# AlexGidiotis/Multimodal-Gesture-Recognition-with-LSTMs-and-CTC

Hardware: AMD Instinct MI355X
Metric: train frames/sec, fusion BiLSTM+CTC (higher is better)
Workload: dtype f32

## Files before the change

### include/mgr.h

```cpp
#ifndef MGR_H_
#define MGR_H_

#include <stddef.h>
#include <stdint.h>

#ifdef __cplusplus
extern "C" {
#endif

typedef struct mgr_ctx mgr_ctx;
typedef struct mgr_comm mgr_comm;

#define MGR_NUM_STREAMS 8
#define MGR_NUM_EVENTS 64
#define MGR_UNIQUE_ID_BYTES 128

int mgr_version(void);
const char* mgr_last_error(void);
int mgr_device_count(int* n);
int mgr_ctx_create(int device, mgr_ctx** out);
int mgr_ctx_destroy(mgr_ctx* ctx);
int mgr_device_info(mgr_ctx* ctx, int* cu_count, size_t* hbm_bytes, char* name, int name_len);

int mgr_alloc(mgr_ctx* ctx, size_t bytes, void** dptr);
int mgr_free(mgr_ctx* ctx, void* dptr);
int mgr_memset(mgr_ctx* ctx, void* d, int byte, size_t n);
int mgr_h2d(mgr_ctx* ctx, void* d, const void* h, size_t n);
int mgr_host_alloc(mgr_ctx* ctx, size_t bytes, void** out);
int mgr_host_free(mgr_ctx* ctx, void* p);
int mgr_h2d_async(mgr_ctx* ctx, void* d, const void* h_pinned, size_t n);
int mgr_d2h(mgr_ctx* ctx, void* h, const void* d, size_t n);
int mgr_d2h_async(mgr_ctx* ctx, void* h_pinned, const void* d, size_t n);
int mgr_event_sync(mgr_ctx* ctx, int ev);
int mgr_d2d(mgr_ctx* ctx, void* dst, const void* src, size_t n);
int mgr_sync(mgr_ctx* ctx);
int mgr_stream_set(mgr_ctx* ctx, int idx);
int mgr_stream_wait(mgr_ctx* ctx, int waiter, int waited);
int mgr_stream_set_priority(mgr_ctx* ctx, int idx, int level);
int mgr_event_record(mgr_ctx* ctx, int ev);
int mgr_stream_wait_event(mgr_ctx* ctx, int waiter, int ev);
int mgr_event_elapsed_ms(mgr_ctx* ctx, int ev0, int ev1, float* ms);
enum {
  MGR_K_GEMM_NN = 0, MGR_K_GEMM_TN = 1, MGR_K_GEMM_NT = 2, MGR_K_SCAN_FWD = 3, MGR_K_SCAN_BWD = 4,
  MGR_K_DENSE_FWD = 5, MGR_K_DENSE_BWD = 6, MGR_K_CTC = 7, MGR_K_ADAM = 8, MGR_K_MISC = 9, MGR_K_ALLREDUCE = 10,
  MGR_K_SCAN_FWD_NARROW = 11, MGR_K_COUNT = 12
};
int mgr_prof_enable(mgr_ctx* ctx, int family_mask);
int mgr_prof_get(mgr_ctx* ctx, int family, int* launches, float* ms);
int mgr_prof_reset(mgr_ctx* ctx);

int mgr_add_gaussian_noise(mgr_ctx* ctx, const float* X, float* Y, size_t n, float stddev, uint64_t seed);
int mgr_dropout_mask(mgr_ctx* ctx, float* mask, size_t n, float p, uint64_t seed);

int mgr_lstm_pack(mgr_ctx* ctx, const float* src, float* dst, int rows, int H, int to_keras);
int mgr_transpose(mgr_ctx* ctx, const float* src, float* dst, int rows, int cols);
int mgr_lstm_input_proj(mgr_ctx* ctx, const float* X, int ldx, const float* mask4, const float* Wp,
                        const float* bp, float* Z, int B, int T, int F, int H);
int mgr_lstm_input_proj_pair(mgr_ctx* ctx, const float* X, int ldx, const float* mask4_fwd, const float* Wp_fwd,
                             const float* bp_fwd, float* Z_fwd, const float* mask4_rev, const float* Wp_rev,
                             const float* bp_rev, float* Z_rev, int B, int T, int F, int H);
size_t mgr_lstm_input_proj_dropout_ws_bytes(int B, int F, int H);
int mgr_lstm_input_proj_dropout(mgr_ctx* ctx, const float* X, int ldx, const float* mask4, float drop_rate,
                                const float* Wp, const float* bp, float* Z, int B, int T, int F, int H, void* ws,
                                size_t ws_bytes);
int mgr_lstm_input_proj_dropout_wants_transposed(mgr_ctx* ctx, float drop_rate, int F);
int mgr_lstm_input_proj_dropout_t(mgr_ctx* ctx, const float* XT, int ldt, const float* mask4, float drop_rate,
                                  const float* Wp, const float* bp, float* Z, int B, int T, int F, int H, void* ws,
                                  size_t ws_bytes, float x_absmax);
int mgr_transpose_bt(mgr_ctx* ctx, const float* X, int ldx, float* XT, int ldt, int B, int T, int F);
size_t mgr_lstm_input_proj_dropout_ts_ws_bytes(int B, int F, int H);
int mgr_lstm_input_proj_dropout_ts(mgr_ctx* ctx, const float* XS, int ldt, const float* mask4, float drop_rate,
                                   const float* Wp, const float* bp, float* Z, int B, int T, int F, int H, void* ws,
                                   size_t ws_bytes);
int mgr_transpose_bt_split(mgr_ctx* ctx, const float* X, int ldx, float* XS, int ldt, int B, int T, int F);
int mgr_transpose_bt_split_shift(mgr_ctx* ctx, const float* X, int ldx, float* XS, int ldt, int B, int T, int F, int tshift);
int mgr_weight_planes_cache(mgr_ctx* ctx, const float* Wp, int frozen);
size_t mgr_lstm_scan_ws_bytes(int B, int T, int H);
int mgr_lstm_scan_fwd(mgr_ctx* ctx, const float* Z, const float* Up, float* Y, int ldy, const float* R,
                      int ldr, float* gates, float* cs, int B, int T, int H, int reverse, void* ws,
                      size_t ws_bytes);
typedef struct mgr_scan_job {
  const float* Z;
  const float* Up;
  float* Y;
  const float* R;
  float* gates;
  float* cs;
  int ldy, ldr, B, T, H, reverse;
  float* YT;
  long long ytb;
  int ldt;
  int yt_split;
} mgr_scan_job;
size_t mgr_lstm_scan_multi_ws_bytes(int njobs, const mgr_scan_job* jobs);
int mgr_lstm_scan_fwd_multi(mgr_ctx* ctx, int njobs, const mgr_scan_job* jobs, void* ws, size_t ws_bytes);
enum { MGR_SCAN_FORM_AUTO = 0, MGR_SCAN_FORM_PLAIN = 1, MGR_SCAN_FORM_FUSED = 3,
       MGR_SCAN_FORM_FUSED_ANY = 4 };
enum { MGR_BPTT_FORM_AUTO = 0, MGR_BPTT_FORM_TRIMMED = 1, MGR_BPTT_FORM_YIELDING = 2, MGR_BPTT_FORM_DIRECT = 3,
       MGR_BPTT_FORM_FUSED = 4, MGR_BPTT_FORM_FUSED_DIRECT = 5,
       MGR_BPTT_FORM_SINGLE_CU = 6 };
#define MGR_SEQ_NONE 0xFFFFFFFFu
typedef struct mgr_scan_launch_opts {
  unsigned struct_size;
  int form;
  unsigned* seq_out;
} mgr_scan_launch_opts;
int mgr_lstm_scan_fwd_multi_ex(mgr_ctx* ctx, int njobs, const mgr_scan_job* jobs, void* ws, size_t ws_bytes,
                               const mgr_scan_launch_opts* opts);
#define MGR_ABI_REVISION 7
int mgr_abi_struct_sizes(unsigned out[4]);
enum {
  MGR_TUNE_SCAN_PATH = 0,
  MGR_TUNE_SCAN_SYNC_CHECK = 1,
  MGR_TUNE_SCAN_PRINT_PLAN = 2,
  MGR_TUNE_SCAN_NO_XCD_LOCAL = 3,
  MGR_TUNE_SCAN_FORM = 4,
  MGR_TUNE_SCAN_LDS_IMAGE = 7,
  MGR_TUNE_BPTT_SPLIT_ROLE = 8,
  MGR_TUNE_PROJ_DENSE = 9,
  MGR_TUNE_PROJ_DENSE16_MASKED = 10,
  MGR_TUNE_PROJ_WIDE_TILES = 11,
  MGR_TUNE_PROJ_TS_TILE = 12,
  MGR_TUNE_DENSE_VALU = 13,
  MGR_TUNE_SCAN_F32_MFMA = 14,
  MGR_TUNE_GEMM_F32 = 15,
  MGR_TUNE_BPTT_FORM = 16,
  MGR_TUNE_CTC_ONE_SAMPLE = 18,
  MGR_TUNE_BPTT_SINGLE_CU = 19,
  MGR_TUNE_CTC_CHAIN_LDS_KIB = 20,
  MGR_TUNE_CTC_FRAME_LDS_KIB = 21,
  MGR_TUNE_COUNT = 24
};
int mgr_tune(mgr_ctx* ctx, int key, int value);
int mgr_tune_get(mgr_ctx* ctx, int key, int* value);
enum { MGR_SCAN_GAVE_UP = 1, MGR_SCAN_NONFINITE = 8 };
int mgr_scan_status(mgr_ctx* ctx, unsigned* out);
int mgr_scan_status_ex(mgr_ctx* ctx, unsigned out[4]);
int mgr_scan_status_clear(mgr_ctx* ctx);
int mgr_scan_status_bind(mgr_ctx* ctx, void* block);
int mgr_scan_status_inject(mgr_ctx* ctx, unsigned bits);
int mgr_update_gate_eval(mgr_ctx* ctx, unsigned mask, float* flag);
int mgr_update_gate_set(mgr_ctx* ctx, const float* flag);
int mgr_stream_wait_next_resident(mgr_ctx* ctx, int timeout_us);
int mgr_stream_wait_resident(mgr_ctx* ctx, unsigned seq, int timeout_us);
int mgr_stream_wait_resident_word(mgr_ctx* ctx, const unsigned* seq_word, int timeout_us);
int mgr_resident_wait_stats(mgr_ctx* ctx, unsigned out[4]);
int mgr_persist_stats(mgr_ctx* ctx, int* launches, int* serialised);
int mgr_probe_xcc(mgr_ctx* ctx, int nblocks, int threads, int lds_bytes, int32_t* out);
int mgr_probe_guest(mgr_ctx* ctx, int nblocks, int threads, int lds_bytes, int us, int64_t* out);
int mgr_stream_delay(mgr_ctx* ctx, int us);
int mgr_lstm_scan_bwd(mgr_ctx* ctx, const float* dY, int lddy, const float* gates, const float* cs,
                      const float* Up, float* dZ, int B, int T, int H, int reverse, void* ws, size_t ws_bytes);
typedef struct mgr_scan_bwd_job {
  const float* dY;
  const float* gates;
  const float* cs;
  const float* Up;
  float* dZ;
  int lddy, B, T, H, reverse;
  unsigned* dzmax;
  float* dbsum;
} mgr_scan_bwd_job;
size_t mgr_lstm_scan_bwd_multi_ws_bytes(int njobs, const mgr_scan_bwd_job* jobs);
int mgr_lstm_scan_bwd_multi(mgr_ctx* ctx, int njobs, const mgr_scan_bwd_job* jobs, void* ws, size_t ws_bytes);
int mgr_lstm_scan_bwd_multi_ex(mgr_ctx* ctx, int njobs, const mgr_scan_bwd_job* jobs, void* ws, size_t ws_bytes,
                               const mgr_scan_launch_opts* opts);
size_t mgr_lstm_param_grads_ws_bytes(int B, int T, int F, int H);
int mgr_lstm_param_grads(mgr_ctx* ctx, const float* X, int ldx, const float* mask4, const float* Hs, int ldh,
                         const float* dZ, float* dWp, float* dUp, float* dbp, int B, int T, int F, int H,
                         int reverse, void* ws, size_t ws_bytes);
size_t mgr_lstm_param_grads_dropout_ws_bytes(int B, int T, int F, int H);
int mgr_lstm_param_grads_dropout(mgr_ctx* ctx, const float* X, int ldx, const float* mask4, float drop_rate,
                                 const float* Hs, int ldh, const float* dZ, float* dWp, float* dUp, float* dbp, int B,
                                 int T, int F, int H, int reverse, void* ws, size_t ws_bytes);
int mgr_lstm_param_grads_dropout_wants_transposed(mgr_ctx* ctx, float drop_rate, int F);
size_t mgr_lstm_param_grads_dropout_t_ws_bytes(int B, int T, int F, int H, int ldt);
int mgr_lstm_param_grads_dropout_t(mgr_ctx* ctx, const float* XT, int ldt, const float* mask4, float drop_rate,
                                   const float* Hs, int ldh, const float* dZ, float* dWp, float* dUp, float* dbp, int B,
                                   int T, int F, int H, int reverse, void* ws, size_t ws_bytes, float x_absmax);
size_t mgr_lstm_param_grads_dropout_ts_ws_bytes(int B, int T, int F, int H, int ldt);
int mgr_lstm_param_grads_dropout_ts(mgr_ctx* ctx, const float* XS, int ldt, const float* mask4, float drop_rate,
                                    const float* Hs, int ldh, const float* dZ, float* dWp, float* dUp, float* dbp, int B,
                                    int T, int F, int H, int reverse, void* ws, size_t ws_bytes, const unsigned* dzmax,
                                    const float* dbsum, const void* proj_ws, const float* HsT);
int mgr_lstm_input_grad(mgr_ctx* ctx, const float* dZ, const float* Wp, const float* mask4, float* dX,
                        int lddx, int accumulate, int B, int T, int F, int H);

int mgr_dense_softmax_fwd(mgr_ctx* ctx, const float* A, int lda, const float* dmask, float p, uint64_t seed,
                          const float* Wd, const float* bd, float* P, int B, int T, int D, int C);
size_t mgr_dense_bwd_ws_bytes(int B, int T, int D, int C);
int mgr_dense_bwd(mgr_ctx* ctx, const float* A, int lda, const float* dmask, float p, uint64_t seed,
                  const float* dLogits, const float* Wd, float* dWd, float* dbd, float* dA, int ldda, int B,
                  int T, int D, int C, void* ws, size_t ws_bytes);
size_t mgr_head_ws_bytes(int B, int T, int D, int C, int Lmax);
int mgr_head_fwd_bwd(mgr_ctx* ctx, const float* A, int lda, const float* dmask, float p, uint64_t seed, const float* Wd, const float* bd,
                     const int32_t* labels, const int32_t* input_len, const int32_t* label_len, int B, int T, int D, int C, int Lmax,
                     int skip, int blank, float eps, float gscale, float* P, float* loss, float* loss_mean, float* dLogits, float* dWd,
                     float* dbd, float* dA, int ldda, void* ws, size_t ws_bytes);

size_t mgr_ctc_ws_bytes(int B, int T, int C, int Lmax);
int mgr_ctc_loss_grad(mgr_ctx* ctx, const float* P, const int32_t* labels, const int32_t* input_len,
                      const int32_t* label_len, int B, int T, int C, int Lmax, int skip, int blank, float eps,
                      float gscale, float* loss, float* dLogits, void* ws, size_t ws_bytes);

int mgr_adam_step(mgr_ctx* ctx, float* p, const float* g, float* m, float* v, size_t n, float lr_t, float b1,
                  float b2, float eps, float clipvalue, float gscale);
int mgr_maxnorm_cols(mgr_ctx* ctx, float* W, int rows, int cols, float maxv, float eps);
int mgr_add2d(mgr_ctx* ctx, const float* A, int lda, const float* Bm, int ldb, float* Out, int ldo, size_t rows,
              int cols);
int mgr_mean(mgr_ctx* ctx, const float* x, int n, float* out);

int mgr_comm_unique_id(uint8_t id[MGR_UNIQUE_ID_BYTES]);
int mgr_comm_init_rank(mgr_ctx* ctx, int nranks, int rank, const uint8_t id[MGR_UNIQUE_ID_BYTES], mgr_comm** out);
int mgr_allreduce_sum(mgr_comm* comm, float* dbuf, size_t n);
int mgr_allreduce_max(mgr_comm* comm, float* dbuf, size_t n);
int mgr_comm_destroy(mgr_comm* comm);
int mgr_comm_count(mgr_comm* comm, int* nranks_seen, int* rank_seen);

int mgr_frame_argmax(mgr_ctx* ctx, const float* P, int B, int T, int C, int skip, int32_t* best, float* prob);
size_t mgr_ctc_beam_ws_bytes(int B, int T, int C, int beam);
int mgr_ctc_beam_search(mgr_ctx* ctx, const float* P, const int32_t* input_len, int B, int T, int C, int skip,
                        int blank, int beam, float eps, int merge_repeated, int32_t* out, int32_t* out_len,
                        double* logp, void* ws, size_t ws_bytes);
size_t mgr_ctc_beam_lm_ws_bytes(int B, int T, int C, int beam, int top_paths);
int mgr_ctc_beam_search_lm(mgr_ctx* ctx, const float* P, const int32_t* input_len, int B, int T, int C, int skip, int blank, int beam,
                           float eps, const double* ext, const double* fin, int top_paths, int32_t* out, int32_t* out_len,
                           double* score, double* logp_ctc, void* ws, size_t ws_bytes);

size_t mgr_ctc_align_ws_bytes(int B, int T, int C, int Lmax);
int mgr_ctc_align(mgr_ctx* ctx, const float* P, const int32_t* labels, const int32_t* input_len, const int32_t* label_len, int B, int T,
                  int C, int Lmax, int skip, int blank, float eps, int32_t* path, int32_t* seg, float* conf, double* logp, void* ws,
                  size_t ws_bytes);
#define MGR_SEGMENTS_MAX_FRAMES 8192
int mgr_greedy_segments(mgr_ctx* ctx, const float* P, int B, int T, int C, int skip, float thr, int cap, int32_t* n_runs, int32_t* lab,
                        int32_t* seg, float* conf);

#define MGR_LEXICON_MAX_PHRASES 64
#define MGR_LEXICON_MAX_WORDS   255
size_t mgr_ctc_lexicon_ws_bytes(int B, int T, int C, int G, const int32_t* phrase_off);
int mgr_ctc_lexicon_decode(mgr_ctx* ctx, const float* P, const int32_t* input_len, int B, int T, int C, int skip, int blank, float eps,
                           const int32_t* phrase_off, const int32_t* phrase_words, int G, const double* ext, const double* fin, int cap,
                           int32_t* n_phr, int32_t* phr, int32_t* seg, float* conf, int32_t* path, double* score, double* logp, void* ws,
                           size_t ws_bytes);

#define MGR_RESCORE_MAX_LABELS 255
#define MGR_RESCORE_MAX_WIDTH  65536
size_t mgr_ctc_rescore_ws_bytes(int B, int T, int C, int G, const int32_t* phrase_off);
int mgr_ctc_rescore(mgr_ctx* ctx, const float* P, const int32_t* input_len, int B, int T, int C, int skip, int blank, float eps,
                    const int32_t* phrase_off, const int32_t* phrase_words, int G, const int32_t* hyp, const int32_t* hyp_len, int K,
                    int Lh, double* logp, int32_t* n_lab, void* ws, size_t ws_bytes);

#define MGR_RISK_MAX_SLOTS 32
size_t mgr_ctc_risk_ws_bytes(int B, int T, int C, int K, int Lcap, int G, const int32_t* phrase_off);
int mgr_ctc_risk_grad(mgr_ctx* ctx, const float* P, const int32_t* input_len, int B, int T, int C, int skip, int blank, float eps,
                      const int32_t* phrase_off, const int32_t* phrase_words, int G, const int32_t* hyp, const int32_t* hyp_len, int K,
                      int Lh, int Lcap, const int32_t* risk, float risk_scale, float post_scale, float gscale, int accumulate,
                      double* logp, float* weight, float* exp_risk, float* dLogits, void* ws, size_t ws_bytes);

#define MGR_SAMPLE_MAX_DRAWS 32
int mgr_ctc_sample_paths(mgr_ctx* ctx, const float* P, const int32_t* input_len, int B, int T, int C, int skip, int blank, float eps,
                         uint64_t seed, int K, int32_t* out, int32_t* out_len, int32_t* count, int32_t* n_unique, int32_t* path);

#define MGR_EDIT_MAX_LEN  4095
#define MGR_EDIT_MAX_COST 16384
size_t mgr_edit_distance_ws_bytes(int n_pairs, int Lh, int Lr, int want_ops);
int mgr_edit_distance(mgr_ctx* ctx, const int32_t* hyp, const int32_t* hyp_len, int n_hyp, int Lh, const int32_t* ref,
                      const int32_t* ref_len, int n_ref, int Lr, const int32_t* pair_h, const int32_t* pair_r, int n_pairs, int cost_sub,
                      int cost_del, int cost_ins, uint64_t ignore_mask, int32_t* dist, int32_t* counts, int32_t* lens, int8_t* ops,
                      int32_t* n_ops, void* ws, size_t ws_bytes);

#define MGR_CONV_NO_GRAD 0xFF
int mgr_conv_pool_fwd(mgr_ctx* ctx, const float* X, int N, int Hin, int Win, int Cin, const float* W, const float* b, int ks, int Cout,
                      float* Y, uint8_t* code);
int mgr_conv_pool_bwd_data(mgr_ctx* ctx, const float* dY, const uint8_t* code, const float* W, int N, int Hin, int Win, int Cin, int ks,
                           int Cout, float* dX);
size_t mgr_conv_pool_bwd_weights_ws_bytes(int N, int Hin, int Win, int Cin, int ks, int Cout);
int mgr_conv_pool_bwd_weights(mgr_ctx* ctx, const float* X, const float* dY, const uint8_t* code, int N, int Hin, int Win, int Cin, int ks,
                              int Cout, float* dW, float* db, void* ws, size_t ws_bytes);

#define MGR_SKELETAL_JOINT_COLS 12
#define MGR_SKELETAL_FEATURE_COLS 23
int mgr_skeletal_features(mgr_ctx* ctx, const double* joints, size_t n_frames, double* out);

#define MGR_ACTIVITY_JOINT_COLS 20
#define MGR_ACTIVITY_REST_COLS 16
#define MGR_ACTIVITY_OUT_COLS 5
#define MGR_ACTIVITY_MAX_FILES 65536
#define MGR_ACTIVITY_MAX_FRAMES (1LL << 26)
int mgr_skeletal_activity(mgr_ctx* ctx, const int32_t* joints, const int64_t* offsets, int n_files, long long n_frames, int rest_given,
                          int32_t* rest, int32_t* out, int32_t* status);

size_t mgr_mfcc_ws_bytes(int n_utts, long long n_frames, int frameSize, int fftN, int numChans, int numCeps);
int mgr_mfcc(mgr_ctx* ctx, const int16_t* samples, const int64_t* sample_offsets, int n_utts, long long n_frames, int frameSize,
             int frameRate, int fftN, int numChans, int numCeps, int cepLifter, double preemph, int deltas, int accs, int out_stride,
             const int32_t* loChan, const double* loWt, float* out, const int64_t* out_offsets, void* ws, size_t ws_bytes);

int mgr_roi_crop(mgr_ctx* ctx, const uint8_t* frames, int n, int H, int W, const int32_t* boxes, int img_dim, uint8_t* out);

#ifdef __cplusplus
}
#endif
#endif
```

### multimodal-gesture-recognition-with-lstms-and-ctc_amd/_capi.py

```python
import ctypes as C
import os

import numpy as np

HERE = os.path.dirname(os.path.abspath(__file__))
LIB_PATH = os.path.join(HERE, "libmgr.so")

c_float_p = C.POINTER(C.c_float)
c_int32_p = C.POINTER(C.c_int32)
vp = C.c_void_p
sz = C.c_size_t
u64 = C.c_uint64
i32 = C.c_int

SIGNATURES = {
    "mgr_version": (i32, []),
    "mgr_last_error": (C.c_char_p, []),
    "mgr_device_count": (i32, [C.POINTER(i32)]),
    "mgr_ctx_create": (i32, [i32, C.POINTER(vp)]),
    "mgr_ctx_destroy": (i32, [vp]),
    "mgr_device_info": (i32, [vp, C.POINTER(i32), C.POINTER(sz), C.c_char_p, i32]),
    "mgr_alloc": (i32, [vp, sz, C.POINTER(vp)]),
    "mgr_free": (i32, [vp, vp]),
    "mgr_memset": (i32, [vp, vp, i32, sz]),
    "mgr_h2d": (i32, [vp, vp, vp, sz]),
    "mgr_d2h": (i32, [vp, vp, vp, sz]),
    "mgr_d2d": (i32, [vp, vp, vp, sz]),
    "mgr_d2h_async": (i32, [vp, vp, vp, sz]),
    "mgr_event_sync": (i32, [vp, i32]),
    "mgr_sync": (i32, [vp]),
    "mgr_stream_set": (i32, [vp, i32]),
    "mgr_stream_wait": (i32, [vp, i32, i32]),
    "mgr_stream_set_priority": (i32, [vp, i32, i32]),
    "mgr_event_record": (i32, [vp, i32]),
    "mgr_stream_wait_event": (i32, [vp, i32, i32]),
    "mgr_event_elapsed_ms": (i32, [vp, i32, i32, C.POINTER(C.c_float)]),
    "mgr_prof_enable": (i32, [vp, i32]),
    "mgr_prof_get": (i32, [vp, i32, C.POINTER(i32), C.POINTER(C.c_float)]),
    "mgr_prof_reset": (i32, [vp]),
    "mgr_add_gaussian_noise": (i32, [vp, vp, vp, sz, C.c_float, u64]),
    "mgr_dropout_mask": (i32, [vp, vp, sz, C.c_float, u64]),
    "mgr_lstm_pack": (i32, [vp, vp, vp, i32, i32, i32]),
    "mgr_transpose": (i32, [vp, vp, vp, i32, i32]),
    "mgr_lstm_input_proj": (i32, [vp, vp, i32, vp, vp, vp, vp, i32, i32, i32, i32]),
    "mgr_lstm_input_proj_dropout_ws_bytes": (sz, [i32, i32, i32]),
    "mgr_lstm_input_proj_dropout": (i32, [vp, vp, i32, vp, C.c_float, vp, vp, vp, i32, i32, i32, i32, vp, sz]),
    "mgr_lstm_input_proj_dropout_wants_transposed": (i32, [vp, C.c_float, i32]),
    "mgr_lstm_input_proj_dropout_t": (i32, [vp, vp, i32, vp, C.c_float, vp, vp, vp, i32, i32, i32, i32, vp, sz, C.c_float]),
    "mgr_transpose_bt": (i32, [vp, vp, i32, vp, i32, i32, i32, i32]),
    "mgr_lstm_input_proj_dropout_ts_ws_bytes": (sz, [i32, i32, i32]),
    "mgr_lstm_input_proj_dropout_ts": (i32, [vp, vp, i32, vp, C.c_float, vp, vp, vp, i32, i32, i32, i32, vp, sz]),
    "mgr_transpose_bt_split": (i32, [vp, vp, i32, vp, i32, i32, i32, i32]),
    "mgr_transpose_bt_split_shift": (i32, [vp, vp, i32, vp, i32, i32, i32, i32, i32]),
    "mgr_weight_planes_cache": (i32, [vp, vp, i32]),
    "mgr_lstm_input_proj_pair": (i32, [vp, vp, i32, vp, vp, vp, vp, vp, vp, vp, vp, i32, i32, i32, i32]),
    "mgr_lstm_scan_ws_bytes": (sz, [i32, i32, i32]),
    "mgr_lstm_scan_fwd": (i32, [vp, vp, vp, vp, i32, vp, i32, vp, vp, i32, i32, i32, i32, vp, sz]),
    "mgr_lstm_scan_multi_ws_bytes": (sz, [i32, vp]),
    "mgr_lstm_scan_fwd_multi": (i32, [vp, i32, vp, vp, sz]),
    "mgr_lstm_scan_fwd_multi_ex": (i32, [vp, i32, vp, vp, sz, vp]),
    "mgr_abi_struct_sizes": (i32, [vp]),
    "mgr_tune": (i32, [vp, i32, i32]),
    "mgr_tune_get": (i32, [vp, i32, C.POINTER(i32)]),
    "mgr_probe_xcc": (i32, [vp, i32, i32, i32, vp]),
    "mgr_stream_delay": (i32, [vp, i32]),
    "mgr_probe_guest": (i32, [vp, i32, i32, i32, i32, vp]),
    "mgr_host_alloc": (i32, [vp, sz, C.POINTER(vp)]),
    "mgr_host_free": (i32, [vp, vp]),
    "mgr_h2d_async": (i32, [vp, vp, vp, sz]),
    "mgr_scan_status": (i32, [vp, vp]),
    "mgr_scan_status_clear": (i32, [vp]),
    "mgr_scan_status_ex": (i32, [vp, vp]),
    "mgr_scan_status_bind": (i32, [vp, vp]),
    "mgr_scan_status_inject": (i32, [vp, C.c_uint]),
    "mgr_update_gate_eval": (i32, [vp, C.c_uint, vp]),
    "mgr_update_gate_set": (i32, [vp, vp]),
    "mgr_stream_wait_next_resident": (i32, [vp, i32]),
    "mgr_stream_wait_resident": (i32, [vp, C.c_uint, i32]),
    "mgr_stream_wait_resident_word": (i32, [vp, vp, i32]),
    "mgr_resident_wait_stats": (i32, [vp, vp]),
    "mgr_persist_stats": (i32, [vp, C.POINTER(i32), C.POINTER(i32)]),
    "mgr_skeletal_features": (i32, [vp, vp, sz, vp]),
    "mgr_skeletal_activity": (i32, [vp, vp, vp, i32, C.c_longlong, i32, vp, vp, vp]),
    "mgr_mfcc_ws_bytes": (sz, [i32, C.c_longlong, i32, i32, i32, i32]),
    "mgr_mfcc": (i32, [vp, vp, vp, i32, C.c_longlong, i32, i32, i32, i32, i32, i32, C.c_double, i32, i32, i32, vp, vp, vp, vp, vp,
                       sz]),
    "mgr_lstm_scan_bwd_multi_ws_bytes": (sz, [i32, vp]),
    "mgr_lstm_scan_bwd_multi": (i32, [vp, i32, vp, vp, sz]),
    "mgr_lstm_scan_bwd_multi_ex": (i32, [vp, i32, vp, vp, sz, vp]),
    "mgr_lstm_scan_bwd": (i32, [vp, vp, i32, vp, vp, vp, vp, i32, i32, i32, i32, vp, sz]),
    "mgr_lstm_param_grads_ws_bytes": (sz, [i32, i32, i32, i32]),
    "mgr_lstm_param_grads": (i32, [vp, vp, i32, vp, vp, i32, vp, vp, vp, vp, i32, i32, i32, i32, i32, vp, sz]),
    "mgr_lstm_param_grads_dropout_ws_bytes": (sz, [i32, i32, i32, i32]),
    "mgr_lstm_param_grads_dropout": (i32, [vp, vp, i32, vp, C.c_float, vp, i32, vp, vp, vp, vp, i32, i32, i32, i32, i32, vp, sz]),
    "mgr_lstm_param_grads_dropout_wants_transposed": (i32, [vp, C.c_float, i32]),
    "mgr_lstm_param_grads_dropout_t_ws_bytes": (sz, [i32, i32, i32, i32, i32]),
    "mgr_lstm_param_grads_dropout_t": (i32, [vp, vp, i32, vp, C.c_float, vp, i32, vp, vp, vp, vp, i32, i32, i32, i32, i32, vp, sz, C.c_float]),
    "mgr_lstm_param_grads_dropout_ts_ws_bytes": (sz, [i32, i32, i32, i32, i32]),
    "mgr_lstm_param_grads_dropout_ts": (i32, [vp, vp, i32, vp, C.c_float, vp, i32, vp, vp, vp, vp, i32, i32, i32, i32, i32, vp, sz, vp, vp, vp, vp]),
    "mgr_lstm_input_grad": (i32, [vp, vp, vp, vp, vp, i32, i32, i32, i32, i32, i32]),
    "mgr_dense_softmax_fwd": (i32, [vp, vp, i32, vp, C.c_float, u64, vp, vp, vp, i32, i32, i32, i32]),
    "mgr_dense_bwd_ws_bytes": (sz, [i32, i32, i32, i32]),
    "mgr_dense_bwd": (i32, [vp, vp, i32, vp, C.c_float, u64, vp, vp, vp, vp, vp, i32, i32, i32, i32, i32, vp, sz]),
    "mgr_head_ws_bytes": (sz, [i32, i32, i32, i32, i32]),
    "mgr_head_fwd_bwd": (i32, [vp, vp, i32, vp, C.c_float, u64, vp, vp, vp, vp, vp, i32, i32, i32, i32, i32, i32, i32, C.c_float, C.c_float,
                               vp, vp, vp, vp, vp, vp, vp, i32, vp, sz]),
    "mgr_ctc_ws_bytes": (sz, [i32, i32, i32, i32]),
    "mgr_ctc_loss_grad": (i32, [vp, vp, vp, vp, vp, i32, i32, i32, i32, i32, i32, C.c_float, C.c_float, vp, vp, vp, sz]),
    "mgr_adam_step": (i32, [vp, vp, vp, vp, vp, sz, C.c_float, C.c_float, C.c_float, C.c_float, C.c_float, C.c_float]),
    "mgr_maxnorm_cols": (i32, [vp, vp, i32, i32, C.c_float, C.c_float]),
    "mgr_add2d": (i32, [vp, vp, i32, vp, i32, vp, i32, sz, i32]),
    "mgr_mean": (i32, [vp, vp, i32, vp]),
    "mgr_comm_unique_id": (i32, [C.c_char_p]),
    "mgr_comm_init_rank": (i32, [vp, i32, i32, C.c_char_p, C.POINTER(vp)]),
    "mgr_allreduce_sum": (i32, [vp, vp, sz]),
    "mgr_allreduce_max": (i32, [vp, vp, sz]),
    "mgr_comm_destroy": (i32, [vp]),
    "mgr_comm_count": (i32, [vp, C.POINTER(i32), C.POINTER(i32)]),
    "mgr_frame_argmax": (i32, [vp, vp, i32, i32, i32, i32, vp, vp]),
    "mgr_ctc_beam_ws_bytes": (sz, [i32, i32, i32, i32]),
    "mgr_ctc_beam_search": (i32, [vp, vp, vp, i32, i32, i32, i32, i32, i32, C.c_float, i32, vp, vp, vp, vp, sz]),
    "mgr_ctc_beam_lm_ws_bytes": (sz, [i32, i32, i32, i32, i32]),
    "mgr_ctc_beam_search_lm": (i32, [vp, vp, vp, i32, i32, i32, i32, i32, i32, C.c_float, vp, vp, i32, vp, vp, vp, vp, vp, sz]),
    "mgr_ctc_align_ws_bytes": (sz, [i32, i32, i32, i32]),
    "mgr_ctc_align": (i32, [vp, vp, vp, vp, vp, i32, i32, i32, i32, i32, i32, C.c_float, vp, vp, vp, vp, vp, sz]),
    "mgr_greedy_segments": (i32, [vp, vp, i32, i32, i32, i32, C.c_float, i32, vp, vp, vp, vp]),
    "mgr_ctc_lexicon_ws_bytes": (sz, [i32, i32, i32, i32, vp]),
    "mgr_ctc_lexicon_decode": (i32, [vp, vp, vp, i32, i32, i32, i32, i32, C.c_float, vp, vp, i32, vp, vp, i32, vp, vp, vp, vp, vp, vp, vp, vp,
                                     sz]),
    "mgr_ctc_rescore_ws_bytes": (sz, [i32, i32, i32, i32, vp]),
    "mgr_ctc_rescore": (i32, [vp, vp, vp, i32, i32, i32, i32, i32, C.c_float, vp, vp, i32, vp, vp, i32, i32, vp, vp, vp, sz]),
    "mgr_ctc_risk_ws_bytes": (sz, [i32, i32, i32, i32, i32, i32, vp]),
    "mgr_ctc_risk_grad": (i32, [vp, vp, vp, i32, i32, i32, i32, i32, C.c_float, vp, vp, i32, vp, vp, i32, i32, i32, vp, C.c_float, C.c_float,
                                C.c_float, i32, vp, vp, vp, vp, vp, sz]),
    "mgr_ctc_sample_paths": (i32, [vp, vp, vp, i32, i32, i32, i32, i32, C.c_float, u64, i32, vp, vp, vp, vp, vp]),
    "mgr_edit_distance_ws_bytes": (sz, [i32, i32, i32, i32]),
    "mgr_edit_distance": (i32, [vp, vp, vp, i32, i32, vp, vp, i32, i32, vp, vp, i32, i32, i32, i32, u64, vp, vp, vp, vp, vp, vp, sz]),
    "mgr_conv_pool_fwd": (i32, [vp, vp, i32, i32, i32, i32, vp, vp, i32, i32, vp, vp]),
    "mgr_conv_pool_bwd_data": (i32, [vp, vp, vp, vp, i32, i32, i32, i32, i32, i32, vp]),
    "mgr_conv_pool_bwd_weights_ws_bytes": (sz, [i32, i32, i32, i32, i32, i32]),
    "mgr_conv_pool_bwd_weights": (i32, [vp, vp, vp, vp, i32, i32, i32, i32, i32, i32, vp, vp, vp, sz]),
    "mgr_roi_crop": (i32, [vp, vp, i32, i32, i32, vp, i32, vp]),
}

SCAN_GAVE_UP, SCAN_NONFINITE = 1, 8

(K_GEMM_NN, K_GEMM_TN, K_GEMM_NT, K_SCAN_FWD, K_SCAN_BWD, K_DENSE_FWD, K_DENSE_BWD, K_CTC, K_ADAM, K_MISC, K_ALLREDUCE, K_SCAN_FWD_NARROW) = range(12)
KERNEL_FAMILIES = ["gemm_nn", "gemm_tn", "gemm_nt", "scan_fwd", "scan_bwd", "dense_fwd", "dense_bwd", "ctc", "adam", "misc", "allreduce",
                   "scan_fwd_narrow"]



class ScanJob(C.Structure):
    _fields_ = [("Z", vp), ("Up", vp), ("Y", vp), ("R", vp), ("gates", vp), ("cs", vp),
                ("ldy", i32), ("ldr", i32), ("B", i32), ("T", i32), ("H", i32), ("reverse", i32),
                ("YT", vp), ("ytb", C.c_longlong), ("ldt", i32), ("yt_split", i32)]


class ScanBwdJob(C.Structure):
    _fields_ = [("dY", vp), ("gates", vp), ("cs", vp), ("Up", vp), ("dZ", vp),
                ("lddy", i32), ("B", i32), ("T", i32), ("H", i32), ("reverse", i32), ("dzmax", vp), ("dbsum", vp)]


class ScanLaunchOpts(C.Structure):
    _fields_ = [("struct_size", C.c_uint), ("form", i32), ("seq_out", vp)]


SCAN_FORM_AUTO, SCAN_FORM_PLAIN, SCAN_FORM_FUSED, SCAN_FORM_FUSED_ANY = 0, 1, 3, 4
BPTT_FORM_AUTO, BPTT_FORM_TRIMMED, BPTT_FORM_YIELDING, BPTT_FORM_DIRECT, BPTT_FORM_FUSED, BPTT_FORM_FUSED_DIRECT, BPTT_FORM_SINGLE_CU = range(7)
SEQ_NONE = 0xFFFFFFFF
ABI_REVISION = 7
TUNE_SCAN_PATH = 0
TUNE_SCAN_SYNC_CHECK = 1
TUNE_SCAN_PRINT_PLAN = 2
TUNE_SCAN_NO_XCD_LOCAL = 3
TUNE_SCAN_FORM = 4
TUNE_SCAN_LDS_IMAGE = 7
TUNE_BPTT_SPLIT_ROLE = 8
TUNE_PROJ_DENSE = 9
TUNE_PROJ_DENSE16_MASKED = 10
TUNE_PROJ_WIDE_TILES = 11
TUNE_PROJ_TS_TILE = 12
TUNE_DENSE_VALU = 13
TUNE_SCAN_F32_MFMA = 14
TUNE_GEMM_F32 = 15
TUNE_BPTT_FORM = 16
TUNE_CTC_ONE_SAMPLE = 18
TUNE_BPTT_SINGLE_CU = 19
TUNE_CTC_CHAIN_LDS_KIB = 20
TUNE_CTC_FRAME_LDS_KIB = 21
TUNE_COUNT = 24


def make_launch_opts(form=0, seq_out=0):
    o = ScanLaunchOpts()
    o.struct_size = C.sizeof(ScanLaunchOpts)
    o.form = int(form)
    o.seq_out = int(seq_out) or None
    return o


def make_scan_bwd_jobs(jobs):
    arr = (ScanBwdJob * len(jobs))()
    for a, j in zip(arr, jobs):
        for k in ("dY", "gates", "cs", "Up", "dZ", "dzmax", "dbsum"):
            v = j.get(k, 0)
            setattr(a, k, v.ptr if isinstance(v, DeviceArray) else (v or 0))
        for k in ("lddy", "B", "T", "H", "reverse"):
            setattr(a, k, int(j[k]))
    return arr


def make_scan_jobs(jobs):
    arr = (ScanJob * len(jobs))()
    for a, j in zip(arr, jobs):
        for k in ("Z", "Up", "Y", "R", "gates", "cs", "YT"):
            v = j.get(k, 0)
            setattr(a, k, v.ptr if isinstance(v, DeviceArray) else (v or 0))
        for k in ("ldy", "ldr", "B", "T", "H", "reverse", "ytb", "ldt", "yt_split"):
            setattr(a, k, int(j.get(k, 0)))
    return arr


_lib = None


class MgrError(RuntimeError):
    pass


def load_library(build_if_missing=True):
    global _lib
    if _lib is not None:
        return _lib
    if not os.path.exists(LIB_PATH) and build_if_missing:
        from . import _build
        _build.build(verbose=False)
    if not os.path.exists(LIB_PATH):
        raise MgrError("libmgr.so is missing (%s) and could not be built; there is no CPU fallback" % LIB_PATH)
    lib = C.CDLL(LIB_PATH)
    for name, (res, args) in SIGNATURES.items():
        fn = getattr(lib, name)
        fn.restype = res
        fn.argtypes = args
    sizes = (C.c_uint * 4)()
    if lib.mgr_abi_struct_sizes(sizes) != 0 or tuple(sizes) != (C.sizeof(ScanJob), C.sizeof(ScanBwdJob), C.sizeof(ScanLaunchOpts), ABI_REVISION):
        raise MgrError("libmgr.so was built from another include/mgr.h than this binding (struct sizes / revision %s, expected %s): rebuild it"
                       % (tuple(sizes), (C.sizeof(ScanJob), C.sizeof(ScanBwdJob), C.sizeof(ScanLaunchOpts), ABI_REVISION)))
    _lib = lib
    return lib


def check(rc, lib=None):
    if rc != 0:
        lib = lib or load_library()
        raise MgrError("libmgr error %d: %s" % (rc, lib.mgr_last_error().decode(errors="replace")))


class DeviceArray:

    __slots__ = ("dev", "ptr", "shape", "dtype", "nbytes", "_own")

    def __init__(self, dev, ptr, shape, dtype, own=True):
# ... 146 lines not shown
```

### multimodal-gesture-recognition-with-lstms-and-ctc_amd/csrc/common.h

```cpp
#pragma once
#include <hip/hip_runtime.h>
#include <stdarg.h>
#include <stdint.h>
#include <stdio.h>
#include <string.h>

#include "../../include/mgr.h"
#include "ws_layout.h"

constexpr int MGR_MAX_PERSIST = 8;
constexpr int MGR_MAX_FROZEN = 32;

constexpr size_t MGR_SMALL_D2H = 4096;

enum : unsigned {
  MGR_ATTR_SCAN_CLUSTER = 1u, MGR_ATTR_SCAN_CLUSTER_BWD = 2u, MGR_ATTR_SCAN_CLUSTER_FUSED = 64u,
  MGR_ATTR_PROJ_SPLIT = 16u, MGR_ATTR_DW_SPLIT = 32u, MGR_ATTR_PROJ_NARROW = 2048u,
  MGR_ATTR_CTC = 128u, MGR_ATTR_ALIGN = 512u, MGR_ATTR_SEGMENTS = 1024u, MGR_ATTR_ROI = 256u,
  MGR_ATTR_LEXICON = 4096u, MGR_ATTR_RISK = 8192u,
};

struct mgr_ctx {
  int device;
  int cu_count;
  size_t hbm_bytes;
  char name[64];
  hipStream_t streams[MGR_NUM_STREAMS];
  int cur;
  hipEvent_t events[MGR_NUM_EVENTS];
  hipEvent_t xev[64];
  int xev_next;
  int prof_mask;
  struct ProfPair {
    hipEvent_t a, b;
  };
  ProfPair* prof_pairs[MGR_K_COUNT];
  int prof_n[MGR_K_COUNT];
  int prof_cap[MGR_K_COUNT];
  float prof_ms[MGR_K_COUNT];
  int prof_launches[MGR_K_COUNT];
  int tune[MGR_TUNE_COUNT];
  void* h_small_pinned;
  unsigned* sticky_status;
  unsigned* status_bound;
  const float* gate_flag;
  struct Persist {
    hipEvent_t done;
    int active, stream, wgs, waves, per_cu, fused;
    unsigned seq;
  };
  Persist persist[MGR_MAX_PERSIST];
  unsigned persist_seq;
  int persist_serialised;
  unsigned attr_done;
  struct PlaneEntry {
    const void* Wp;
    const void* ws;
    int B, F, H;
    const char* region;
    size_t region_bytes;
  };
  const void* frozen_w[MGR_MAX_FROZEN];
  PlaneEntry planes[MGR_MAX_FROZEN];
  unsigned planes_evict, frozen_evict;
};

int mgr_fail(int code, const char* fmt, ...);

static inline bool mgr_planes_overlap(const mgr_ctx::PlaneEntry& e, const void* p, size_t n) {
  const char* a = static_cast<const char*>(p);
  return e.Wp && a < e.region + e.region_bytes && e.region < a + n;
}
static inline void mgr_planes_forget_range(mgr_ctx* c, const void* p, size_t n) {
  if (!p || !n) return;
  for (int i = 0; i < MGR_MAX_FROZEN; ++i)
    if (mgr_planes_overlap(c->planes[i], p, n)) c->planes[i] = mgr_ctx::PlaneEntry{};
}

#define MGR_HIP(expr)                                                                      \
  do {                                                                                     \
    hipError_t _e = (expr);                                                                \
    if (_e != hipSuccess) return mgr_fail(-2, "%s failed: %s", #expr, hipGetErrorString(_e)); \
  } while (0)

#define MGR_REQUIRE(cond, ...)                  \
  do {                                          \
    if (!(cond)) return mgr_fail(-1, __VA_ARGS__); \
  } while (0)

#define MGR_LAUNCH_CHECK() MGR_HIP(hipGetLastError())

static inline hipStream_t mgr_stream(mgr_ctx* c) { return c->streams[c->cur]; }
static inline unsigned* mgr_status_block(mgr_ctx* c) { return c->status_bound ? c->status_bound : c->sticky_status; }

int mgr_prof_begin(mgr_ctx* c, int family);
int mgr_prof_end(mgr_ctx* c, int family);

static inline size_t mgr_align_up(size_t x, size_t a) { return (x + a - 1) / a * a; }
static inline int mgr_grid256(size_t n, size_t cap) { return (int)((n + 255) / 256 < cap ? (n + 255) / 256 : cap); }

__host__ __device__ static inline uint64_t mgr_mix64(uint64_t z) {
  z += 0x9E3779B97F4A7C15ull;
  z = (z ^ (z >> 30)) * 0xBF58476D1CE4E5B9ull;
  z = (z ^ (z >> 27)) * 0x94D049BB133111EBull;
  return z ^ (z >> 31);
}
__host__ __device__ static inline uint32_t mgr_rand_u32(uint64_t seed, uint64_t idx) {
  return (uint32_t)(mgr_mix64(seed * 0xD1342543DE82EF95ull + idx) >> 32);
}
__host__ __device__ static inline float mgr_drop_scale(uint64_t seed, uint64_t idx, float p, float inv_keep) {
  float u = (float)(mgr_rand_u32(seed, idx) >> 8) * (1.0f / 16777216.0f);
  return (u >= p) ? inv_keep : 0.0f;
}
int mgr_transpose_bt_strided(mgr_ctx* c, const float* X, int ldx, float* XT, int ldt, long long xtb, int ldt_fill, int B, int T, int F);
int mgr_transpose_bt_split_strided(mgr_ctx* c, const float* X, int ldx, float* XS, int ldt, long long xsb, int ldt_fill, int B, int T, int F);
int mgr_param_grads_du_db(mgr_ctx* c, const float* Hs, int ldh, const float* dZ, float* dUp, float* dbp, int B, int T, int F, int H, int reverse,
                          void* ws, const float* dbsum);

int mgr_rowmax_bt(mgr_ctx* c, const float* dZ, int N, int T, int B, unsigned* zmax, float* zsum);
```

### multimodal-gesture-recognition-with-lstms-and-ctc_amd/csrc/elementwise.hip

```cpp
#include "common.h"

namespace {

constexpr int kBlock = 256;
static inline int grid_for(size_t n, int per_block = kBlock) {
  size_t g = (n + per_block - 1) / per_block;
  if (g > 2048) g = 2048;
  if (g < 1) g = 1;
  return (int)g;
}

__global__ void k_add_noise(const float* __restrict__ X, float* __restrict__ Y, size_t n, float stddev, uint64_t seed) {
  size_t npair = (n + 1) / 2;
  for (size_t i = blockIdx.x * (size_t)blockDim.x + threadIdx.x; i < npair; i += (size_t)gridDim.x * blockDim.x) {
    uint64_t r = mgr_mix64(seed * 0xD1342543DE82EF95ull + i);
    float u1 = ((float)((uint32_t)(r >> 40)) + 1.0f) * (1.0f / 16777216.0f);
    float u2 = (float)((uint32_t)(r >> 8) & 0xFFFFFF) * (1.0f / 16777216.0f);
    float rad = sqrtf(-2.0f * logf(u1)) * stddev;
    float s, c;
    sincosf(6.283185307179586f * u2, &s, &c);
    size_t e = 2 * i;
    Y[e] = X[e] + rad * c;
    if (e + 1 < n) Y[e + 1] = X[e + 1] + rad * s;
  }
}

__global__ void k_dropout_mask(float* __restrict__ m, size_t n, float p, float inv_keep, uint64_t seed) {
  for (size_t i = blockIdx.x * (size_t)blockDim.x + threadIdx.x; i < n; i += (size_t)gridDim.x * blockDim.x)
    m[i] = mgr_drop_scale(seed, i, p, inv_keep);
}

__global__ void k_pack(const float* __restrict__ src, float* __restrict__ dst, int rows, int H, int to_keras) {
  size_t n = (size_t)rows * 4 * H;
  for (size_t i = blockIdx.x * (size_t)blockDim.x + threadIdx.x; i < n; i += (size_t)gridDim.x * blockDim.x) {
    size_t r = i / (4 * H);
    int c = (int)(i % (4 * H));
    int sc;
    if (to_keras) {
      int g = c / H, u = c % H;
      sc = u * 4 + g;
    } else {
      int u = c / 4, g = c % 4;
      sc = g * H + u;
    }
    dst[i] = src[r * 4 * H + sc];
  }
}

__global__ void k_transpose(const float* __restrict__ src, float* __restrict__ dst, int rows, int cols) {
  __shared__ float tile[32][33];
  int bx = blockIdx.x * 32, by = blockIdx.y * 32;
  int tx = threadIdx.x & 31, ty = threadIdx.x >> 5;
  for (int j = ty; j < 32; j += 8) {
    int r = by + j, c = bx + tx;
    tile[j][tx] = (r < rows && c < cols) ? src[(size_t)r * cols + c] : 0.f;
  }
  __syncthreads();
  for (int j = ty; j < 32; j += 8) {
    int c = bx + j, r = by + tx;
    if (c < cols && r < rows) dst[(size_t)c * rows + r] = tile[tx][j];
  }
}

__global__ void k_adam(float* __restrict__ p, const float* __restrict__ g, float* __restrict__ m, float* __restrict__ v,
                       size_t n, float lr_t, float b1, float b2, float eps, float clipvalue, float gscale,
                       const float* __restrict__ gate, unsigned* __restrict__ skipped) {
  if (gate && gate[0] != 0.f) {
    if (blockIdx.x == 0 && threadIdx.x == 0) atomicAdd(skipped, 1u);
    return;
  }
  for (size_t i = blockIdx.x * (size_t)blockDim.x + threadIdx.x; i < n; i += (size_t)gridDim.x * blockDim.x) {
    float gi = g[i] * gscale;
    if (clipvalue > 0.f) gi = fminf(fmaxf(gi, -clipvalue), clipvalue);
    float mi = b1 * m[i] + (1.f - b1) * gi;
    float vi = b2 * v[i] + (1.f - b2) * gi * gi;
    m[i] = mi;
    v[i] = vi;
    p[i] = p[i] - lr_t * mi / (sqrtf(vi) + eps);
  }
}

constexpr int MN_RG = 32;
__global__ __launch_bounds__(32 * MN_RG) void k_maxnorm(float* __restrict__ W, int rows, int cols, float maxv, float eps,
                                                         const float* __restrict__ gate) {
  __shared__ float part[MN_RG][32];
  if (gate && gate[0] != 0.f) return;
  int tx = threadIdx.x & 31, ty = threadIdx.x >> 5;
  int c = blockIdx.x * 32 + tx;
  float s = 0.f;
  if (c < cols)
    for (int r = ty; r < rows; r += MN_RG) {
      float w = W[(size_t)r * cols + c];
      s += w * w;
    }
  part[ty][tx] = s;
  __syncthreads();
  if (ty == 0) {
    float t = 0.f;
    for (int k = 0; k < MN_RG; ++k) t += part[k][tx];
    float nrm = sqrtf(t);
    part[0][tx] = fminf(fmaxf(nrm, 0.f), maxv) / (eps + nrm);
  }
  __syncthreads();
  float sc = part[0][tx];
  if (c < cols)
    for (int r = ty; r < rows; r += MN_RG) W[(size_t)r * cols + c] *= sc;
}

__global__ void k_add2d(const float* __restrict__ A, int lda, const float* __restrict__ Bm, int ldb, float* __restrict__ O,
                        int ldo, size_t rows, int cols) {
  size_t n = rows * (size_t)cols;
  for (size_t i = blockIdx.x * (size_t)blockDim.x + threadIdx.x; i < n; i += (size_t)gridDim.x * blockDim.x) {
    size_t r = i / cols;
    int c = (int)(i % cols);
    O[r * ldo + c] = A[r * lda + c] + Bm[r * ldb + c];
  }
}

__global__ void k_mean(const float* __restrict__ x, int n, float* __restrict__ out) {
  __shared__ double sh[kBlock];
  double s = 0;
  for (int i = threadIdx.x; i < n; i += blockDim.x) s += (double)x[i];
  sh[threadIdx.x] = s;
  __syncthreads();
  for (int o = kBlock / 2; o > 0; o >>= 1) {
    if ((int)threadIdx.x < o) sh[threadIdx.x] += sh[threadIdx.x + o];
    __syncthreads();
  }
  if (threadIdx.x == 0) out[0] = (float)(sh[0] / (double)n);
}

__global__ void k_frame_argmax(const float* __restrict__ P, int B, int T, int C, int skip, int32_t* __restrict__ best,
                               float* __restrict__ prob) {
  int To = T - skip;
  size_t n = (size_t)B * To;
  for (size_t i = blockIdx.x * (size_t)blockDim.x + threadIdx.x; i < n; i += (size_t)gridDim.x * blockDim.x) {
    int b = (int)(i / To), t = (int)(i % To);
    const float* row = P + ((size_t)b * T + skip + t) * C;
    float mx = row[0];
    int am = 0;
    for (int c = 1; c < C; ++c) {
      float v = row[c];
      if (v > mx) {
        mx = v;
        am = c;
      }
    }
    best[i] = am;
    prob[i] = mx;
  }
}

__global__ void k_probe_xcc(int32_t* out) {
  extern __shared__ float dummy[];
  unsigned x;
  asm volatile("s_getreg_b32 %0, hwreg(HW_REG_XCC_ID)" : "=s"(x));
  if (threadIdx.x == 0) out[blockIdx.x] = (int32_t)(x & 0xF);
}

__global__ void k_guest(long long* __restrict__ out, int us) {
  extern __shared__ float dummy[];
  const unsigned long long t0 = wall_clock64();
  if (us > 0) {
    const unsigned long long ticks = (unsigned long long)us * 100ull;
    for (int i = 0; i < (1 << 22); ++i) {
      if (wall_clock64() - t0 >= ticks) break;
      __builtin_amdgcn_s_sleep(16);
    }
  }
  if (threadIdx.x == 0) {
    out[2 * blockIdx.x] = (long long)t0;
    out[2 * blockIdx.x + 1] = (long long)wall_clock64();
  }
}

}

__global__ void k_delay(int us) {
  const unsigned long long t0 = wall_clock64();
  const unsigned long long ticks = (unsigned long long)us * 100ull;
  for (int i = 0; i < (1 << 22); ++i) {
    if (wall_clock64() - t0 >= ticks) break;
    __builtin_amdgcn_s_sleep(16);
  }
}

extern "C" {

int mgr_stream_delay(mgr_ctx* c, int us) {
  MGR_REQUIRE(c && us >= 0 && us <= 100000, "bad argument");
  if (us == 0) return 0;
  hipLaunchKernelGGL(k_delay, dim3(1), dim3(64), 0, mgr_stream(c), us);
  MGR_LAUNCH_CHECK();
  return 0;
}

int mgr_probe_guest(mgr_ctx* c, int nblocks, int threads, int lds_bytes, int us, int64_t* out) {
  MGR_REQUIRE(c && out && nblocks > 0 && threads > 0 && threads <= 1024 && lds_bytes >= 0 && lds_bytes <= 160 * 1024 && us >= 0 && us <= 100000,
              "bad argument");
  MGR_HIP(hipFuncSetAttribute(reinterpret_cast<const void*>(k_guest), hipFuncAttributeMaxDynamicSharedMemorySize, 160 * 1024));
  hipLaunchKernelGGL(k_guest, dim3(1), dim3(64), 0, mgr_stream(c), reinterpret_cast<long long*>(out), 0);
  hipLaunchKernelGGL(k_guest, dim3(nblocks), dim3(threads), lds_bytes, mgr_stream(c), reinterpret_cast<long long*>(out) + 2, us);
  MGR_LAUNCH_CHECK();
  return 0;
}

int mgr_probe_xcc(mgr_ctx* c, int nblocks, int threads, int lds_bytes, int32_t* out) {
  MGR_REQUIRE(c && out && nblocks > 0 && threads > 0, "bad argument");
  MGR_HIP(hipFuncSetAttribute(reinterpret_cast<const void*>(k_probe_xcc), hipFuncAttributeMaxDynamicSharedMemorySize, 160 * 1024));
  hipLaunchKernelGGL(k_probe_xcc, dim3(nblocks), dim3(threads), lds_bytes, mgr_stream(c), out);
  MGR_LAUNCH_CHECK();
  return 0;
}

int mgr_add_gaussian_noise(mgr_ctx* c, const float* X, float* Y, size_t n, float stddev, uint64_t seed) {
  MGR_REQUIRE(c && X && Y, "null argument");
  if (n == 0) return 0;
  mgr_prof_begin(c, MGR_K_MISC);
  hipLaunchKernelGGL(k_add_noise, dim3(grid_for((n + 1) / 2)), dim3(kBlock), 0, mgr_stream(c), X, Y, n, stddev, seed);
  MGR_LAUNCH_CHECK();
  mgr_prof_end(c, MGR_K_MISC);
  return 0;
}

int mgr_dropout_mask(mgr_ctx* c, float* mask, size_t n, float p, uint64_t seed) {
  MGR_REQUIRE(c && mask, "null argument");
  MGR_REQUIRE(p >= 0.f && p < 1.f, "dropout rate %f out of [0,1)", p);
  if (n == 0) return 0;
  hipLaunchKernelGGL(k_dropout_mask, dim3(grid_for(n)), dim3(kBlock), 0, mgr_stream(c), mask, n, p, 1.0f / (1.0f - p), seed);
  MGR_LAUNCH_CHECK();
  return 0;
}

int mgr_lstm_pack(mgr_ctx* c, const float* src, float* dst, int rows, int H, int to_keras) {
  MGR_REQUIRE(c && src && dst && src != dst, "null or aliased argument");
  MGR_REQUIRE(rows > 0 && H > 0, "bad shape");
  hipLaunchKernelGGL(k_pack, dim3(grid_for((size_t)rows * 4 * H)), dim3(kBlock), 0, mgr_stream(c), src, dst, rows, H, to_keras);
  MGR_LAUNCH_CHECK();
  return 0;
}

int mgr_transpose(mgr_ctx* c, const float* src, float* dst, int rows, int cols) {
  MGR_REQUIRE(c && src && dst && src != dst, "null or aliased argument");
  MGR_REQUIRE(rows > 0 && cols > 0, "bad shape");
  dim3 grid((cols + 31) / 32, (rows + 31) / 32);
  hipLaunchKernelGGL(k_transpose, grid, dim3(kBlock), 0, mgr_stream(c), src, dst, rows, cols);
  MGR_LAUNCH_CHECK();
  return 0;
}

int mgr_adam_step(mgr_ctx* c, float* p, const float* g, float* m, float* v, size_t n, float lr_t, float b1, float b2,
                  float eps, float clipvalue, float gscale) {
  MGR_REQUIRE(c && p && g && m && v, "null argument");
  if (n == 0) return 0;
  mgr_prof_begin(c, MGR_K_ADAM);
  hipLaunchKernelGGL(k_adam, dim3(grid_for(n)), dim3(kBlock), 0, mgr_stream(c), p, g, m, v, n, lr_t, b1, b2, eps, clipvalue, gscale,
                     c->gate_flag, mgr_status_block(c) + 2);
  MGR_LAUNCH_CHECK();
  mgr_prof_end(c, MGR_K_ADAM);
  return 0;
}

int mgr_maxnorm_cols(mgr_ctx* c, float* W, int rows, int cols, float maxv, float eps) {
  MGR_REQUIRE(c && W, "null argument");
  MGR_REQUIRE(rows > 0 && cols > 0, "bad shape");
  hipLaunchKernelGGL(k_maxnorm, dim3((cols + 31) / 32), dim3(32 * MN_RG), 0, mgr_stream(c), W, rows, cols, maxv, eps, c->gate_flag);
  MGR_LAUNCH_CHECK();
  return 0;
}

int mgr_add2d(mgr_ctx* c, const float* A, int lda, const float* Bm, int ldb, float* Out, int ldo, size_t rows, int cols) {
  MGR_REQUIRE(c && A && Bm && Out, "null argument");
  MGR_REQUIRE(cols > 0 && lda >= cols && ldb >= cols && ldo >= cols, "bad shape");
  if (rows == 0) return 0;
  hipLaunchKernelGGL(k_add2d, dim3(grid_for(rows * (size_t)cols)), dim3(kBlock), 0, mgr_stream(c), A, lda, Bm, ldb, Out, ldo, rows, cols);
  MGR_LAUNCH_CHECK();
  return 0;
}

int mgr_mean(mgr_ctx* c, const float* x, int n, float* out) {
  MGR_REQUIRE(c && x && out && n > 0, "bad argument");
  hipLaunchKernelGGL(k_mean, dim3(1), dim3(kBlock), 0, mgr_stream(c), x, n, out);
  MGR_LAUNCH_CHECK();
  return 0;
}

int mgr_frame_argmax(mgr_ctx* c, const float* P, int B, int T, int C, int skip, int32_t* best, float* prob) {
  MGR_REQUIRE(c && P && best && prob, "null argument");
  MGR_REQUIRE(B > 0 && T > skip && C > 0 && skip >= 0, "bad shape");
  hipLaunchKernelGGL(k_frame_argmax, dim3(grid_for((size_t)B * (T - skip))), dim3(kBlock), 0, mgr_stream(c), P, B, T, C, skip, best, prob);
  MGR_LAUNCH_CHECK();
  return 0;
}

}
```

### multimodal-gesture-recognition-with-lstms-and-ctc_amd/csrc/gemm.hip

```cpp
#include "common.h"
#include "split_f16.h"

namespace {

#ifndef MGR_GEMM_BK
#define MGR_GEMM_BK 16
#endif
#ifndef MGR_GEMM_NBUF
#define MGR_GEMM_NBUF 2
#endif
constexpr int BM = 128, BN = 128, BK = MGR_GEMM_BK, NBUF = MGR_GEMM_NBUF, LDS_LD = BM + 4;
constexpr int LPT = BK / 8;

struct RegTile {
  float v[4 * LPT];
};

__device__ __forceinline__ void load_kc(RegTile& r, const float* __restrict__ base, size_t ld, int m0, int k0, int Mlim,
                                        int Klim, bool vec, int tid) {
#pragma unroll
  for (int i = 0; i < LPT; ++i) {
    int idx4 = tid + i * 256;
    int m = idx4 / (BK / 4), k4 = (idx4 % (BK / 4)) * 4;
    int gm = m0 + m, gk = k0 + k4;
// ... 1059 lines not shown
  fetch(R1, (nst > 1 ? 1 : 0) * TK);
  stash(R0, 0);
  __syncthreads();
  for (int st = 0; st < nst; st += 2) {
    fetch(R0, (st + 2 < nst ? st + 2 : nst - 1) * TK);
    mma(0);
    stash(R1, 1);
    __syncthreads();
    fetch(R1, (st + 3 < nst ? st + 3 : nst - 1) * TK);
    if (st + 1 < nst) mma(1);
    stash(R0, 0);
    __syncthreads();
  }
  float* out = P + (size_t)gb * Fp * H;
#pragma unroll
  for (int mt = 0; mt < 2; ++mt)
#pragma unroll
    for (int nt = 0; nt < 2; ++nt) {
      const int u = u0 + acc_col(wc * 64 + nt * 32, lane & 31);
      const float cz = 1.f / zscale(u < H ? u : H - 1), cx = 1.f / sx;
#pragma unroll
      for (int reg = 0; reg < 16; ++reg) {
        const int r = acc_row(wr * 64 + mt * 32, reg, lane >> 5);
        if (q0 + r < cnt && u < H) out[(size_t)(q0 + r) * H + u] = acc[mt][nt][reg] * cx * cz * kval[(size_t)gb * Fp + q0 + r];
      }
    }
}

__global__ __launch_bounds__(256) void k_dw_gather(const float* __restrict__ P, const int* __restrict__ kpos, float* __restrict__ dWp,
                                                   int B, int F, int Fp, int H) {
  const size_t n = (size_t)4 * F * H;
  for (size_t i = blockIdx.x * (size_t)256 + threadIdx.x; i < n; i += (size_t)gridDim.x * 256) {
    const int u = (int)(i % H);
    const int f = (int)((i / H) % F);
    const int g = (int)(i / ((size_t)H * F));
    float s = 0.f;
    for (int b = 0; b < B; ++b) {
      const int pos = kpos[((size_t)g * B + b) * F + f];
      if (pos >= 0) s += P[(((size_t)g * B + b) * Fp + pos) * H + u];
    }
    dWp[(size_t)f * 4 * H + 4 * u + g] = s;
  }
}

__global__ __launch_bounds__(256, 2) void k_gemm_nt(const float* __restrict__ dZ, const float* __restrict__ Wp,
                                                 const float* __restrict__ mask4, float* __restrict__ dX, int lddx,
                                                 int accumulate, int B, int T, int F, int N) {
  __shared__ __attribute__((aligned(16))) float As2[NBUF][BK][LDS_LD];
  __shared__ __attribute__((aligned(16))) float Bs2[NBUF][BK][LDS_LD];
  const int tid = threadIdx.x, lane = tid & 63, wave = tid >> 6, wr = wave >> 1, wc = wave & 1;
  const int f0 = blockIdx.x * BN, r0 = blockIdx.y * BM, b = blockIdx.z;
  const float* Zb = dZ + (size_t)b * T * N;
  f32x16 acc[2][2];
  zero_acc(acc);
  RegTile ra, rb, rm;
  if (mask4) {
#pragma unroll
    for (int i = 0; i < LPT; ++i) {
      int idx4 = tid + i * 256;
      int f = f0 + idx4 / (BK / 4);
      f = f < F ? f : F - 1;
#pragma unroll
      for (int g = 0; g < 4; ++g) rm.v[i * 4 + g] = mask4[((size_t)g * B + b) * F + f];
    }
  }
  auto stash = [&](int buf) {
    if (mask4) {
#pragma unroll
      for (int e = 0; e < 4 * LPT; ++e) rb.v[e] *= rm.v[e];
    }
    store_kc(As2[buf], ra, tid);
    store_kc(Bs2[buf], rb, tid);
  };
  const int nfast = N / BK;
  if (nfast > 0) {
    load_kc_fast(ra, Zb, (size_t)N, r0, 0, T, tid);
    load_kc_fast(rb, Wp, (size_t)N, f0, 0, F, tid);
    stash(0);
    __syncthreads();
    int buf = 0;
    for (int kt = 0; kt < nfast; ++kt) {
      const bool more = kt + 1 < nfast;
      if (more) {
        load_kc_fast(ra, Zb, (size_t)N, r0, (kt + 1) * BK, T, tid);
        load_kc_fast(rb, Wp, (size_t)N, f0, (kt + 1) * BK, F, tid);
      }
      mma_stage(As2[buf], Bs2[buf], acc, wr, wc, lane);
      if (NBUF == 1) __syncthreads();
      if (more) stash(buf ^ (NBUF - 1));
      __syncthreads();
      buf ^= (NBUF - 1);
    }
  }
  for (int k0 = nfast * BK; k0 < N; k0 += BK) {
    load_kc(ra, Zb, (size_t)N, r0, k0, T, N, true, tid);
    load_kc(rb, Wp, (size_t)N, f0, k0, F, N, true, tid);
    stash(0);
    __syncthreads();
    mma_stage(As2[0], Bs2[0], acc, wr, wc, lane);
    __syncthreads();
  }
#pragma unroll
  for (int mt = 0; mt < 2; ++mt)
#pragma unroll
    for (int nt = 0; nt < 2; ++nt) {
      int f = f0 + acc_col(wc * 64 + nt * 32, lane & 31);
#pragma unroll
      for (int reg = 0; reg < 16; ++reg) {
        int r = r0 + acc_row(wr * 64 + mt * 32, reg, lane >> 5);
        if (r < T && f < F) {
          float* o = dX + ((size_t)b * T + r) * lddx + f;
          *o = accumulate ? (*o + acc[mt][nt][reg]) : acc[mt][nt][reg];
        }
      }
    }
}

__global__ void k_reduce(const float* __restrict__ slab, float* __restrict__ out, size_t n, int nslab) {
  for (size_t i = blockIdx.x * (size_t)blockDim.x + threadIdx.x; i < n; i += (size_t)gridDim.x * blockDim.x) {
    float s = 0.f;
    for (int k = 0; k < nslab; ++k) s += slab[(size_t)k * n + i];
    out[i] = s;
  }
}

__global__ __launch_bounds__(256) void k_colsum(const float* __restrict__ dZ, float* __restrict__ slab, size_t rows, int N,
                                                int rows_per_wg) {
  __shared__ float4 part[128];
  const size_t rbeg = (size_t)blockIdx.x * rows_per_wg;
  const size_t rend = rbeg + rows_per_wg < rows ? rbeg + rows_per_wg : rows;
  const int cl = threadIdx.x & 127, ry = threadIdx.x >> 7, N4 = N / 4;
  for (int c0 = 0; c0 < N4; c0 += 128) {
    const int c4 = c0 + cl;
    float4 s = make_float4(0.f, 0.f, 0.f, 0.f);
    if (c4 < N4)
      for (size_t r = rbeg + ry; r < rend; r += 2) {
        const float4 v = *reinterpret_cast<const float4*>(dZ + r * N + 4 * c4);
        s.x += v.x;
        s.y += v.y;
        s.z += v.z;
        s.w += v.w;
      }
    if (ry == 1) part[cl] = s;
    __syncthreads();
    if (ry == 0 && c4 < N4) {
      const float4 o = part[cl];
      *reinterpret_cast<float4*>(slab + (size_t)blockIdx.x * N + 4 * c4) = make_float4(s.x + o.x, s.y + o.y, s.z + o.z, s.w + o.w);
    }
    __syncthreads();
  }
}

__global__ __launch_bounds__(256) void k_reduce_tall(const float* __restrict__ slab, float* __restrict__ out, int n, int nslab) {
  __shared__ float part[8][32];
  const int e = blockIdx.x * 32 + (threadIdx.x & 31), kl = threadIdx.x >> 5;
  float s = 0.f;
  if (e < n)
    for (int k = kl; k < nslab; k += 8) s += slab[(size_t)k * n + e];
  part[kl][threadIdx.x & 31] = s;
  __syncthreads();
  if (kl == 0 && e < n) {
    float t = 0.f;
    for (int k = 0; k < 8; ++k) t += part[k][threadIdx.x & 31];
    out[e] = t;
  }
}

static int tn_groups(int B, int F, int N) {
  int tiles = ((F + BM - 1) / BM) * ((N + BN - 1) / BN);
  int sg = (1024 + tiles - 1) / tiles;
  if (sg > B) sg = B;
  if (sg < 1) sg = 1;
  return sg;
}
static int colsum_wgs(size_t rows) {
  size_t w = (rows + 31) / 32;
  if (w > 512) w = 512;
  if (w < 1) w = 1;
  return (int)w;
}

static bool aligned16(const void* p) { return (reinterpret_cast<uintptr_t>(p) & 15) == 0; }

struct SplitCall {
  bool f16, trusted;
  float sx;
  unsigned* gate;
};
static SplitCall split_call(const mgr_ctx* c, float x_absmax, bool shape_ok , unsigned* gate_word) {
  const float xb = fabsf(x_absmax);
  SplitCall k;
  k.trusted = x_absmax < 0.f;
  k.f16 = shape_ok && xb > 0.f && xb < 1.0e30f && c->tune[MGR_TUNE_GEMM_F32] == 0;
  k.sx = k.f16 ? split_scale<SPLIT_NONFINITE_NONE>(xb, SPLIT_NO_FLOOR) : 0.f;
  k.gate = (k.f16 && !k.trusted) ? gate_word : nullptr;
  return k;
}
static void launch_absmax_gate(hipStream_t s, const float* X, size_t n4, const SplitCall& k) {
  hipLaunchKernelGGL(k_absmax_gate, dim3(mgr_grid256(n4, 4096)), dim3(256), 0, s, X, n4, 65000.f / k.sx, k.gate);
}

}

extern "C" {

int mgr_lstm_input_proj(mgr_ctx* c, const float* X, int ldx, const float* mask4, const float* Wp, const float* bp,
                        float* Z, int B, int T, int F, int H) {
  MGR_REQUIRE(c && X && Wp && bp && Z, "null argument");
  MGR_REQUIRE(B > 0 && T > 0 && F > 0 && H > 0 && ldx >= F, "bad shape");
  MGR_REQUIRE(aligned16(Wp) && aligned16(Z), "Wp/Z must be 16-byte aligned");
  int N = 4 * H;
  int vecA = (ldx % 4 == 0) && (F % 4 == 0) && aligned16(X);
  dim3 grid((N + BN - 1) / BN, (T + BM - 1) / BM, B);
  mgr_prof_begin(c, MGR_K_GEMM_NN);
  hipLaunchKernelGGL(k_gemm_nn, grid, dim3(256), 0, mgr_stream(c), X, ldx, mask4, Wp, bp, Z, B, T, F, N, vecA);
  MGR_LAUNCH_CHECK();
  mgr_prof_end(c, MGR_K_GEMM_NN);
  return 0;
}

int mgr_lstm_input_proj_pair(mgr_ctx* c, const float* X, int ldx, const float* mask4_fwd, const float* Wp_fwd,
                             const float* bp_fwd, float* Z_fwd, const float* mask4_rev, const float* Wp_rev,
                             const float* bp_rev, float* Z_rev, int B, int T, int F, int H) {
  MGR_REQUIRE(c && X && Wp_fwd && bp_fwd && Z_fwd && Wp_rev && bp_rev && Z_rev, "null argument");
  MGR_REQUIRE((mask4_fwd == nullptr) == (mask4_rev == nullptr), "both directions masked or neither");
  MGR_REQUIRE(B > 0 && T > 0 && F > 0 && H > 0 && ldx >= F, "bad shape");
  const int Nd = 4 * H;
  const bool fast = (ldx % 4 == 0) && (F % BK == 0) && aligned16(X) && aligned16(Wp_fwd) && aligned16(Wp_rev);
  if (!fast || (2 * Nd + BN - 1) / BN >= 2 * ((Nd + BN - 1) / BN)) {
    int r = mgr_lstm_input_proj(c, X, ldx, mask4_fwd, Wp_fwd, bp_fwd, Z_fwd, B, T, F, H);
    if (r) return r;
    return mgr_lstm_input_proj(c, X, ldx, mask4_rev, Wp_rev, bp_rev, Z_rev, B, T, F, H);
  }
  dim3 grid((2 * Nd + BN - 1) / BN, (T + BM - 1) / BM, B);
  mgr_prof_begin(c, MGR_K_GEMM_NN);
  hipLaunchKernelGGL(k_gemm_nn2, grid, dim3(256), 0, mgr_stream(c), X, ldx, mask4_fwd, mask4_rev, Wp_fwd, Wp_rev, bp_fwd, bp_rev,
                     Z_fwd, Z_rev, B, T, F, Nd);
  MGR_LAUNCH_CHECK();
  mgr_prof_end(c, MGR_K_GEMM_NN);
  return 0;
}

static size_t sp_fp(int F) { return (size_t)(F + SP_SK - 1) / SP_SK * SP_SK; }

struct ProjDropWs { int* kidx; float* kval; int* kcnt; unsigned* wmax; float* Wg; size_t bytes; };
static ProjDropWs proj_dropout_ws_layout(void* ws, int B, int F, int H) {
  mgr_ws_carver w(ws);
  const size_t nl = (size_t)4 * B * sp_fp(F);
  return {w.take<int>(nl), w.take<float>(nl), w.take<int>((size_t)4 * B), w.take<unsigned>(64), w.take<float>((size_t)F * 4 * H), w.off};
}
size_t mgr_lstm_input_proj_dropout_ws_bytes(int B, int F, int H) { return proj_dropout_ws_layout(nullptr, B, F, H).bytes; }

static bool sparse_proj_shape(const mgr_ctx* c, float drop_rate, int F) {
  return drop_rate >= 0.3f && F >= 16 && F <= SP_MAXF && c->tune[MGR_TUNE_PROJ_DENSE] == 0;
}

int mgr_lstm_input_proj_dropout_wants_transposed(mgr_ctx* c, float drop_rate, int F) {
  return (c && sparse_proj_shape(c, drop_rate, F) && F >= 128) ? 1 : 0;
}

static int input_proj_dropout_impl(mgr_ctx* c, const float* X, int ldx, bool transposed, const float* mask4, float drop_rate,
                                   const float* Wp, const float* bp, float* Z, int B, int T, int F, int H, void* ws, size_t ws_bytes,
                                   float x_absmax = 0.f) {
  const int Fp = (int)sp_fp(F);
  const ProjDropWs L = proj_dropout_ws_layout(ws, B, F, H);
  int *kidx = L.kidx, *kcnt = L.kcnt;
  float *kval = L.kval, *Wg = L.Wg;
  unsigned* wmax = L.wmax;
  hipStream_t s = mgr_stream(c);
  const SplitCall sc = split_call(c, x_absmax, transposed && drop_rate < 0.99f, wmax + 1);
  const bool f16 = sc.f16;
  unsigned* const gate = sc.gate;
  const bool dense = f16 && (!mask4 || c->tune[MGR_TUNE_PROJ_DENSE16_MASKED] == 2);
  MGR_REQUIRE(mask4 || transposed, "a projection without a dropout mask is only handled from the transposed copy");
  const bool lists = !dense || gate;
  mgr_prof_begin(c, MGR_K_GEMM_NN);
  if (!transposed && mask4 && F >= 16 && F <= NP_MAXF && c->tune[MGR_TUNE_PROJ_WIDE_TILES] != 2) {
    if (!(c->attr_done & MGR_ATTR_PROJ_NARROW)) {
      MGR_HIP(hipFuncSetAttribute(reinterpret_cast<const void*>(k_proj_narrow<32>), hipFuncAttributeMaxDynamicSharedMemorySize, (int)np_lds_bytes(NP_MAXF)));
      c->attr_done |= MGR_ATTR_PROJ_NARROW;
    }
    const int nchunk = ((T + SP_TM - 1) / SP_TM + NP_RPW - 1) / NP_RPW;
    const int nwg = ((H + NP_TU - 1) / NP_TU) * ((nchunk * B + 7) / 8) * 8;
    if (F <= 20)
      hipLaunchKernelGGL(k_proj_narrow<10>, dim3(nwg), dim3(256), np_lds_bytes(F), s, X, ldx, mask4, Wp, bp, Z, B, T, F, H);
    else if (F <= 40)
      hipLaunchKernelGGL(k_proj_narrow<20>, dim3(nwg), dim3(256), np_lds_bytes(F), s, X, ldx, mask4, Wp, bp, Z, B, T, F, H);
    else
      hipLaunchKernelGGL(k_proj_narrow<32>, dim3(nwg), dim3(256), np_lds_bytes(F), s, X, ldx, mask4, Wp, bp, Z, B, T, F, H);
    MGR_LAUNCH_CHECK();
    mgr_prof_end(c, MGR_K_GEMM_NN);
    return 0;
  }
  if (lists && mask4)
    hipLaunchKernelGGL(k_mask_compact, dim3(4 * B), dim3(64), 0, s, mask4, F, Fp, kidx, kval, kcnt, (int*)nullptr, wmax);
  else if (lists)
    hipLaunchKernelGGL(k_mask_all, dim3(4 * B), dim3(64), 0, s, F, Fp, kidx, kval, kcnt, wmax);
  else
    MGR_HIP(hipMemsetAsync(wmax, 0, sizeof(unsigned), s));
  {
    const size_t n = (size_t)F * H;
    const int wgs = mgr_grid256(n, 2048);
    hipLaunchKernelGGL(k_gate_major, dim3(wgs), dim3(256), 0, s, Wp, Wg, F, H, wmax);
  }
  const bool wide = c->tune[MGR_TUNE_PROJ_WIDE_TILES] == 2 && !transposed;
  const int tu = wide ? 128 : 64;
  const int ntiles = ((H + tu - 1) / tu) * ((((T + SP_TM - 1) / SP_TM) * B + 7) / 8) * 8;
  if (f16) {
    const float sx = sc.sx;
    if (gate) {
      MGR_HIP(hipMemsetAsync(gate, 0, sizeof(unsigned), s));
      launch_absmax_gate(s, X, (size_t)B * F * ldx / 4, sc);
    }
    if (dense)
      hipLaunchKernelGGL(k_gemm_nn_dense16, dim3(ntiles), dim3(256), 0, s, X, ldx, mask4, Wg, bp, Z, B, T, F, H, wmax,
                         mask4 ? 1.f / (1.f - drop_rate) : 1.f, sx, gate);
    else
      hipLaunchKernelGGL(k_gemm_nn_sparse16, dim3(ntiles), dim3(256), 0, s, X, ldx, kidx, kval, kcnt, Wg, bp, Z, B, T, Fp, F, H, wmax,
// ... 255 lines not shown
```

### multimodal-gesture-recognition-with-lstms-and-ctc_amd/csrc/gemm_split.hip

```cpp
#include "common.h"
#include "split_f16.h"

namespace {

typedef short tr4 __attribute__((__vector_size__(4 * sizeof(short))));
typedef short tr8 __attribute__((__vector_size__(8 * sizeof(short))));
typedef __attribute__((address_space(3))) char lds_char;
typedef __attribute__((address_space(3))) tr4 lds_tr4;

constexpr float XS_SCALE = 8192.f;
constexpr int PS_TM = 128, PS_SK = 32;
constexpr int PS_HP = 128;

__device__ __forceinline__ void ps_dma_b128(const void* gbase, unsigned voff, unsigned lds_addr) {
  unsigned keep;
  asm volatile("s_mov_b32 %0, m0\n\ts_mov_b32 m0, %3\n\ts_nop 0\n\tglobal_load_lds_dwordx4 %1, %2\n\ts_mov_b32 m0, %0"
               : "=&s"(keep)
               : "v"(voff), "s"(gbase), "s"(lds_addr)
               : "memory");
}
__device__ __forceinline__ int ps_swz(int row) { return ((row & 3) << 2) | ((row >> 2) & 3); }

__global__ __launch_bounds__(64) void k_lists32(const float* __restrict__ mask4, int F, int Fp32, int* __restrict__ lists, int* __restrict__ kcnt,
                                                int* __restrict__ kpos ,
                                                unsigned* __restrict__ cword) {
  const int gb = blockIdx.x, lane = threadIdx.x;
  int* out = lists + (size_t)gb * Fp32;
  int n = 0;
  unsigned seen = 0u;
  bool mixed = false;
  if (mask4) {
    const float* m = mask4 + (size_t)gb * F;
    for (int f0 = 0; f0 < F; f0 += 64) {
      const int f = f0 + lane;
      const float v = f < F ? m[f] : 0.f;
      const bool take = f < F && v != 0.f;
      const unsigned long long bal = __ballot(take);
      if (take) {
        out[n + __popcll(bal & ((1ull << lane) - 1ull))] = f | (f << 16);
        const unsigned vb = __float_as_uint(v);
        mixed = mixed || (seen != 0u && seen != vb);
        seen = vb;
      }
      if (kpos && f < F) kpos[(size_t)gb * F + f] = take ? n + __popcll(bal & ((1ull << lane) - 1ull)) : -1;
      n += __popcll(bal);
    }
  } else {
    for (int f = lane; f < F; f += 64) {
      out[f] = f | (f << 16);
      if (kpos) kpos[(size_t)gb * F + f] = f;
    }
    n = F;
    seen = __float_as_uint(1.f);
  }
  const unsigned long long have = __ballot(seen != 0u);
  if (have) {
    const unsigned first = __shfl(seen, __ffsll((long long)have) - 1);
    mixed = __any(mixed || (seen != 0u && seen != first));
    if (lane == 0) {
      const unsigned old = atomicCAS(cword, 0u, first);
      if (mixed || (old != 0u && old != first)) atomicExch(cword, 0x7FC00000u);
    }
  }
  if (lane == 0) kcnt[gb] = n;
  __syncthreads();
  const int first_kept = n > 0 ? (out[0] & 0xFFFF) : 0;
  for (int i = n + lane; i < (n + 31) / 32 * 32; i += 64) out[i] = first_kept | (F << 16);
}

__global__ __launch_bounds__(256) void k_wmax(const float* __restrict__ Wp, size_t n4, unsigned* __restrict__ wmax) {
  __shared__ float part[4];
  float m = 0.f;
  for (size_t i = blockIdx.x * (size_t)256 + threadIdx.x; i < n4; i += (size_t)gridDim.x * 256) {
    const float4 w = reinterpret_cast<const float4*>(Wp)[i];
    m = fmaxf(fmaxf(m, fmaxf(fabsf(w.x), fabsf(w.y))), fmaxf(fabsf(w.z), fabsf(w.w)));
  }
#pragma unroll
  for (int o = 32; o > 0; o >>= 1) m = fmaxf(m, __shfl_xor(m, o));
  if ((threadIdx.x & 63) == 0) part[threadIdx.x >> 6] = m;
  __syncthreads();
  if (threadIdx.x == 0) atomicMax(wmax, __float_as_uint(fmaxf(fmaxf(part[0], part[1]), fmaxf(part[2], part[3]))));
}
__device__ __forceinline__ float ps_wscale(const unsigned* wmax) {
  return split_scale<SPLIT_NONFINITE_ZERO>(__uint_as_float(*wmax), -60);
}
__global__ __launch_bounds__(256) void k_wplanes(const float* __restrict__ Wp, _Float16* __restrict__ WS, int F, int H, int Hp,
                                                 const unsigned* __restrict__ wmax) {
  const float sw = ps_wscale(wmax);
  const size_t n = (size_t)(F + 1) * Hp;
  for (size_t i = blockIdx.x * (size_t)256 + threadIdx.x; i < n; i += (size_t)gridDim.x * 256) {
    const int u = (int)(i % Hp), f = (int)(i / Hp);
    float4 w = make_float4(0.f, 0.f, 0.f, 0.f);
    if (f < F && u < H) w = *reinterpret_cast<const float4*>(Wp + ((size_t)f * H + u) * 4);
    const float g4[4] = {w.x, w.y, w.z, w.w};
#pragma unroll
    for (int g = 0; g < 4; ++g) {
      _Float16 hi, lo;
      split_f16(g4[g] * sw, hi, lo);
      _Float16* row = WS + ((size_t)g * (F + 1) + f) * 2 * Hp;
      row[u] = hi;
      row[Hp + u] = lo;
    }
  }
}

constexpr int TS_TT = 128, TS_LP = 66;
__device__ __forceinline__ float dw_zscale(unsigned zm_bits);

template <bool SCALED>
__device__ __forceinline__ void ts_tile(const float* __restrict__ Xb, int ldx, float* __restrict__ XSb, int ldt, int T, int F, int fill, int tshift,
                                        const unsigned* __restrict__ zmax_b, bool vec) {
  __shared__ __attribute__((aligned(16))) unsigned img[2][64][TS_LP];
  const int t0 = blockIdx.x * TS_TT, f0 = blockIdx.y * 64;
  const int lane = threadIdx.x & 63, w = threadIdx.x >> 6;
  {
    const int f = f0 + lane, fc = f < F ? f : F - 1;
    float v[16][2];
#pragma unroll
    for (int i = 0; i < 16; ++i)
#pragma unroll
      for (int h = 0; h < 2; ++h) {
        const int ts = t0 + 2 * (w + 4 * i) + h + tshift;
        v[i][h] = Xb[(size_t)(ts < 0 ? 0 : ts < T ? ts : T - 1) * ldx + fc];
      }
#pragma unroll
    for (int i = 0; i < 16; ++i)
#pragma unroll
      for (int h = 0; h < 2; ++h) {
        const int t = t0 + 2 * (w + 4 * i) + h, ts = t + tshift;
        v[i][h] = (t < T && ts >= 0 && ts < T && f < F) ? v[i][h] : 0.f;
      }
    float sc = XS_SCALE;
    if constexpr (SCALED) sc = dw_zscale(zmax_b[fc]);
#pragma unroll
    for (int i = 0; i < 16; ++i) {
      _Float16 hi0, lo0, hi1, lo1;
      split_f16(v[i][0] * sc, hi0, lo0);
      split_f16(v[i][1] * sc, hi1, lo1);
      const int p = w + 4 * i;
      img[0][lane][p] = (unsigned)__builtin_bit_cast(unsigned short, hi0) | ((unsigned)__builtin_bit_cast(unsigned short, hi1) << 16);
      img[1][lane][p] = (unsigned)__builtin_bit_cast(unsigned short, lo0) | ((unsigned)__builtin_bit_cast(unsigned short, lo1) << 16);
    }
  }
  __syncthreads();
  const int j = lane & 15;
  const int t = t0 + 8 * j;
#pragma unroll
  for (int i = 0; i < 4; ++i) {
    const int r = (lane >> 4) + 4 * w + 16 * i, f = f0 + r;
    if (f >= F || t >= fill) continue;
    _Float16* row = reinterpret_cast<_Float16*>(XSb + (size_t)f * ldt);
    const uint2 h0 = *reinterpret_cast<const uint2*>(&img[0][r][4 * j]), h1 = *reinterpret_cast<const uint2*>(&img[0][r][4 * j + 2]);
    const uint2 l0 = *reinterpret_cast<const uint2*>(&img[1][r][4 * j]), l1 = *reinterpret_cast<const uint2*>(&img[1][r][4 * j + 2]);
    if (vec && t + 8 <= fill) {
      *reinterpret_cast<uint4*>(row + t) = make_uint4(h0.x, h0.y, h1.x, h1.y);
      *reinterpret_cast<uint4*>(row + ldt + t) = make_uint4(l0.x, l0.y, l1.x, l1.y);
    } else {
      const unsigned hw[4] = {h0.x, h0.y, h1.x, h1.y}, lw[4] = {l0.x, l0.y, l1.x, l1.y};
#pragma unroll
      for (int k = 0; k < 8; ++k)
        if (t + k < fill) {
          row[t + k] = __builtin_bit_cast(_Float16, (unsigned short)(hw[k >> 1] >> (16 * (k & 1))));
          row[ldt + t + k] = __builtin_bit_cast(_Float16, (unsigned short)(lw[k >> 1] >> (16 * (k & 1))));
        }
    }
  }
}

__global__ __launch_bounds__(256) void k_transpose_split(const float* __restrict__ X, int ldx, float* __restrict__ XS, int ldt, int T, int F,
                                                         long long xsb , int fill, int tshift,
                                                         int vec ) {
  const int b = blockIdx.z;
  ts_tile<false>(X + (size_t)b * T * ldx, ldx, XS + (size_t)b * (xsb ? (size_t)xsb : (size_t)F * ldt), ldt, T, F, fill, tshift, nullptr, vec != 0);
}

template <int WC>
struct PsCfg {
  static constexpr int NW = 2 * WC, TU = 32 * WC, NBUF = WC == 2 ? 3 : 4;
  static constexpr int B_ROW = 4 * TU;
  static constexpr int A_BYTES = 2 * PS_SK * 256, B_BYTES = PS_SK * B_ROW, STAGE = A_BYTES + B_BYTES, LDS = NBUF * STAGE;
  static constexpr int NI = PS_SK / NW;
  static constexpr int AI = 16 / NW;
  static constexpr int BI = B_BYTES / 1024 / NW;
  static constexpr int RB = 1024 / B_ROW;
};

template <int WC>
__global__ __launch_bounds__(128 * WC, WC == 2 ? 2 : 1) void k_proj_split(const char* __restrict__ XS, int ldt, const int* __restrict__ lists,
                                                                          const int* __restrict__ kcnt, const unsigned* __restrict__ cword,
                                                                          const char* __restrict__ WS, int Hp, const unsigned* __restrict__ wmax,
                                                                          const float* __restrict__ bp, float* __restrict__ Z, int B, int T,
                                                                          int Fp32, int F, int H) {
  typedef PsCfg<WC> C;
  extern __shared__ __attribute__((aligned(16))) char ps_smem[];
  const int tid = threadIdx.x, lane = tid & 63;
  const int wave = __builtin_amdgcn_readfirstlane(tid >> 6), wr = wave / WC, wc = wave % WC;
  const int N = 4 * H;
  const int ncol = (H + C::TU - 1) / C::TU, nrow = (T + PS_TM - 1) / PS_TM;
  const XcdTile wt = xcd_tile(blockIdx.x, ncol);
  const int rt = wt.group;
  if (rt >= nrow * B) return;
  const int u0 = wt.item * C::TU, r0 = (rt % nrow) * PS_TM, b = rt / nrow;
  const char* XSb = XS + (size_t)b * F * ldt * 4;
  const unsigned lds0 = (unsigned)(uintptr_t)(lds_char*)ps_smem;

  const int c1 = (__builtin_amdgcn_readfirstlane(kcnt[0 * B + b]) + PS_SK - 1) / PS_SK;
  const int c2 = c1 + (__builtin_amdgcn_readfirstlane(kcnt[1 * B + b]) + PS_SK - 1) / PS_SK;
  const int c3 = c2 + (__builtin_amdgcn_readfirstlane(kcnt[2 * B + b]) + PS_SK - 1) / PS_SK;
  const int NT = c3 + (__builtin_amdgcn_readfirstlane(kcnt[3 * B + b]) + PS_SK - 1) / PS_SK;

  const int dch = lane & 15;
  const int hsel = -(lane >> 5);
  const int drow = lane >> 4;
  const int m1 = -(int)(drow == 1), m2 = -(int)(drow == 2), m3 = -(int)(drow == 3);
  unsigned a_src[C::AI], b_src[C::BI];
#pragma unroll
  for (int i = 0; i < C::AI; ++i) {
    const int k = 2 * (C::AI * wave + i) + (lane >> 5);
    const int ch = dch ^ ps_swz(k);
    a_src[i] = (unsigned)((drow & 1) * 2 * ldt + (r0 + 8 * ch) * 2);
  }
#pragma unroll
  for (int j = 0; j < C::BI; ++j) {
    if constexpr (WC == 2) {
      const int k = 4 * (C::BI * wave + j) + drow;
      const int ch = dch ^ ps_swz(k);
      b_src[j] = (unsigned)((ch >> 3) * 2 * Hp + (u0 + 8 * (ch & 7)) * 2);
    } else {
      const int k = 2 * (C::BI * wave + j) + (lane >> 5);
      const int ch = dch ^ ps_swz(k);
      b_src[j] = (unsigned)((drow & 1) * 2 * Hp + (u0 + 8 * ch) * 2);
    }
  }
  struct Idx {
    int e[C::NI];
  };
  auto stage_gate = [&](int n) { return (n >= c1) + (n >= c2) + (n >= c3); };
  auto load_idx = [&](Idx& I, int n) {
    n = n < NT ? n : NT - 1;
    const int g = stage_gate(n);
    const int first = n >= c3 ? c3 : n >= c2 ? c2 : n >= c1 ? c1 : 0;
    const int* lp = lists + ((size_t)g * B + b) * Fp32 + (n - first) * PS_SK + C::NI * wave;
#pragma unroll
    for (int r = 0; r < C::NI; ++r) I.e[r] = lp[r];
  };
  auto issue = [&](const Idx& I, int n) {
    const unsigned buf = lds0 + (unsigned)(n % C::NBUF) * C::STAGE;
    const int wbase = stage_gate(n < NT ? n : NT - 1) * (F + 1);
#pragma unroll
    for (int i = 0; i < C::AI; ++i) {
      const int f0 = I.e[2 * i] & 0xFFFF, f1 = I.e[2 * i + 1] & 0xFFFF;
      const int f = f0 + ((f1 - f0) & hsel);
      ps_dma_b128(XSb, (unsigned)f * (unsigned)(4 * ldt) + a_src[i], buf + (unsigned)((C::AI * wave + i) * 1024));
    }
#pragma unroll
    for (int j = 0; j < C::BI; ++j) {
// ... 109 lines not shown

__global__ __launch_bounds__(256) void k_rowmax_bt(const float* __restrict__ dZ, int N, int T, unsigned* __restrict__ zmax, float* __restrict__ zsum) {
  __shared__ float part[2][4][64];
  const int b = blockIdx.y, col = blockIdx.x * 64 + (threadIdx.x & 63), w = threadIdx.x >> 6;
  float m = 0.f, sm = 0.f;
  if (col < N) {
    const float* p = dZ + (size_t)b * T * N + col;
    for (int t = w; t < T; t += 4) {
      const float v = p[(size_t)t * N];
      m = fmaxf(m, fabsf(v));
      sm += v;
    }
  }
  part[0][w][threadIdx.x & 63] = m;
  part[1][w][threadIdx.x & 63] = sm;
  __syncthreads();
  if (w == 0 && col < N) {
    if (zmax) zmax[(size_t)b * N + col] = __float_as_uint(fmaxf(fmaxf(part[0][0][threadIdx.x], part[0][1][threadIdx.x]), fmaxf(part[0][2][threadIdx.x], part[0][3][threadIdx.x])));
    if (zsum) zsum[(size_t)b * N + col] = (part[1][0][threadIdx.x] + part[1][1][threadIdx.x]) + (part[1][2][threadIdx.x] + part[1][3][threadIdx.x]);
  }
}
__device__ __forceinline__ float dw_zscale(unsigned zm_bits) {
  return split_scale<SPLIT_NONFINITE_NAN>(__uint_as_float(zm_bits), -100);
}
__global__ __launch_bounds__(256) void k_transpose_split_scaled(const float* __restrict__ dZ, int N, float* __restrict__ dZS, int ldt, int T,
                                                                const unsigned* __restrict__ zmax, int vec) {
  const int b = blockIdx.z;
  ts_tile<true>(dZ + (size_t)b * T * N, N, dZS + (size_t)b * N * ldt, ldt, T, N, ldt, 0, zmax + (size_t)b * N, vec != 0);
}

typedef float dw_f4 __attribute__((ext_vector_type(4)));

template <int NW>
__global__ __launch_bounds__(64 * NW, 1) void k_dw_split(const char* __restrict__ XS, int ldt, const int* __restrict__ lists,
                                                         const int* __restrict__ kcnt, const unsigned* __restrict__ cword,
                                                         const char* __restrict__ dZS, const unsigned* __restrict__ zmax, float* __restrict__ P,
                                                         int B, int T, int Fp32, int F, int H) {
  constexpr int MB = 8 / NW;
  constexpr int NBUF = NW == 8 ? 4 : 3;
  constexpr int DPW = 16 / NW;
  extern __shared__ __attribute__((aligned(16))) char dw_smem[];
  const int tid = threadIdx.x, lane = tid & 63;
  const int wave = __builtin_amdgcn_readfirstlane(tid >> 6), wr = wave >> 1, wc = wave & 1;
  const int N = 4 * H;
  const int nft = (Fp32 + DW_BM - 1) / DW_BM, nut = (H + DW_BN - 1) / DW_BN, wps = 4 * nft * nut;
  const XcdTile wt = xcd_tile(blockIdx.x, wps);
  const int b = wt.group;
  if (b >= B) return;
  const int w_ = wt.item, g = w_ / (nft * nut), gb = g * B + b;
  const int q0 = ((w_ / nut) % nft) * DW_BM, u0 = (w_ % nut) * DW_BN;
  const int cnt = kcnt[gb];
  if (q0 >= cnt) return;
  const unsigned lds0 = (unsigned)(uintptr_t)(lds_char*)dw_smem;
  const char* XSb = XS + (size_t)b * F * ldt * 4;
  const char* ZSb = dZS + (size_t)b * N * ldt * 4;

  unsigned a_off[DPW], b_off[DPW];
#pragma unroll
  for (int i = 0; i < DPW; ++i) {
    const int id = DPW * wave + i, part = id >> 3, r = 16 * (id & 7) + (lane >> 2);
    const int ch = (lane & 3) ^ ((r >> 2) & 3);
    int q = q0 + r;
    q = q < cnt ? q : cnt - 1;
    const int f = lists[(size_t)gb * Fp32 + q] & 0xFFFF;
    a_off[i] = (unsigned)f * (unsigned)(4 * ldt) + (unsigned)(part * 2 * ldt + ch * 16);
    int u = u0 + r;
    u = u < H ? u : H - 1;
    b_off[i] = (unsigned)(4 * u + g) * (unsigned)(4 * ldt) + (unsigned)(part * 2 * ldt + ch * 16);
  }
  const int nst = (T + DW_TK - 1) / DW_TK;
  auto issue = [&](int n) {
    const unsigned buf = lds0 + (unsigned)(n % NBUF) * DW_STAGE;
    const int nn = (n < nst ? n : nst - 1) * DW_TK * 2;
#pragma unroll
    for (int i = 0; i < DPW; ++i) {
      ps_dma_b128(XSb + nn, a_off[i], buf + (unsigned)((DPW * wave + i) * 1024));
      ps_dma_b128(ZSb + nn, b_off[i], buf + (unsigned)(16384 + (DPW * wave + i) * 1024));
    }
  };
  const int l31 = lane & 31, kh = lane >> 5;
  unsigned oA[MB][2], oB[2][2];
#pragma unroll
  for (int mb = 0; mb < MB; ++mb) {
    const int m = 32 * MB * wr + 32 * mb + l31;
#pragma unroll
    for (int ks = 0; ks < 2; ++ks) oA[mb][ks] = (unsigned)(m * 64 + 16 * ((2 * ks + kh) ^ ((m >> 2) & 3)));
  }
#pragma unroll
  for (int nb = 0; nb < 2; ++nb) {
    const int nn = 64 * wc + 32 * nb + l31;
#pragma unroll
    for (int ks = 0; ks < 2; ++ks) oB[nb][ks] = (unsigned)(16384 + nn * 64 + 16 * ((2 * ks + kh) ^ ((nn >> 2) & 3)));
  }
  f32x16 acc[MB][2];
  zero_acc(acc);
  constexpr int PD = NBUF - 1;
#pragma unroll
  for (int s0 = 0; s0 < PD; ++s0) issue(s0);
  for (int n = 0; n < nst; ++n) {
    if constexpr (NW == 8)
      asm volatile("s_waitcnt vmcnt(8)" ::: "memory");
    else
      asm volatile("s_waitcnt vmcnt(8)" ::: "memory");
    __syncthreads();
    issue(n + PD);
    const unsigned sb = lds0 + (unsigned)(n % NBUF) * DW_STAGE;
#pragma unroll
    for (int ks = 0; ks < 2; ++ks) {
      dw_f4 fa[MB][2], fb[2][2];
      const unsigned ca0 = sb + oA[0][ks], ca1 = sb + oA[MB - 1][ks], cb0 = sb + oB[0][ks], cb1 = sb + oB[1][ks];
      if constexpr (MB == 1)
        asm volatile("ds_read_b128 %0, %6\n\tds_read_b128 %2, %7\n\tds_read_b128 %4, %8\n\tds_read_b128 %1, %6 offset:8192"
                     "\n\tds_read_b128 %3, %7 offset:8192\n\tds_read_b128 %5, %8 offset:8192\n\ts_waitcnt lgkmcnt(0)"
                     : "=&v"(fa[0][0]), "=&v"(fa[0][1]), "=&v"(fb[0][0]), "=&v"(fb[0][1]), "=&v"(fb[1][0]), "=&v"(fb[1][1])
                     : "v"(ca0), "v"(cb0), "v"(cb1)
                     : "memory");
      else
        asm volatile("ds_read_b128 %0, %8\n\tds_read_b128 %4, %10\n\tds_read_b128 %6, %11\n\tds_read_b128 %2, %9"
                     "\n\tds_read_b128 %1, %8 offset:8192\n\tds_read_b128 %5, %10 offset:8192\n\tds_read_b128 %7, %11 offset:8192"
                     "\n\tds_read_b128 %3, %9 offset:8192\n\ts_waitcnt lgkmcnt(0)"
                     : "=&v"(fa[0][0]), "=&v"(fa[0][1]), "=&v"(fa[MB - 1][0]), "=&v"(fa[MB - 1][1]), "=&v"(fb[0][0]), "=&v"(fb[0][1]),
                       "=&v"(fb[1][0]), "=&v"(fb[1][1])
                     : "v"(ca0), "v"(ca1), "v"(cb0), "v"(cb1)
                     : "memory");
#pragma unroll
      for (int mb = 0; mb < MB; ++mb) {
        const f16x8 ah = __builtin_bit_cast(f16x8, fa[mb][0]), al = __builtin_bit_cast(f16x8, fa[mb][1]);
#pragma unroll
        for (int nb = 0; nb < 2; ++nb) {
          const f16x8 bh = __builtin_bit_cast(f16x8, fb[nb][0]), bl = __builtin_bit_cast(f16x8, fb[nb][1]);
          mfma3_split(ah, al, bh, bl, acc[mb][nb]);
        }
      }
    }
  }
  asm volatile("s_waitcnt vmcnt(0)" ::: "memory");
  const float cf = __uint_as_float(*cword) * (1.f / XS_SCALE);
  float* out = P + (size_t)gb * Fp32 * H;
#pragma unroll
  for (int nb = 0; nb < 2; ++nb) {
    const int u = acc_col(u0 + 64 * wc + 32 * nb, l31);
    const float cz = u < H ? 1.f / dw_zscale(zmax[(size_t)b * N + 4 * u + g]) : 0.f;
#pragma unroll
    for (int mb = 0; mb < MB; ++mb)
#pragma unroll
      for (int reg = 0; reg < 16; ++reg) {
        const int r = acc_row(32 * MB * wr + 32 * mb, reg, kh);
        if (q0 + r < cnt && u < H) out[(size_t)(q0 + r) * H + u] = acc[mb][nb][reg] * cf * cz;
      }
  }
}

constexpr int DG_SB = 8;
__global__ __launch_bounds__(256) void k_dw_gather32(const float* __restrict__ P, const int* __restrict__ kpos, float* __restrict__ dWp, int B, int F,
                                                     int Fp32, int H, int vec ) {
  const size_t n = (size_t)F * H;
  for (size_t i = blockIdx.x * (size_t)256 + threadIdx.x; i < n; i += (size_t)gridDim.x * 256) {
    const int u = (int)(i % H);
    const int f = (int)(i / H);
    float sacc[4] = {0.f, 0.f, 0.f, 0.f};
    for (int b0 = 0; b0 < B; b0 += DG_SB) {
      int pos[DG_SB][4];
      float v[DG_SB][4];
#pragma unroll
      for (int k = 0; k < DG_SB; ++k)
#pragma unroll
        for (int g = 0; g < 4; ++g) pos[k][g] = b0 + k < B ? (kpos ? kpos[((size_t)g * B + b0 + k) * F + f] : f) : -1;
#pragma unroll
      for (int k = 0; k < DG_SB; ++k)
#pragma unroll
        for (int g = 0; g < 4; ++g) {
          v[k][g] = 0.f;
          if (pos[k][g] >= 0) v[k][g] = P[(((size_t)g * B + b0 + k) * Fp32 + pos[k][g]) * H + u];
        }
#pragma unroll
      for (int k = 0; k < DG_SB; ++k)
#pragma unroll
        for (int g = 0; g < 4; ++g)
          if (pos[k][g] >= 0) sacc[g] += v[k][g];
    }
    float* out = dWp + ((size_t)f * H + u) * 4;
    if (vec) {
      *reinterpret_cast<float4*>(out) = make_float4(sacc[0], sacc[1], sacc[2], sacc[3]);
    } else {
#pragma unroll
      for (int g = 0; g < 4; ++g) out[g] = sacc[g];
    }
  }
}

static bool aligned16(const void* p) { return (reinterpret_cast<uintptr_t>(p) & 15) == 0; }
static int hp_of(int H) { return (H + PS_HP - 1) / PS_HP * PS_HP; }
static int fp32_of(int F) { return (F + PS_SK - 1) / PS_SK * PS_SK; }

}

extern "C" {

struct ProjTsWs { int *lists, *kcnt; unsigned* words ; _Float16* WSp; int* kpos; size_t bytes; };
static ProjTsWs proj_ts_ws_layout(const void* ws, int B, int F, int H) {
  mgr_ws_carver w(ws);
  return {w.take<int>((size_t)4 * B * fp32_of(F)), w.take<int>((size_t)4 * B), w.take<unsigned>(64),
          w.take<_Float16>((size_t)4 * (F + 1) * 2 * hp_of(H)), w.take<int>((size_t)4 * B * F), w.off};
}
size_t mgr_lstm_input_proj_dropout_ts_ws_bytes(int B, int F, int H) { return proj_ts_ws_layout(nullptr, B, F, H).bytes; }

int mgr_lstm_input_proj_dropout_ts(mgr_ctx* c, const float* XS, int ldt, const float* mask4, float drop_rate, const float* Wp,
                                   const float* bp, float* Z, int B, int T, int F, int H, void* ws, size_t ws_bytes) {
  MGR_REQUIRE(c && XS && Wp && bp && Z, "null argument");
  MGR_REQUIRE(B > 0 && T > 0 && H > 0 && F >= 16 && F <= 2048, "bad shape (16 <= F <= 2048)");
  MGR_REQUIRE(ldt % PS_TM == 0 && ldt >= T, "the split copy must be padded to whole row tiles of %d (ldt %d, T %d)", PS_TM, ldt, T);
  MGR_REQUIRE(aligned16(XS) && aligned16(bp) && aligned16(Z) && aligned16(Wp), "XS / bp / Z / Wp must be 16-byte aligned");
  MGR_REQUIRE((size_t)F * ldt * 4 < (1ull << 32), "sample block too large");
  const ProjTsWs L = proj_ts_ws_layout(ws, B, F, H);
  const size_t need = L.bytes;
  MGR_REQUIRE(ws && ws_bytes >= need, "workspace too small");
  (void)drop_rate;
  const int Fp32 = fp32_of(F), Hp = hp_of(H);
  int *lists = L.lists, *kcnt = L.kcnt, *kpos = L.kpos;
  unsigned* words = L.words;
  _Float16* WSp = L.WSp;
  hipStream_t s = mgr_stream(c);
  if (!(c->attr_done & MGR_ATTR_PROJ_SPLIT)) {
    MGR_HIP(hipFuncSetAttribute(reinterpret_cast<const void*>(k_proj_split<2>), hipFuncAttributeMaxDynamicSharedMemorySize, PsCfg<2>::LDS));
    MGR_HIP(hipFuncSetAttribute(reinterpret_cast<const void*>(k_proj_split<4>), hipFuncAttributeMaxDynamicSharedMemorySize, PsCfg<4>::LDS));
    c->attr_done |= MGR_ATTR_PROJ_SPLIT;
  }
  mgr_prof_begin(c, MGR_K_GEMM_NN);
  const char* region = reinterpret_cast<const char*>(words);
  const size_t region_bytes = (size_t)(reinterpret_cast<const char*>(kpos) - region);
  bool frozen = false;
  int hit = -1;
  for (int i = 0; i < MGR_MAX_FROZEN; ++i) frozen = frozen || (c->frozen_w[i] == Wp);
  if (frozen) {
    for (int i = 0; i < MGR_MAX_FROZEN; ++i) {
      const mgr_ctx::PlaneEntry& e = c->planes[i];
      if (e.Wp == Wp && e.ws == ws && e.B == B && e.F == F && e.H == H) hit = i;
    }
  }
  for (int i = 0; i < MGR_MAX_FROZEN; ++i)
    if (i != hit && mgr_planes_overlap(c->planes[i], ws, need)) c->planes[i] = mgr_ctx::PlaneEntry{};
  const bool cached = hit >= 0;
  MGR_HIP(hipMemsetAsync(words + (cached ? 1 : 0), 0, (cached ? 1 : 2) * sizeof(unsigned), s));
  hipLaunchKernelGGL(k_lists32, dim3(4 * B), dim3(64), 0, s, mask4, F, Fp32, lists, kcnt, kpos, words + 1);
  if (!cached) {
    const size_t n4 = (size_t)F * H;
    hipLaunchKernelGGL(k_wmax, dim3(mgr_grid256(n4, 256)), dim3(256), 0, s, Wp, n4, words);
    const size_t n = (size_t)(F + 1) * Hp;
    hipLaunchKernelGGL(k_wplanes, dim3(mgr_grid256(n, 2048)), dim3(256), 0, s, Wp, WSp, F, H, Hp, words);
    if (frozen) {
      int slot = -1;
      for (int i = 0; i < MGR_MAX_FROZEN && slot < 0; ++i)
        if (!c->planes[i].Wp) slot = i;
      if (slot < 0) slot = (int)(c->planes_evict++ % MGR_MAX_FROZEN);
      c->planes[slot] = mgr_ctx::PlaneEntry{Wp, ws, B, F, H, region, region_bytes};
    }
  }
  const int waste128 = (H + 127) / 128 * 128 - H, waste64 = (H + 63) / 64 * 64 - H;
  const bool wide = c->tune[MGR_TUNE_PROJ_TS_TILE] == 2 || (c->tune[MGR_TUNE_PROJ_TS_TILE] == 0 && waste128 - waste64 <= H / 8);
  const int tu = wide ? 128 : 64;
  const int ntiles = ((H + tu - 1) / tu) * ((((T + PS_TM - 1) / PS_TM) * B + 7) / 8) * 8;
  if (wide)
    hipLaunchKernelGGL(k_proj_split<4>, dim3(ntiles), dim3(512), PsCfg<4>::LDS, s, reinterpret_cast<const char*>(XS), ldt, lists, kcnt, words + 1,
                       reinterpret_cast<const char*>(WSp), Hp, words, bp, Z, B, T, Fp32, F, H);
  else
    hipLaunchKernelGGL(k_proj_split<2>, dim3(ntiles), dim3(256), PsCfg<2>::LDS, s, reinterpret_cast<const char*>(XS), ldt, lists, kcnt, words + 1,
                       reinterpret_cast<const char*>(WSp), Hp, words, bp, Z, B, T, Fp32, F, H);
  MGR_LAUNCH_CHECK();
  mgr_prof_end(c, MGR_K_GEMM_NN);
  return 0;
}

struct DwTsGroup { int *lists, *kcnt; unsigned* words ; int* kpos; float* P; };
static DwTsGroup dw_ts_group(mgr_ws_carver& w, int B, int F, int H) {
  const size_t nl = (size_t)4 * B * fp32_of(F);
  return {w.take<int>(nl), w.take<int>((size_t)4 * B), w.take<unsigned>(64), w.take<int>((size_t)4 * B * F), w.take<float>(nl * H)};
}
struct DwTsWs { DwTsGroup dW; float* dZS; unsigned* zmax; DwTsGroup dU; size_t bytes; };
static DwTsWs dw_ts_ws_layout(void* ws, int B, int T, int F, int H, int ldt) {
  mgr_ws_carver w(ws, mgr_lstm_param_grads_ws_bytes(B, T, F, H));
  return {dw_ts_group(w, B, F, H), w.take<float>((size_t)B * 4 * H * ldt), w.take<unsigned>((size_t)B * 4 * H), dw_ts_group(w, B, H, H), w.off};
}
size_t mgr_lstm_param_grads_dropout_ts_ws_bytes(int B, int T, int F, int H, int ldt) { return dw_ts_ws_layout(nullptr, B, T, F, H, ldt).bytes; }

int mgr_lstm_param_grads_dropout_ts(mgr_ctx* c, const float* XS, int ldt, const float* mask4, float drop_rate, const float* Hs, int ldh,
                                    const float* dZ, float* dWp, float* dUp, float* dbp, int B, int T, int F, int H, int reverse,
                                    void* ws, size_t ws_bytes, const unsigned* dzmax, const float* dbsum, const void* proj_ws,
                                    const float* HsT) {
  MGR_REQUIRE(c && XS && mask4 && Hs && dZ && dWp && dUp && dbp, "null argument");
  mgr_planes_forget_range(c, ws, ws_bytes);
  MGR_REQUIRE(B > 0 && T > 0 && H > 0 && F >= 16 && F <= 2048 && ldh >= H, "bad shape (16 <= F <= 2048)");
  MGR_REQUIRE(ldt % 32 == 0 && ldt >= (T + DW_TK - 1) / DW_TK * DW_TK, "the split copy must be padded to whole stages of %d time steps (ldt %d, T %d)", DW_TK, ldt, T);
  MGR_REQUIRE(aligned16(dZ) && aligned16(XS), "dZ / XS must be 16-byte aligned");
  MGR_REQUIRE((size_t)F * ldt * 4 < (1ull << 32) && (size_t)4 * H * ldt * 4 < (1ull << 32), "sample block too large");
  const DwTsWs L = dw_ts_ws_layout(ws, B, T, F, H, ldt);
  MGR_REQUIRE(ws && ws_bytes >= L.bytes, "workspace too small");
  (void)drop_rate;
  mgr_prof_begin(c, MGR_K_GEMM_TN);
  MGR_REQUIRE(!HsT || (H >= 16 && aligned16(HsT) && (size_t)H * ldt * 4 < (1ull << 32)), "HsT: 16 <= H, 16-byte aligned");
  int r = mgr_param_grads_du_db(c, Hs, ldh, dZ, HsT ? nullptr : dUp, dbp, B, T, F, H, reverse, ws, dbsum);
  if (r) return r;
  const int Fp32 = fp32_of(F), N = 4 * H;
  int *lists = L.dW.lists, *kcnt = L.dW.kcnt, *kpos = L.dW.kpos;
  unsigned* words = L.dW.words;
  float *P = L.dW.P, *dZS = L.dZS;
  const unsigned* zmax = dzmax ? dzmax : L.zmax;
  const int Hp32 = fp32_of(H);
  int *lists2 = L.dU.lists, *kcnt2 = L.dU.kcnt;
  unsigned* words2 = L.dU.words;
  float* P2 = L.dU.P;
  hipStream_t s = mgr_stream(c);
  if (!(c->attr_done & MGR_ATTR_DW_SPLIT)) {
    MGR_HIP(hipFuncSetAttribute(reinterpret_cast<const void*>(k_dw_split<8>), hipFuncAttributeMaxDynamicSharedMemorySize, 4 * DW_STAGE));
    MGR_HIP(hipFuncSetAttribute(reinterpret_cast<const void*>(k_dw_split<4>), hipFuncAttributeMaxDynamicSharedMemorySize, 3 * DW_STAGE));
    c->attr_done |= MGR_ATTR_DW_SPLIT;
  }
  if (proj_ws) {
    const ProjTsWs Lp = proj_ts_ws_layout(proj_ws, B, F, H);
    lists = Lp.lists, kcnt = Lp.kcnt, words = Lp.words, kpos = Lp.kpos;
  } else {
    MGR_HIP(hipMemsetAsync(words, 0, 2 * sizeof(unsigned), s));
    hipLaunchKernelGGL(k_lists32, dim3(4 * B), dim3(64), 0, s, mask4, F, Fp32, lists, kcnt, kpos, words + 1);
  }
  if (!dzmax) hipLaunchKernelGGL(k_rowmax_bt, dim3((N + 63) / 64, B), dim3(256), 0, s, dZ, N, T, const_cast<unsigned*>(zmax), (float*)nullptr);
  hipLaunchKernelGGL(k_transpose_split_scaled, dim3((ldt + TS_TT - 1) / TS_TT, (N + 63) / 64, B), dim3(256), 0, s, dZ, N, dZS, ldt, T, zmax,
                     (int)(ldt % 8 == 0));
  if (HsT) {
    const int grid2 = 8 * ((B + 7) / 8) * 4 * ((Hp32 + DW_BM - 1) / DW_BM) * ((H + DW_BN - 1) / DW_BN);
    MGR_HIP(hipMemsetAsync(words2, 0, 2 * sizeof(unsigned), s));
    hipLaunchKernelGGL(k_lists32, dim3(4 * B), dim3(64), 0, s, (const float*)nullptr, H, Hp32, lists2, kcnt2, (int*)nullptr, words2 + 1);
    if (c->tune[MGR_TUNE_PROJ_TS_TILE] == 1)
      hipLaunchKernelGGL(k_dw_split<4>, dim3(grid2), dim3(256), 3 * DW_STAGE, s, reinterpret_cast<const char*>(HsT), ldt, lists2, kcnt2, words2 + 1,
                         reinterpret_cast<const char*>(dZS), zmax, P2, B, T, Hp32, H, H);
    else
      hipLaunchKernelGGL(k_dw_split<8>, dim3(grid2), dim3(512), 4 * DW_STAGE, s, reinterpret_cast<const char*>(HsT), ldt, lists2, kcnt2, words2 + 1,
                         reinterpret_cast<const char*>(dZS), zmax, P2, B, T, Hp32, H, H);
    const size_t n2 = (size_t)H * H;
    hipLaunchKernelGGL(k_dw_gather32, dim3(mgr_grid256(n2, 4096)), dim3(256), 0, s, P2, (const int*)nullptr, dUp, B, H,
                       Hp32, H, (int)aligned16(dUp));
  }
  const int grid = 8 * ((B + 7) / 8) * 4 * ((Fp32 + DW_BM - 1) / DW_BM) * ((H + DW_BN - 1) / DW_BN);
  if (c->tune[MGR_TUNE_PROJ_TS_TILE] == 1)
    hipLaunchKernelGGL(k_dw_split<4>, dim3(grid), dim3(256), 3 * DW_STAGE, s, reinterpret_cast<const char*>(XS), ldt, lists, kcnt, words + 1,
                       reinterpret_cast<const char*>(dZS), zmax, P, B, T, Fp32, F, H);
  else
    hipLaunchKernelGGL(k_dw_split<8>, dim3(grid), dim3(512), 4 * DW_STAGE, s, reinterpret_cast<const char*>(XS), ldt, lists, kcnt, words + 1,
                       reinterpret_cast<const char*>(dZS), zmax, P, B, T, Fp32, F, H);
  const size_t n = (size_t)F * H;
  hipLaunchKernelGGL(k_dw_gather32, dim3(mgr_grid256(n, 4096)), dim3(256), 0, s, P, kpos, dWp, B, F, Fp32, H,
                     (int)aligned16(dWp));
  MGR_LAUNCH_CHECK();
  mgr_prof_end(c, MGR_K_GEMM_TN);
  return 0;
}

int mgr_weight_planes_cache(mgr_ctx* c, const float* Wp, int frozen) {
  MGR_REQUIRE(c && Wp, "null argument");
  for (int i = 0; i < MGR_MAX_FROZEN; ++i) {
    if (c->planes[i].Wp == Wp) c->planes[i] = mgr_ctx::PlaneEntry{};
    if (c->frozen_w[i] == Wp) c->frozen_w[i] = nullptr;
  }
  if (!frozen) return 0;
  for (int i = 0; i < MGR_MAX_FROZEN; ++i)
    if (!c->frozen_w[i]) {
      c->frozen_w[i] = Wp;
      return 0;
    }
  const int victim = (int)(c->frozen_evict++ % MGR_MAX_FROZEN);
  for (int i = 0; i < MGR_MAX_FROZEN; ++i)
    if (c->planes[i].Wp == c->frozen_w[victim]) c->planes[i] = mgr_ctx::PlaneEntry{};
  c->frozen_w[victim] = Wp;
  return 0;
}

int mgr_transpose_bt_split(mgr_ctx* c, const float* X, int ldx, float* XS, int ldt, int B, int T, int F) {
  MGR_REQUIRE(c && X && XS, "null argument");
  MGR_REQUIRE(B > 0 && T > 0 && F > 0 && ldx >= F && ldt >= T && ldt % 8 == 0, "bad shape");
  mgr_prof_begin(c, MGR_K_MISC);
  hipLaunchKernelGGL(k_transpose_split, dim3((ldt + TS_TT - 1) / TS_TT, (F + 63) / 64, B), dim3(256), 0, mgr_stream(c), X, ldx, XS, ldt, T, F, 0LL, ldt, 0,
                     (int)aligned16(XS));
  MGR_LAUNCH_CHECK();
  mgr_prof_end(c, MGR_K_MISC);
  return 0;
}

int mgr_transpose_bt_split_shift(mgr_ctx* c, const float* X, int ldx, float* XS, int ldt, int B, int T, int F, int tshift) {
  MGR_REQUIRE(c && X && XS, "null argument");
  MGR_REQUIRE(B > 0 && T > 0 && F > 0 && ldx >= F && ldt >= T && ldt % 8 == 0 && tshift >= -1 && tshift <= 1, "bad shape");
  mgr_prof_begin(c, MGR_K_MISC);
  hipLaunchKernelGGL(k_transpose_split, dim3((ldt + TS_TT - 1) / TS_TT, (F + 63) / 64, B), dim3(256), 0, mgr_stream(c), X, ldx, XS, ldt, T, F, 0LL, ldt, tshift,
                     (int)aligned16(XS));
  MGR_LAUNCH_CHECK();
  mgr_prof_end(c, MGR_K_MISC);
  return 0;
}

}

int mgr_rowmax_bt(mgr_ctx* c, const float* dZ, int N, int T, int B, unsigned* zmax, float* zsum) {
  hipLaunchKernelGGL(k_rowmax_bt, dim3((N + 63) / 64, B), dim3(256), 0, mgr_stream(c), dZ, N, T, zmax, zsum);
  MGR_LAUNCH_CHECK();
  return 0;
}

int mgr_transpose_bt_split_strided(mgr_ctx* c, const float* X, int ldx, float* XS, int ldt, long long xsb, int ldt_fill, int B, int T, int F) {
  hipLaunchKernelGGL(k_transpose_split, dim3((ldt_fill + TS_TT - 1) / TS_TT, (F + 63) / 64, B), dim3(256), 0, mgr_stream(c), X, ldx, XS, ldt, T, F, xsb, ldt_fill, 0,
                     (int)(aligned16(XS) && ldt % 8 == 0 && xsb % 4 == 0));
  MGR_LAUNCH_CHECK();
  return 0;
}
```

### multimodal-gesture-recognition-with-lstms-and-ctc_amd/engine.py

```python
import collections
import ctypes as C
import itertools
import math

import numpy as np

from . import _capi, decoding
from ._capi import Device, DeviceArray
from .spec import frontend_layers, input_width


def _pad4(n):
    return (n + 3) // 4 * 4


class _Arena:

    def __init__(self, dev):
        self.dev = dev
        self.arrays = []

    def _keep(self, a):
        self.arrays.append(a)
        return a

    def empty(self, shape, dtype=np.float32):
        return self._keep(self.dev.empty(shape, dtype))

    def zeros(self, shape, dtype=np.float32):
        return self._keep(self.dev.zeros(shape, dtype))

    def bytes(self, nbytes):
        return self._keep(self.dev.bytes(nbytes))

    def pinned(self, shape, dtype=np.float32):
        return self.dev.pinned(shape, dtype)

    def release(self, arrays):
        dead = set(id(a) for a in arrays)
        for a in arrays:
            a.free()
        self.arrays = [a for a in self.arrays if id(a) not in dead]
        self.dev._arrays = [a for a in self.dev._arrays if id(a) not in dead]

    def free_all(self):
        dead = set(id(a) for a in self.arrays)
        for a in self.arrays:
            a.free()
        self.dev._arrays = [a for a in self.dev._arrays if id(a) not in dead]
        self.arrays = []


class _LstmDir:

    def __init__(self, prefix, d, fin, H, trainable):
        self.prefix = prefix
        self.d = d
        self.reverse = 1 if d == "bwd" else 0
        self.fin = fin
        self.H = H
        self.trainable = trainable
        self.Wp = self.Up = self.bp = None
        self.gWp = self.gUp = self.gbp = None
        self.mask = None
        self.Z = None
        self.gates = self.cs = self.dZ = self.dzmax = self.dbsum = None
        self.ws_scan = self.ws_pg = self.ws_sp = None
        self.lists_mask = 0
        self.HsT = None
        self.hst_ready = False


class Schedule:

    def __init__(self, pipeline=True, defer_param_grads=True, encoders_run_ahead=True, resident_wait_us=2000,
                 transposed_inputs=True, bptt_beside_deepest_scan=True, split_rows=True, encoders_two_ahead=True,
                 deepest_scan_after_fusion_proj=True, depth1_proj_ahead=True, bptt_yields_beside_scans=True,
                 fused_encoder_scans=True, fused_wide_tiles=True, bptt_direct_when_alone=False, fusion_scan_fused=True,
                 bptt_fused=False, chain_stream_priority=0, param_grads_two_streams=False, first_pass_on_encoder_stream=True,
                 bptt_single_cu=False, du_split=True):
        self.bptt_single_cu = bool(bptt_single_cu)
        self.du_split = bool(du_split)
        self.first_pass_on_encoder_stream = bool(first_pass_on_encoder_stream)
        self.param_grads_two_streams = bool(param_grads_two_streams)
        self.chain_stream_priority = int(chain_stream_priority)
        self.bptt_fused = bool(bptt_fused)
        self.fusion_scan_fused = bool(fusion_scan_fused)
        self.bptt_direct_when_alone = bool(bptt_direct_when_alone)
        self.fused_wide_tiles = bool(fused_wide_tiles)
        self.fused_encoder_scans = bool(fused_encoder_scans)
        self.bptt_yields_beside_scans = bool(bptt_yields_beside_scans)
        self.depth1_proj_ahead = bool(depth1_proj_ahead)
        self.deepest_scan_after_fusion_proj = bool(deepest_scan_after_fusion_proj)
        self.encoders_two_ahead = bool(encoders_two_ahead)
        self.split_rows = bool(split_rows)
        self.bptt_beside_deepest_scan = bool(bptt_beside_deepest_scan)
        self.transposed_inputs = bool(transposed_inputs)
        self.pipeline = bool(pipeline)
        self.defer_param_grads = bool(defer_param_grads)
        self.encoders_run_ahead = bool(encoders_run_ahead)
        self.resident_wait_us = int(resident_wait_us)


class Engine:
    def __init__(self, spec, B, T, Lmax, device=0, seed=1234, comm=None, world=1, inference_only=False, schedule=None):
        self.spec = spec
        self.B, self.T, self.Lmax = int(B), int(T), int(Lmax)
        cdev = getattr(comm, "dev", None)
        if cdev is not None:
            if isinstance(device, Device) and device is not cdev:
                raise ValueError("the communicator was created on another Device than the engine's")
            device = cdev
        self._own_dev = not isinstance(device, Device)
        self.dev = device if isinstance(device, Device) else Device(device)
        self.schedule = schedule or Schedule()
        self.mem = _Arena(self.dev)
        self.lib = self.dev.lib
        self.seed = int(seed)
        self.comm = comm
        self.world = int(world)
        self.inference_only = inference_only
        if self.schedule.chain_stream_priority:
            if self.schedule.chain_stream_priority > 0:
                self.dev.call("mgr_stream_set_priority", 0, 1)
            else:
                self.dev.call("mgr_stream_set_priority", self.ES, -1)
        self._adam_calls = 0
        self.rng_step = 0
        self._risk = None
        self._build()

    def _build(self):
        sp, dev, B, T = self.spec, self.mem, self.B, self.T
        table = sp.weight_table()
        self.seg = {}
        off = 0
        for name, shape, tr, kind in table:
            n = int(np.prod(shape))
            if tr:
                self.seg[name] = (off, n, shape, kind)
                off += _pad4(n)
        self.n_train = off
        self.params = dev.zeros((max(off, 4),))
        self.status = dev.zeros((16,), np.uint32)
        self._pass_status = [dev.zeros((16,), np.uint32) for _ in range(2)]
        self.loss_host = dev.pinned((4,), np.float32)
        self.status_host = dev.pinned((4,), np.uint32)
        self._seq_words = dev.pinned((16,), np.uint32)
        self._seq_words[...] = 0
        self._seq_next = 0
        self._gate_log = collections.deque(maxlen=16)
        self.gloss_host = [dev.pinned((4,), np.float32) for _ in range(2)]
        self._gloss_step = [-1, -1]
        if not self.inference_only:
            self.grads = dev.zeros((max(off, 4) + 4,))
            self.gate_flag = self.grads.view(max(off, 4), (4,))
            self.loss_slot = self.grads.view(max(off, 4) + 1, (1,))
            self.m = dev.zeros((max(off, 4),))
            self.v = dev.zeros((max(off, 4),))
        self.frozen = {}
        for name, shape, tr, kind in table:
            if not tr:
                self.frozen[name] = dev.zeros((_pad4(int(np.prod(shape))),))
        self.kinds = {name: kind for name, _, _, kind in table}
        self.shapes = {name: shape for name, shape, _, _ in table}

        self.dirs = {}
        train = not self.inference_only
        for prefix, fin, H, p, tr in sp.lstm_layers():
            for d in ("fwd", "bwd"):
                L = _LstmDir(prefix, d, fin, H, tr)
                base = "%s/%s" % (prefix, d)
                L.Wp, L.Up, L.bp = (self._wview(base + "/W"), self._wview(base + "/U"), self._wview(base + "/b"))
                if tr and train:
                    L.gWp, L.gUp, L.gbp = (self._gview(base + "/W"), self._gview(base + "/U"), self._gview(base + "/b"))
                    L.gates = dev.empty((B, T, H, 4))
                    L.cs = dev.empty((B, T, H))
                    L.dZ = dev.empty((B, T, 4 * H))
                    L.dzmax = dev.zeros((B, 4 * H), np.uint32)
                    L.dbsum = dev.zeros((B, 4 * H))
                    L.ws_scan = dev.bytes(self.lib.mgr_lstm_scan_ws_bytes(B, T, H))
                    need = (self.lib.mgr_lstm_param_grads_dropout_ws_bytes(B, T, fin, H) if p > 0
                            else self.lib.mgr_lstm_param_grads_ws_bytes(B, T, fin, H))
                    if p > 0 and self.schedule.transposed_inputs:
                        need = max(need, self.lib.mgr_lstm_param_grads_dropout_t_ws_bytes(B, T, fin, H, (T + 127) // 128 * 128))
                        if self._ts_shape(fin):
                            need = max(need, self.lib.mgr_lstm_param_grads_dropout_ts_ws_bytes(B, T, fin, H, (T + 127) // 128 * 128))
                    L.ws_pg = dev.bytes(need)
                if p > 0:
                    L.mask = dev.empty((4, B, fin))
                    need = self.lib.mgr_lstm_input_proj_dropout_ws_bytes(B, fin, H)
                    if self._ts_shape(fin):
                        need = max(need, self.lib.mgr_lstm_input_proj_dropout_ts_ws_bytes(B, fin, H))
                    L.ws_sp = dev.bytes(need)
                L.p = p
                self.dirs[base] = L

        W = sp.concat_width
        self.X = {}
        self.Y1 = {}
        self.Y2 = {}
        self.dY1 = {}
        self.Zbuf = {}
        self.Z1buf = {}
        self._xcur = {}
        self._xin_ring = [{}, {}]
        self._xin_slot = 0
        self._xin_pin = None
        self._xin_user = [-1, -1]
        self._xin_copied = [False, False]
        self._lab_copied = [False, False]
        self._lab_user = [-1, -1]
        self._step_id = 0
        self._synced_step = -1
        self.fe = {}
        for s in sp.streams:
            for ring in self._xin_ring:
                ring[s["name"]] = dev.empty((B, T, input_width(s)))
            if s.get("frontend"):
                self._build_frontend(s, train)
            if s["noise"] > 0:
                self.X[s["name"]] = dev.empty((B, T, s["F"]))
            self.Xin = self._xin_ring[0]
            Hs = [lay["H"] for lay in s["layers"]]
            zf = dev.empty((B, T, 4 * max(Hs)))
            zb = dev.empty((B, T, 4 * max(Hs)))
            self.Zbuf[s["name"]] = (zf, zb)
            if train and self.can_pipeline and self.schedule.depth1_proj_ahead and len(Hs) == 2:
                self.Z1buf[s["name"]] = (dev.empty((B, T, 4 * Hs[0])), dev.empty((B, T, 4 * Hs[0])))
            if len(Hs) == 2:
                self.Y1[s["name"]] = dev.empty((B, T, 2 * Hs[0]))
                if s["trainable"] and train:
                    if s["residual"]:
                        self.Y2[s["name"]] = dev.empty((B, T, 2 * Hs[1]))
                    self.dY1[s["name"]] = dev.empty((B, T, 2 * Hs[0]))
        self.FEAT = dev.empty((B, T, W))
        self._feat_ring = [self.FEAT]
        if (train and self.can_pipeline) or self.inference_only:
            self._feat_ring.append(dev.empty((B, T, W)))
        self.ldt = (T + 127) // 128 * 128
        self.Y1T = {}
        self._featT = {}
        self._featT_ready = {}
        self._xt_split = {}
        if self.schedule.transposed_inputs:
            want = lambda p, F: bool(self.lib.mgr_lstm_input_proj_dropout_wants_transposed(self.dev.ctx, C.c_float(float(p)), int(F)))
            for s in sp.streams:
                if len(s["layers"]) == 2 and want(s["layers"][1]["dropout"], 2 * s["layers"][0]["H"]):
                    self.Y1T[s["name"]] = dev.zeros((B, 2 * s["layers"][0]["H"], self.ldt))
            if sp.fusion and want(sp.fusion["dropout"], W):
                for fb in self._feat_ring:
                    self._featT[fb.ptr] = dev.zeros((B, W, self.ldt))
        self._feat_idx = 0
        self._prefetched = None
        self._prefetched_for = None
        self._masks = {}
        any_tr_stream = any(s["trainable"] for s in sp.streams)
        if sp.fusion:
            Hf = sp.fusion["H"]
            self.ZF = (dev.empty((B, T, 4 * Hf)), dev.empty((B, T, 4 * Hf)))
            self.YF = dev.empty((B, T, 2 * Hf))
            if train:
                self.dYF = dev.empty((B, T, 2 * Hf))
        if train and any_tr_stream:
            self.dFEAT = dev.empty((B, T, W))
        D, Cn = sp.head_width, sp.num_classes
        self.P = dev.empty((B, T, Cn))
        self.head_mask = None
        if train:
            self.dLogits = dev.empty((B, T, Cn))
            self.loss_b = dev.empty((B,))
            self.loss_mean = dev.empty((4,))
            self._lab_ring = [(dev.empty((B, self.Lmax), np.int32), dev.empty((B,), np.int32), dev.empty((B,), np.int32))
                              for _ in range(2)]
            self._lab_slot = 0
            self.labels_d, self.ilen_d, self.llen_d = self._lab_ring[0]
            self._lab_pin = [(dev.pinned((B, self.Lmax), np.int32), dev.pinned((B,), np.int32), dev.pinned((B,), np.int32))
                             for _ in range(2)]
            self.ws_ctc = dev.bytes(self.lib.mgr_ctc_ws_bytes(B, T, Cn, self.Lmax))
            self.ws_dense = dev.bytes(self.lib.mgr_dense_bwd_ws_bytes(B, T, D, Cn))
            self.ws_head = dev.bytes(self.lib.mgr_head_ws_bytes(B, T, D, Cn, self.Lmax))
        self.dev.sync()

    def _build_frontend(self, s, train):
        dev, N = self.mem, self.B * self.T
        layers = []
        for i, c in enumerate(frontend_layers(s["frontend"])):
            lay = dict(c, Y=dev.empty((self.B, self.T, c["F"])), code=dev.empty((N * c["F"],), np.uint8), dX=None)
            if train and s["trainable"] and i > 0:
                lay["dX"] = dev.empty((N * c["Hin"] * c["Win"] * c["Cin"],))
            layers.append(lay)
        ws = None
        if train and s["trainable"]:
            ws = dev.bytes(max(self.lib.mgr_conv_pool_bwd_weights_ws_bytes(N, c["Hin"], c["Win"], c["Cin"], c["ks"], c["Cout"])
                               for c in layers))
        self.fe[s["name"]] = dict(layers=layers, ws=ws, dF=dev.empty((self.B, self.T, s["F"])) if ws is not None else None)

    def _frontend_fwd(self, name, X):
        N = self.B * self.T
        self.fe[name]["X0"] = X
        for c in self.fe[name]["layers"]:
            pre = "%s/%s/" % (name, c["name"])
            self.dev.call("mgr_conv_pool_fwd", X, N, c["Hin"], c["Win"], c["Cin"], self._wview(pre + "W"), self._wview(pre + "b"),
                          c["ks"], c["Cout"], c["Y"], c["code"])
            X = c["Y"]
        return X

    def _frontend_bwd(self, name):
        fe, N = self.fe[name], self.B * self.T
        layers = fe["layers"]
        dY = fe["dF"]
        for i in range(len(layers) - 1, -1, -1):
# ... 41 lines not shown
        if isinstance(out, tuple):
            return tuple(self._nan_rows(o, bad) for o in out)
        if isinstance(out, list) and len(out) == len(bad):
            return [[] if bad[b] else o for b, o in enumerate(out)]
        if isinstance(out, np.ndarray) and out.shape[:1] == bad.shape:
            out = out.copy()
            out[bad] = np.nan if out.dtype.kind == "f" else -1
        return out

    def set_weights(self, weights):
        dev = self.dev
        dev.stream(0)
        self.clear_scan_status()
        for name, shape, tr, kind in self.spec.weight_table():
            if name not in weights:
                continue
            w = np.ascontiguousarray(np.asarray(weights[name], dtype=np.float32))
            if tuple(w.shape) != tuple(shape):
                raise ValueError("weight %s: expected shape %s, got %s" % (name, shape, w.shape))
            dst = self._wview(name)
            if kind in ("kernel", "recurrent", "bias"):
                H = shape[-1] // 4
                rows = 1 if kind == "bias" else shape[0]
                tmp = dev.array(w.reshape(-1))
                dev.call("mgr_lstm_pack", tmp, dst, rows, H, 0)
                dev.sync()
                tmp.free()
            else:
                dst.view(0, (w.size,)).upload(w.reshape(-1))
        dev.sync()
        self._freeze_planes()

    def _freeze_planes(self):
        for L in self.dirs.values():
            if L.ws_sp is not None and (L.prefix + "/" + L.d + "/W") in self.frozen:
                self.dev.call("mgr_weight_planes_cache", L.Wp, 1)

    def get_weights(self):
        dev = self.dev
        dev.stream(0)
        out = {}
        for name, shape, tr, kind in self.spec.weight_table():
            n = int(np.prod(shape))
            src = self._wview(name)
            if kind in ("kernel", "recurrent", "bias"):
                H = shape[-1] // 4
                rows = 1 if kind == "bias" else shape[0]
                tmp = dev.empty((n,))
                dev.call("mgr_lstm_pack", src, tmp, rows, H, 1)
                out[name] = tmp.download().reshape(shape)
                tmp.free()
            else:
                out[name] = src.view(0, (n,)).download().reshape(shape)
        return out

    def get_grads(self):
        dev = self.dev
        dev.stream(0)
        out = {}
        for name, (off, n, shape, kind) in self.seg.items():
            src = self.grads.view(off, (n,))
            if kind in ("kernel", "recurrent", "bias"):
                H = shape[-1] // 4
                rows = 1 if kind == "bias" else shape[0]
                tmp = dev.empty((n,))
                dev.call("mgr_lstm_pack", src, tmp, rows, H, 1)
                out[name] = tmp.download().reshape(shape)
                tmp.free()
            else:
                out[name] = src.download().reshape(shape)
        return out

    def reset_optimizer(self):
        self.m.zero()
        self.v.zero()
        self.clear_scan_status()
        self.iterations = 0

    def _seed(self, slot):
        return (self.seed * 1000003 + self.rng_step * 131 + slot) & 0xFFFFFFFFFFFFFFFF

    SAMPLE_SLOT = 998
    _head_step = 0

    def _sample_seed(self, base):
        return ((self.seed if base is None else int(base)) * 1000003 + self._head_step * 131 + self.SAMPLE_SLOT) & 0xFFFFFFFFFFFFFFFF

    COPY_STREAM = 7
    EV_IN = (41, 42)
    EV_LAB = (43, 44)
    EV_XIN_COPIED = (59, 60)
    EV_LAB_COPIED = (61, 62)

    def _upload_inputs(self, inputs, rand, train, stream=0):
        dev = self.dev
        slot = self._xin_slot ^ 1
        dev.stream(self.COPY_STREAM)
        if self._xin_user[slot] > self._synced_step:
            dev.wait_event(self.COPY_STREAM, self.EV_IN[slot])
        if self._xin_pin is None:
            self._xin_pin = [{s["name"]: dev.pinned((self.B, self.T, input_width(s)), np.float32) for s in self.spec.streams}
                             for _ in range(2)]
        if self._xin_copied[slot]:
            dev.event_sync(self.EV_XIN_COPIED[slot])
        for s in self.spec.streams:
            x = np.asarray(inputs[s["name"]])
            if s.get("frontend"):
                want = (self.B, self.T) + tuple(int(v) for v in s["frontend"]["input_shape"])
                if x.shape != want:
                    raise ValueError("input %s: expected %s got %s" % (s["name"], want, x.shape))
                x = x.reshape(self.B, self.T, -1)
            elif x.shape != (self.B, self.T, s["F"]):
                raise ValueError("input %s: expected %s got %s" % (s["name"], (self.B, self.T, s["F"]), x.shape))
            stage = self._xin_pin[slot][s["name"]]
            np.copyto(stage, x, casting="unsafe")
            nz = rand.get(s["name"] + "/noise") if rand else None
            if train and nz is not None:
                stage += np.asarray(nz, dtype=np.float32)
            dev.h2d_async(self._xin_ring[slot][s["name"]], stage)
        dev.record(self.EV_XIN_COPIED[slot])
        self._xin_copied[slot] = True
        dev.wait(stream, self.COPY_STREAM)
        self._xin_slot = slot
        self._xin_user[slot] = 1 << 60
        self.Xin = self._xin_ring[slot]
        dev.stream(stream)

    XT_BOUND = -2.0
    _fmt_train = True

    @staticmethod
    def _ts_shape(fin):
        return 128 <= fin <= 2048

    def _split_rows_wanted(self):
        if not self.schedule.split_rows or self.inference_only or not self._fmt_train:
            return False
        v = C.c_int()
        self.dev.call("mgr_tune_get", _capi.TUNE_GEMM_F32, C.byref(v))
        return v.value == 0

    def _make_xt(self, X, ldx, XT, B, T, fin):
        split = self._split_rows_wanted() and self._ts_shape(fin)
        self.dev.call("mgr_transpose_bt_split" if split else "mgr_transpose_bt", X, ldx, XT, self.ldt, B, T, fin)
        self._xt_split[XT.ptr] = split

    def _project_pair(self, X, ldx, pair, Ls, B, T, fin, H, XT=None, xt_ready=False):
        masked = bool(pair[0]) and Ls[0].ws_sp is not None
        unmasked_wide = not pair[0] and XT is not None and 128 <= fin <= 2048 and Ls[0].ws_sp is not None
        if XT is not None and (masked or unmasked_wide) and not xt_ready:
            self._make_xt(X, ldx, XT, B, T, fin)
        split = XT is not None and self._xt_split.get(XT.ptr, False)
        if masked or unmasked_wide:
            for d in range(2):
                m, Wp, bp, Z = pair[4 * d:4 * d + 4]
                ws = Ls[d].ws_sp
                p = float(Ls[d].p) if masked else 0.0
                if split:
                    self.dev.call("mgr_lstm_input_proj_dropout_ts", XT, self.ldt, m, p, Wp, bp, Z, B, T, fin, H, ws, ws.nbytes)
                    Ls[d].lists_mask = m if masked else 0
                elif XT is not None:
                    self.dev.call("mgr_lstm_input_proj_dropout_t", XT, self.ldt, m, p, Wp, bp, Z, B, T, fin, H, ws, ws.nbytes, self.XT_BOUND)
                else:
                    self.dev.call("mgr_lstm_input_proj_dropout", X, ldx, m, p, Wp, bp, Z, B, T, fin, H, ws, ws.nbytes)
        else:
            self.dev.call("mgr_lstm_input_proj_pair", X, ldx, *pair, B, T, fin, H)

    def _prep_mask(self, L, train, rand, slot):
        if not train or L.p <= 0:
            return 0
        key = "%s/%s/mask" % (L.prefix, L.d)
        if rand is not None:
            if key in rand and rand[key] is not None:
                L.mask.upload(np.asarray(rand[key], dtype=np.float32))
                return L.mask.ptr
            return 0
        self.dev.call("mgr_dropout_mask", L.mask, L.mask.size, float(L.p), C.c_uint64(self._seed(slot)))
        return L.mask.ptr

    def _forward(self, train, rand):
        if self._prefetched is not None:
            self.dev.wait(0, self.ES)
            self._prefetched = None
        self._enqueue_encoders(train, rand, self.FEAT, 0, self.rng_step)
        self._enqueue_fusion_head(train, rand, self.FEAT, self.rng_step)
        if train:
            self.rng_step += 1

    def _enqueue_encoders(self, train, rand, feat_buf, es, rng_step, hold_scans_for=None):
        for tag, k in self._encoder_phases(train, rand, feat_buf, es, rng_step):
            if tag != "projected":
                continue
            if hold_scans_for is not None and k >= 1:
                self.dev.stream(es)
                self.dev.wait(es, hold_scans_for)

    def _encoder_phases(self, train, rand, feat_buf, es, rng_step, first_stream=None, z_first=None, seq_words=None):
        sp, dev, B, T = self.spec, self.dev, self.B, self.T
        W = sp.concat_width
        save = train and not self.inference_only
        self._fmt_train = bool(train)
        saved_step, self.rng_step = self.rng_step, rng_step
        slot = 0
        cols = {}
        col = 0
        for s in sp.streams:
            cols[s["name"]] = col
            col += sp.stream_width(s)
        dev.stream(es if first_stream is None else first_stream)
        for si, s in enumerate(sp.streams):
            name = s["name"]
            X = self.Xin[name]
            if train and rand is None and s["noise"] > 0:
                dev.call("mgr_add_gaussian_noise", X, self.X[name], X.size, float(s["noise"]),
                         C.c_uint64(self._seed(900 + si)))
                X = self.X[name]
            if name in self.fe:
                X = self._frontend_fwd(name, X)
            self._xcur[name] = X
        depth = max(len(s["layers"]) for s in sp.streams)
        feat_by_scans = True
        split_now = self._split_rows_wanted()
        for k in range(depth):
            jobs = []
            for si, s in enumerate(sp.streams):
                nl = len(s["layers"])
                if k >= nl:
                    continue
                name = s["name"]
                H = s["layers"][k]["H"]
                last = k == nl - 1
                col = cols[name]
                if k == 0:
                    cur, ldcur, fin = self._xcur[name], s["F"], s["F"]
                else:
                    Hp = s["layers"][k - 1]["H"]
                    cur, ldcur, fin = self.Y1[name], 2 * Hp, 2 * Hp
                pair, Ls_pair = [], []
                for di, dname in enumerate(("fwd", "bwd")):
                    L = self.dirs["%s/l%d/%s" % (name, k, dname)]
                    Ls_pair.append(L)
                    slot += 1
                    mptr = self._prep_mask(L, train, rand, slot)
                    self._masks[(L.prefix, L.d)] = mptr
                    zb = z_first[name] if (k == 0 and z_first is not None) else self.Zbuf[name]
                    pair += [mptr, L.Wp, L.bp, zb[di]]
                self._project_pair(cur, ldcur, pair, Ls_pair, B, T, fin, H, XT=self.Y1T.get(name) if k == 1 else None,
                                   xt_ready=True)
                for di, dname in enumerate(("fwd", "bwd")):
                    L = self.dirs["%s/l%d/%s" % (name, k, dname)]
                    Z = (z_first[name] if (k == 0 and z_first is not None) else self.Zbuf[name])[di]
                    R, ldr = 0, 0
                    YT, ytb = 0, 0
                    yt_fmt = 0
                    if not last:
                        Y, ldy = self.Y1[name].view(di * H, (1,)), 2 * H
                        if name in self.Y1T:
                            YT, ytb = self.Y1T[name].ptr + di * H * self.ldt * 4, 2 * H * self.ldt
                            yt_fmt = int(split_now and self._ts_shape(2 * H))
                            self._xt_split[self.Y1T[name].ptr] = bool(yt_fmt)
                    elif nl == 2 and s["residual"] and name in self.Y2 and save:
                        Y, ldy = self.Y2[name].view(di * H, (1,)), 2 * H
                        feat_by_scans = False
                    else:
                        Y, ldy = feat_buf.view(col + di * H, (1,)), W
                        if nl == 2 and s["residual"]:
                            R, ldr = self.Y1[name].view(di * H, (1,)), 2 * H
                        if feat_buf.ptr in self._featT:
                            YT, ytb = self._featT[feat_buf.ptr].ptr + (col + di * H) * self.ldt * 4, W * self.ldt
                            yt_fmt = int(split_now and self._ts_shape(W))
                            self._xt_split[self._featT[feat_buf.ptr].ptr] = bool(yt_fmt)
                    keep = save and L.trainable
                    jobs.append(dict(Z=Z, Up=L.Up, Y=Y, ldy=ldy, R=R, ldr=ldr, gates=L.gates if keep else 0,
                                     cs=L.cs if keep else 0, B=B, T=T, H=H, reverse=L.reverse, YT=YT, ytb=ytb,
                                     ldt=self.ldt if YT else 0, yt_split=yt_fmt))
            if k == 0:
                dev.record(self.EV_IN[self._xin_slot])
            self.rng_step = saved_step
            yield ("projected", k)
            saved_step, self.rng_step = self.rng_step, rng_step
            self._fmt_train = bool(train)
            dev.stream(es)
            self._scan_multi(jobs, "_ws_multi", form=self._enc_scan_form, seq_word=(seq_words or {}).get(k, 0))
            self.rng_step = saved_step
            yield ("scanned", k)
            saved_step, self.rng_step = self.rng_step, rng_step
            self._fmt_train = bool(train)
            dev.stream(es)
        self._featT_ready[feat_buf.ptr] = feat_by_scans
        for si, s in enumerate(sp.streams):
            name = s["name"]
            if len(s["layers"]) == 2 and s["residual"] and name in self.Y2 and save:
                H = s["layers"][-1]["H"]
                dev.call("mgr_add2d", self.Y1[name], 2 * H, self.Y2[name], 2 * H, feat_buf.view(cols[name], (1,)), W,
                         B * T, 2 * H)
        self.rng_step = saved_step

    def _enqueue_fusion_head(self, train, rand, feat_buf, rng_step, dense=True):
        sp, dev, B, T = self.spec, self.dev, self.B, self.T
        W = sp.concat_width
        save = train and not self.inference_only
        self._fmt_train = bool(train)
        saved_step, self.rng_step = self.rng_step, rng_step
        dev.stream(0)
        feat, ldf = feat_buf, W
        self._featin = feat_buf
# ... 815 lines not shown
            dev.wait_event(ES, self.EV_FPROJ)
        for _ in phases:
            pass
        dev.stream(ES)
        dev.record(self.EV_ENC[self._feat_ring.index(nxt)])
        self._prefetched = nxt
        self._prefetched_for = next_inputs
        dev.stream(0)
        yield

    def _resident_gate(self):
        if self.schedule.resident_wait_us <= 0 or getattr(self.comm, "host_blocking", False):
            return None
        return lambda: self.dev.call("mgr_stream_wait_next_resident", self.schedule.resident_wait_us)

    def _enqueue_next_encoders(self, next_inputs, finish, defer, ahead, depth, free_running=False):
        dev, ES = self.dev, self.ES
        self._feat_idx ^= 1
        nxt = self._feat_ring[self._feat_idx]
        self._prefetched_for = next_inputs
        if next_inputs is not None:
            dev.stream(ES)
            self._upload_inputs(next_inputs, None, True, stream=ES)
            self._xin_user[self._xin_slot] = self._step_id
        if not defer:
            finish()
            self._enqueue_encoders(True, None, nxt, ES, self.rng_step, hold_scans_for=0)
        else:
            for tag, k in self._encoder_phases(True, None, nxt, ES, self.rng_step):
                if tag != "projected":
                    continue
                if ahead and k == 0 and not free_running:
                    dev.stream(ES)
                    dev.wait_event(ES, self.EV_FPROJ)
                if k == depth - 1:
                    dev.wait(0, ES)
                    dev.stream(0)
                    finish(self._resident_gate())
                    if ahead:
                        dev.wait_event(ES, self.EV_PREV)
        dev.stream(ES)
        dev.record(self.EV_ENC[self._feat_ring.index(nxt)])
        self._prefetched = nxt

    def _bilstm_backward(self, prefix, dY, lddy, Xin, ldx, fin, Hbuf, ldh, dX, lddx, defer_param_grads=False, XinT=None):
        dev, B, T = self.dev, self.B, self.T
        jobs = []
        for di, dname in enumerate(("fwd", "bwd")):
            L = self.dirs["%s/%s" % (prefix, dname)]
            H = L.H
            dYv = dY.view(di * H, (1,)) if isinstance(dY, DeviceArray) else dY
            jobs.append(dict(dY=dYv, gates=L.gates, cs=L.cs, Up=L.Up, dZ=L.dZ, lddy=lddy, B=B, T=T, H=H,
                             reverse=L.reverse, dzmax=L.dzmax, dbsum=L.dbsum))
        dev.stream(0)
        arr = _capi.make_scan_bwd_jobs(jobs)
        need = self.lib.mgr_lstm_scan_bwd_multi_ws_bytes(len(jobs), arr)
        if getattr(self, "_ws_bwd_multi", None) is None or self._ws_bwd_multi.nbytes < need:
            self._ws_bwd_multi = self.mem.bytes(need)
        beside_scans = self._beside_scans
        wide_ok = self._wide_ok
        form = _capi.BPTT_FORM_AUTO
        if beside_scans and self.schedule.bptt_yields_beside_scans:
            direct = (self._wide_ok or self._gate_words[1] is not None) and self.schedule.bptt_direct_when_alone
            form = _capi.BPTT_FORM_DIRECT if direct else _capi.BPTT_FORM_YIELDING
            if self._gate_words[0] is not None and self.schedule.bptt_fused:
                form = _capi.BPTT_FORM_FUSED_DIRECT if direct else _capi.BPTT_FORM_FUSED
        if self.schedule.bptt_single_cu and jobs[0]["H"] in (32, 64, 100):
            form = _capi.BPTT_FORM_SINGLE_CU
        opts = _capi.make_launch_opts(form, 0)
        _capi.check(self.lib.mgr_lstm_scan_bwd_multi_ex(dev.ctx, len(jobs), arr, self._ws_bwd_multi.ptr, self._ws_bwd_multi.nbytes,
                                                        C.byref(opts)))

        two = self.schedule.param_grads_two_streams

        def param_grads():
            if two:
                dev.stream(0)
                dev.wait(self.PG_STREAM, 0)
            for di, dname in enumerate(("fwd", "bwd")):
                L = self.dirs["%s/%s" % (prefix, dname)]
                H = L.H
                mptr = self._masks.get((L.prefix, L.d), 0)
                if two:
                    dev.stream(self.PG_STREAM if di == 1 else 0)
                if mptr and XinT is not None and self._xt_split.get(XinT.ptr, False):
                    pws = L.ws_sp if (L.ws_sp is not None and L.lists_mask == mptr) else 0
                    L.lists_mask = 0
                    hst = 0
                    if self.schedule.du_split and H >= 16:
                        self._prep_hst(L, Hbuf.view(di * H, (1,)), ldh)
                        hst, L.hst_ready = L.HsT, False
                    with self._narrow_tiles(beside_scans and not wide_ok):
                        dev.call("mgr_lstm_param_grads_dropout_ts", XinT, self.ldt, mptr, float(L.p), Hbuf.view(di * H, (1,)), ldh, L.dZ,
                                 L.gWp, L.gUp, L.gbp, B, T, fin, H, L.reverse, L.ws_pg, L.ws_pg.nbytes, L.dzmax, L.dbsum, pws, hst)
                elif mptr and XinT is not None and self.lib.mgr_lstm_param_grads_dropout_wants_transposed(
                        dev.ctx, C.c_float(float(L.p)), int(fin)):
                    need = self.lib.mgr_lstm_param_grads_dropout_t_ws_bytes(B, T, fin, H, self.ldt)
                    if L.ws_pg.nbytes < need:
                        L.ws_pg = self.mem.bytes(need)
                    dev.call("mgr_lstm_param_grads_dropout_t", XinT, self.ldt, mptr, float(L.p), Hbuf.view(di * H, (1,)), ldh, L.dZ,
                             L.gWp, L.gUp, L.gbp, B, T, fin, H, L.reverse, L.ws_pg, L.ws_pg.nbytes, self.XT_BOUND)
                elif mptr:
                    dev.call("mgr_lstm_param_grads_dropout", Xin, ldx, mptr, float(L.p), Hbuf.view(di * H, (1,)), ldh, L.dZ,
                             L.gWp, L.gUp, L.gbp, B, T, fin, H, L.reverse, L.ws_pg, L.ws_pg.nbytes)
                else:
                    dev.call("mgr_lstm_param_grads", Xin, ldx, mptr, Hbuf.view(di * H, (1,)), ldh, L.dZ, L.gWp, L.gUp,
                             L.gbp, B, T, fin, H, L.reverse, L.ws_pg, L.ws_pg.nbytes)
            if two:
                dev.stream(0)
                dev.wait(0, self.PG_STREAM)
        if not defer_param_grads:
            param_grads()
        if dX is not None:
            for di, dname in enumerate(("fwd", "bwd")):
                L = self.dirs["%s/%s" % (prefix, dname)]
                mptr = self._masks.get((L.prefix, L.d), 0)
                dev.call("mgr_lstm_input_grad", L.dZ, L.Wp, mptr, dX, lddx, 1 if di == 1 else 0, B, T, fin, L.H)
        return param_grads if defer_param_grads else None

    def _prep_hst(self, L, Hdir, ldh):
        if L.hst_ready:
            return
        if L.HsT is None:
            L.HsT = self.dev.zeros((self.B, L.H, self.ldt))
        self.dev.call("mgr_transpose_bt_split_shift", Hdir, ldh, L.HsT, self.ldt, self.B, self.T, L.H, 1 if L.reverse else -1)
        L.hst_ready = True

    def _stream_backward(self, s, col):
        sp, dev, B, T = self.spec, self.dev, self.B, self.T
        W = sp.concat_width
        name = s["name"]
        nl = len(s["layers"])
        dout = self.dFEAT.view(col, (1,))
        dF = self.fe[name]["dF"] if name in self.fe else None
        if nl == 2:
            H1, H2 = s["layers"][0]["H"], s["layers"][1]["H"]
            if s["residual"]:
                Hbuf, ldh = self.Y2[name], 2 * H2
            else:
                Hbuf, ldh = self.FEAT.view(col, (1,)), W
            self._bilstm_backward("%s/l1" % name, dout, W, self.Y1[name], 2 * H1, 2 * H1, Hbuf, ldh,
                                  self.dY1[name], 2 * H1, XinT=self.Y1T.get(name))
            if s["residual"]:
                dev.call("mgr_add2d", self.dY1[name], 2 * H1, dout, W, self.dY1[name], 2 * H1, B * T, 2 * H1)
            self._bilstm_backward("%s/l0" % name, self.dY1[name], 2 * H1, self._xcur[name], s["F"], s["F"],
                                  self.Y1[name], 2 * H1, dF, s["F"] if dF is not None else 0)
        else:
            H1 = s["layers"][0]["H"]
            self._bilstm_backward("%s/l0" % name, dout, W, self._xcur[name], s["F"], s["F"],
                                  self.FEAT.view(col, (1,)), W, dF, s["F"] if dF is not None else 0)
        if dF is not None:
            self._frontend_bwd(name)

    def apply_gradients(self):
        dev, o = self.dev, self.spec.optimizer
        dev.stream(0)
        self._bind()
        dev.call("mgr_update_gate_eval", _capi.SCAN_GAVE_UP | _capi.SCAN_NONFINITE, self.gate_flag)
        gscale = 1.0
        if self.comm is not None:
            self.comm.allreduce_sum(self.grads, max(self.n_train, 4) + 4)
            gscale = 1.0 / self.world
            step = self._step_id - 1
            dev.d2h_async(self.gloss_host[step & 1], self.gate_flag)
            dev.record(self.EV_GLOSS[step & 1])
            self._gloss_step[step & 1] = step
        k = self.iterations
        lr_k = o["lr"] * (1.0 / (1.0 + o["decay"] * k))
        t = k + 1
        b1, b2 = float(np.float32(o["beta_1"])), float(np.float32(o["beta_2"]))
        lr_t = lr_k * math.sqrt(1.0 - b2 ** t) / (1.0 - b1 ** t)
        dev.call("mgr_update_gate_set", self.gate_flag)
        try:
            dev.call("mgr_adam_step", self.params, self.grads, self.m, self.v, self.n_train, lr_t, b1, b2, o["epsilon"],
                     o["clipvalue"] or 0.0, gscale)
            for name, (off, n, shape, kind) in self.seg.items():
                if kind == "kernel":
                    mv = self.spec.kernel_maxnorm(name.rsplit("/", 2)[0])
                    if mv > 0:
                        dev.call("mgr_maxnorm_cols", self.params.view(off, (n,)), shape[0], shape[1], mv, 1e-7)
        finally:
            dev.call("mgr_update_gate_set", 0)
        self._adam_calls += 1

    def close(self):
        if self.dev.ctx is None:
            return
        self.dev.sync()
        if self._own_dev:
            self.dev.close()
            return
        self.dev.call("mgr_scan_status_bind", 0)
        self.mem.free_all()
```

Before: 8.335 million.

## Fuse Adam step with max-norm and cache per-weight prep across steps

Replaces the separate Adam kernel and per-kernel max-norm launches with a single segmented kernel. It applies the Adam update, the column max-norm rescale and a per-slab weight abs-max in one pass. It also adds a generation-tracked cache of input-projection preparation and dU list builds, so unchanged work is skipped on later steps, and folds the db reduction into the dW gather kernel. This cuts kernel launches and repeated passes over the parameters. The cost is extra invalidation bookkeeping and a larger, register-heavy update kernel.

Result: no change. 8.367 million (median of 6 runs) (+0.4%).

```diff
diff --git a/include/mgr.h b/include/mgr.h
--- a/include/mgr.h
+++ b/include/mgr.h
@@ -75,6 +75,8 @@
 int mgr_transpose_bt_split(mgr_ctx* ctx, const float* X, int ldx, float* XS, int ldt, int B, int T, int F);
 int mgr_transpose_bt_split_shift(mgr_ctx* ctx, const float* X, int ldx, float* XS, int ldt, int B, int T, int F, int tshift);
 int mgr_weight_planes_cache(mgr_ctx* ctx, const float* Wp, int frozen);
+int mgr_lstm_input_proj_prepare_ts(mgr_ctx* ctx, int njobs, const float* const* mask4, const float* const* Wp, void* const* ws,
+                                   const size_t* ws_bytes, int B, int F, int H);
 size_t mgr_lstm_scan_ws_bytes(int B, int T, int H);
 int mgr_lstm_scan_fwd(mgr_ctx* ctx, const float* Z, const float* Up, float* Y, int ldy, const float* R,
                       int ldr, float* gates, float* cs, int B, int T, int H, int reverse, void* ws,
@@ -206,6 +208,10 @@
 int mgr_adam_step(mgr_ctx* ctx, float* p, const float* g, float* m, float* v, size_t n, float lr_t, float b1,
                   float b2, float eps, float clipvalue, float gscale);
 int mgr_maxnorm_cols(mgr_ctx* ctx, float* W, int rows, int cols, float maxv, float eps);
+int mgr_update_fused(mgr_ctx* ctx, float* p, const float* g, float* m, float* v, size_t n, float lr_t, float b1, float b2,
+                     float eps, float clipvalue, float gscale, float maxnorm_eps, int nseg, const long long* seg_off,
+                     const int* seg_rows, const int* seg_cols, const float* seg_maxv, float* const* seg_wmax,
+                     unsigned gate_mask);
 int mgr_add2d(mgr_ctx* ctx, const float* A, int lda, const float* Bm, int ldb, float* Out, int ldo, size_t rows,
               int cols);
 int mgr_mean(mgr_ctx* ctx, const float* x, int n, float* out);
diff --git a/multimodal-gesture-recognition-with-lstms-and-ctc_amd/_capi.py b/multimodal-gesture-recognition-with-lstms-and-ctc_amd/_capi.py
--- a/multimodal-gesture-recognition-with-lstms-and-ctc_amd/_capi.py
+++ b/multimodal-gesture-recognition-with-lstms-and-ctc_amd/_capi.py
@@ -53,6 +53,7 @@
     "mgr_transpose_bt_split": (i32, [vp, vp, i32, vp, i32, i32, i32, i32]),
     "mgr_transpose_bt_split_shift": (i32, [vp, vp, i32, vp, i32, i32, i32, i32, i32]),
     "mgr_weight_planes_cache": (i32, [vp, vp, i32]),
+    "mgr_lstm_input_proj_prepare_ts": (i32, [vp, i32, vp, vp, vp, vp, i32, i32, i32]),
     "mgr_lstm_input_proj_pair": (i32, [vp, vp, i32, vp, vp, vp, vp, vp, vp, vp, vp, i32, i32, i32, i32]),
     "mgr_lstm_scan_ws_bytes": (sz, [i32, i32, i32]),
     "mgr_lstm_scan_fwd": (i32, [vp, vp, vp, vp, i32, vp, i32, vp, vp, i32, i32, i32, i32, vp, sz]),
@@ -109,6 +110,8 @@
     "mgr_ctc_loss_grad": (i32, [vp, vp, vp, vp, vp, i32, i32, i32, i32, i32, i32, C.c_float, C.c_float, vp, vp, vp, sz]),
     "mgr_adam_step": (i32, [vp, vp, vp, vp, vp, sz, C.c_float, C.c_float, C.c_float, C.c_float, C.c_float, C.c_float]),
     "mgr_maxnorm_cols": (i32, [vp, vp, i32, i32, C.c_float, C.c_float]),
+    "mgr_update_fused": (i32, [vp, vp, vp, vp, vp, sz, C.c_float, C.c_float, C.c_float, C.c_float, C.c_float, C.c_float, C.c_float,
+                               i32, vp, vp, vp, vp, vp, C.c_uint]),
     "mgr_add2d": (i32, [vp, vp, i32, vp, i32, vp, i32, sz, i32]),
     "mgr_mean": (i32, [vp, vp, i32, vp]),
     "mgr_comm_unique_id": (i32, [C.c_char_p]),
diff --git a/multimodal-gesture-recognition-with-lstms-and-ctc_amd/csrc/common.h b/multimodal-gesture-recognition-with-lstms-and-ctc_amd/csrc/common.h
--- a/multimodal-gesture-recognition-with-lstms-and-ctc_amd/csrc/common.h
+++ b/multimodal-gesture-recognition-with-lstms-and-ctc_amd/csrc/common.h
@@ -10,6 +10,9 @@
 
 constexpr int MGR_MAX_PERSIST = 8;
 constexpr int MGR_MAX_FROZEN = 32;
+constexpr int MGR_MAX_WMAX = 64;
+constexpr int MGR_MAX_PREP = 8;
+constexpr int MGR_WMAX_SLOTS = 64;
 
 constexpr size_t MGR_SMALL_D2H = 4096;
 
@@ -63,6 +66,31 @@
   const void* frozen_w[MGR_MAX_FROZEN];
   PlaneEntry planes[MGR_MAX_FROZEN];
   unsigned planes_evict, frozen_evict;
+  unsigned weights_gen;
+  struct WmaxEntry {
+    const void* W;
+    size_t bytes;
+    const float* slots;
+    int nslots;
+    unsigned gen;
+  };
+  WmaxEntry wmax[MGR_MAX_WMAX];
+  unsigned wmax_evict;
+  struct PrepEntry {
+    const void *Wp, *ws, *mask;
+    int B, F, H, stream;
+    unsigned gen;
+    size_t ws_bytes;
+  };
+  PrepEntry prep[MGR_MAX_PREP];
+  unsigned prep_evict;
+  struct DuListEntry {
+    const void* lists;
+    size_t bytes;
+    int B, H, stream;
+  };
+  DuListEntry du_lists[MGR_MAX_PREP];
+  unsigned du_evict;
 };
 
 int mgr_fail(int code, const char* fmt, ...);
@@ -71,10 +99,29 @@
   const char* a = static_cast<const char*>(p);
   return e.Wp && a < e.region + e.region_bytes && e.region < a + n;
 }
+static inline bool mgr_ranges_overlap(const void* a, size_t na, const void* b, size_t nb) {
+  const char *x = static_cast<const char*>(a), *y = static_cast<const char*>(b);
+  return a && b && x < y + nb && y < x + na;
+}
+static inline void mgr_prepared_forget_range(mgr_ctx* c, const void* p, size_t n) {
+  for (int i = 0; i < MGR_MAX_WMAX; ++i) {
+    const mgr_ctx::WmaxEntry& e = c->wmax[i];
+    if (e.W && (mgr_ranges_overlap(e.W, e.bytes, p, n) || mgr_ranges_overlap(e.slots, e.nslots * sizeof(float), p, n)))
+      c->wmax[i] = mgr_ctx::WmaxEntry{};
+  }
+  for (int i = 0; i < MGR_MAX_PREP; ++i) {
+    const mgr_ctx::PrepEntry& e = c->prep[i];
+    if (e.Wp && (mgr_ranges_overlap(e.ws, e.ws_bytes, p, n) || mgr_ranges_overlap(e.Wp, (size_t)e.F * 4 * e.H * sizeof(float), p, n) ||
+                 mgr_ranges_overlap(e.mask, (size_t)4 * e.B * e.F * sizeof(float), p, n)))
+      c->prep[i] = mgr_ctx::PrepEntry{};
+    if (mgr_ranges_overlap(c->du_lists[i].lists, c->du_lists[i].bytes, p, n)) c->du_lists[i] = mgr_ctx::DuListEntry{};
+  }
+}
 static inline void mgr_planes_forget_range(mgr_ctx* c, const void* p, size_t n) {
   if (!p || !n) return;
   for (int i = 0; i < MGR_MAX_FROZEN; ++i)
     if (mgr_planes_overlap(c->planes[i], p, n)) c->planes[i] = mgr_ctx::PlaneEntry{};
+  mgr_prepared_forget_range(c, p, n);
 }
 
 #define MGR_HIP(expr)                                                                      \
@@ -112,6 +159,22 @@
   float u = (float)(mgr_rand_u32(seed, idx) >> 8) * (1.0f / 16777216.0f);
   return (u >= p) ? inv_keep : 0.0f;
 }
+#ifdef __HIPCC__
+__device__ __forceinline__ void mgr_reduce_tall_part(const float* __restrict__ slab, float* __restrict__ out, int n, int nslab, int wg) {
+  __shared__ float part[8][32];
+  const int e = wg * 32 + (threadIdx.x & 31), kl = threadIdx.x >> 5;
+  float s = 0.f;
+  if (e < n)
+    for (int k = kl; k < nslab; k += 8) s += slab[(size_t)k * n + e];
+  part[kl][threadIdx.x & 31] = s;
+  __syncthreads();
+  if (kl == 0 && e < n) {
+    float t = 0.f;
+    for (int k = 0; k < 8; ++k) t += part[k][threadIdx.x & 31];
+    out[e] = t;
+  }
+}
+#endif
 int mgr_transpose_bt_strided(mgr_ctx* c, const float* X, int ldx, float* XT, int ldt, long long xtb, int ldt_fill, int B, int T, int F);
 int mgr_transpose_bt_split_strided(mgr_ctx* c, const float* X, int ldx, float* XS, int ldt, long long xsb, int ldt_fill, int B, int T, int F);
 int mgr_param_grads_du_db(mgr_ctx* c, const float* Hs, int ldh, const float* dZ, float* dUp, float* dbp, int B, int T, int F, int H, int reverse,
diff --git a/multimodal-gesture-recognition-with-lstms-and-ctc_amd/csrc/elementwise.hip b/multimodal-gesture-recognition-with-lstms-and-ctc_amd/csrc/elementwise.hip
--- a/multimodal-gesture-recognition-with-lstms-and-ctc_amd/csrc/elementwise.hip
+++ b/multimodal-gesture-recognition-with-lstms-and-ctc_amd/csrc/elementwise.hip
@@ -62,6 +62,18 @@
   }
 }
 
+__device__ __forceinline__ float adam_elem(float p, float g, float& m, float& v, float lr_t, float b1, float b2, float eps,
+                                           float clipvalue, float gscale) {
+#pragma clang fp contract(off)
+  float gi = g * gscale;
+  if (clipvalue > 0.f) gi = fminf(fmaxf(gi, -clipvalue), clipvalue);
+  const float mi = b1 * m + (1.f - b1) * gi;
+  const float vi = b2 * v + (1.f - b2) * gi * gi;
+  m = mi;
+  v = vi;
+  return p - lr_t * mi / (sqrtf(vi) + eps);
+}
+
 __global__ void k_adam(float* __restrict__ p, const float* __restrict__ g, float* __restrict__ m, float* __restrict__ v,
                        size_t n, float lr_t, float b1, float b2, float eps, float clipvalue, float gscale,
                        const float* __restrict__ gate, unsigned* __restrict__ skipped) {
@@ -70,13 +82,10 @@
     return;
   }
   for (size_t i = blockIdx.x * (size_t)blockDim.x + threadIdx.x; i < n; i += (size_t)gridDim.x * blockDim.x) {
-    float gi = g[i] * gscale;
-    if (clipvalue > 0.f) gi = fminf(fmaxf(gi, -clipvalue), clipvalue);
-    float mi = b1 * m[i] + (1.f - b1) * gi;
-    float vi = b2 * v[i] + (1.f - b2) * gi * gi;
+    float mi = m[i], vi = v[i];
+    p[i] = adam_elem(p[i], g[i], mi, vi, lr_t, b1, b2, eps, clipvalue, gscale);
     m[i] = mi;
     v[i] = vi;
-    p[i] = p[i] - lr_t * mi / (sqrtf(vi) + eps);
   }
 }
 
@@ -91,7 +100,7 @@
   if (c < cols)
     for (int r = ty; r < rows; r += MN_RG) {
       float w = W[(size_t)r * cols + c];
-      s += w * w;
+      s = __builtin_fmaf(w, w, s);
     }
   part[ty][tx] = s;
   __syncthreads();
@@ -105,6 +114,150 @@
   float sc = part[0][tx];
   if (c < cols)
     for (int r = ty; r < rows; r += MN_RG) W[(size_t)r * cols + c] *= sc;
+}
+
+struct UpdSeg {
+  long long off;
+  int rows, cols;
+  float maxv;
+  int wg0, nwg;
+  float* wmax;
+};
+constexpr int UPD_MAXSEG = 48, UPD_KEEP = 64, UPD_LB = 8, UPD_TC = 16;
+struct UpdTable {
+  int nseg;
+  UpdSeg s[UPD_MAXSEG];
+};
+__global__ __launch_bounds__(UPD_TC * MN_RG) void k_adam_maxnorm(float* __restrict__ p, const float* __restrict__ g, float* __restrict__ m,
+                                                              float* __restrict__ v, const UpdTable tab, float lr_t, float b1, float b2,
+                                                              float eps, float clipvalue, float gscale, float mn_eps,
+                                                              const float* __restrict__ gate, const unsigned* __restrict__ status,
+                                                              unsigned gate_mask, unsigned* __restrict__ skipped) {
+  __shared__ float part[MN_RG][UPD_TC];
+  __shared__ float wred[UPD_TC * MN_RG / 64];
+  const bool closed = (gate && gate[0] != 0.f) || (status && (status[0] & gate_mask) != 0u);
+  if (closed && skipped && blockIdx.x == 0 && threadIdx.x == 0) atomicAdd(skipped, 1u);
+  int si = 0;
+  while (si + 1 < tab.nseg && (int)blockIdx.x >= tab.s[si + 1].wg0) ++si;
+  const long long off = tab.s[si].off;
+  const int rows = tab.s[si].rows, cols = tab.s[si].cols, wg = (int)blockIdx.x - tab.s[si].wg0, nwg = tab.s[si].nwg;
+  const float maxv = tab.s[si].maxv;
+  float* const wslots = tab.s[si].wmax;
+  float* __restrict__ P = p + off;
+  const float* __restrict__ G = g + off;
+  float* __restrict__ M = m + off;
+  float* __restrict__ V = v + off;
+  if (rows == 0) {
+    if (closed) return;
+    for (size_t i = (size_t)wg * blockDim.x + threadIdx.x; i < (size_t)cols; i += (size_t)nwg * blockDim.x) {
+      float mi = M[i], vi = V[i];
+      P[i] = adam_elem(P[i], G[i], mi, vi, lr_t, b1, b2, eps, clipvalue, gscale);
+      M[i] = mi;
+      V[i] = vi;
+    }
+    return;
+  }
+  const int tx = threadIdx.x % UPD_TC, ty = threadIdx.x / UPD_TC;
+  const bool scale = maxv > 0.f && !closed;
+  float wm = 0.f;
+  for (int ct = wg; ct < (cols + UPD_TC - 1) / UPD_TC; ct += nwg) {
+    const int c = ct * UPD_TC + tx;
+    const bool in = c < cols;
+    const int cc = in ? c : cols - 1;
+    const size_t rs = (size_t)MN_RG * cols;
+    const unsigned vo = (unsigned)ty * cols + cc, safe = ty < rows ? vo : cc;
+    float wk[UPD_KEEP];
+    float s = 0.f;
+#pragma unroll
+    for (int k0 = 0; k0 < UPD_KEEP; k0 += UPD_LB) {
+      float pv[UPD_LB], gv[UPD_LB], mv[UPD_LB], vv[UPD_LB];
+      if (MN_RG * k0 >= rows) {
+#pragma unroll
+        for (int j = 0; j < UPD_LB; ++j) wk[k0 + j] = 0.f;
+        continue;
+      }
+#pragma unroll
+      for (int j = 0; j < UPD_LB; ++j) {
+        const int r = ty + MN_RG * (k0 + j);
+        const size_t i = r < rows ? (k0 + j) * rs + vo : (size_t)safe;
+        pv[j] = P[i];
+        if (!closed) gv[j] = G[i], mv[j] = M[i], vv[j] = V[i];
+      }
+#pragma unroll
+      for (int j = 0; j < UPD_LB; ++j) {
+        const int r = ty + MN_RG * (k0 + j);
+        float w = 0.f;
+        if (in && r < rows) {
+          const size_t i = (k0 + j) * rs + vo;
+          w = pv[j];
+          if (!closed) {
+            w = adam_elem(pv[j], gv[j], mv[j], vv[j], lr_t, b1, b2, eps, clipvalue, gscale);
+            M[i] = mv[j];
+            V[i] = vv[j];
+          }
+          s = __builtin_fmaf(w, w, s);
+        }
+        wk[k0 + j] = w;
+      }
+      asm volatile("" ::: "memory");
+      __builtin_amdgcn_sched_barrier(0);
+    }
+    if (in)
+      for (int r = ty + MN_RG * UPD_KEEP; r < rows; r += MN_RG) {
+        const size_t i = (size_t)r * cols + c;
+        float w = P[i];
+        if (!closed) {
+          float mi = M[i], vi = V[i];
+          w = adam_elem(w, G[i], mi, vi, lr_t, b1, b2, eps, clipvalue, gscale);
+          M[i] = mi;
+          V[i] = vi;
+          P[i] = w;
+        }
+        s = __builtin_fmaf(w, w, s);
+      }
+    float sc = 1.f;
+    if (scale) {
+      part[ty][tx] = s;
+      __syncthreads();
+      if (ty == 0) {
+        float t = 0.f;
+        for (int k = 0; k < MN_RG; ++k) t += part[k][tx];
+        float nrm = sqrtf(t);
+        part[0][tx] = fminf(fmaxf(nrm, 0.f), maxv) / (mn_eps + nrm);
+      }
+      __syncthreads();
+      sc = part[0][tx];
+      __syncthreads();
+    }
+    if (in) {
+#pragma unroll
+      for (int k = 0; k < UPD_KEEP; ++k) {
+        const int r = ty + MN_RG * k;
+        if (r < rows) {
+          const float w = scale ? wk[k] * sc : wk[k];
+          if (!closed) P[k * rs + vo] = w;
+          wm = fmaxf(wm, fabsf(w));
+        }
+      }
+      for (int r = ty + MN_RG * UPD_KEEP; r < rows; r += MN_RG) {
+        float w = P[(size_t)r * cols + c];
+        if (scale) {
+          w *= sc;
+          P[(size_t)r * cols + c] = w;
+        }
+        wm = fmaxf(wm, fabsf(w));
+      }
+    }
+  }
+#pragma unroll
+  for (int o = 32; o > 0; o >>= 1) wm = fmaxf(wm, __shfl_xor(wm, o));
+  if ((threadIdx.x & 63) == 0) wred[threadIdx.x >> 6] = wm;
+  __syncthreads();
+  if (threadIdx.x == 0 && wslots) {
+    float t = 0.f;
+    for (int k = 0; k < UPD_TC * MN_RG / 64; ++k) t = fmaxf(t, wred[k]);
+    wslots[wg] = t;
+  }
 }
 
 __global__ void k_add2d(const float* __restrict__ A, int lda, const float* __restrict__ Bm, int ldb, float* __restrict__ O,
@@ -227,6 +380,7 @@
   MGR_REQUIRE(c && mask, "null argument");
   MGR_REQUIRE(p >= 0.f && p < 1.f, "dropout rate %f out of [0,1)", p);
   if (n == 0) return 0;
+  mgr_planes_forget_range(c, mask, n * sizeof(float));
   hipLaunchKernelGGL(k_dropout_mask, dim3(grid_for(n)), dim3(kBlock), 0, mgr_stream(c), mask, n, p, 1.0f / (1.0f - p), seed);
   MGR_LAUNCH_CHECK();
   return 0;
@@ -235,6 +389,7 @@
 int mgr_lstm_pack(mgr_ctx* c, const float* src, float* dst, int rows, int H, int to_keras) {
   MGR_REQUIRE(c && src && dst && src != dst, "null or aliased argument");
   MGR_REQUIRE(rows > 0 && H > 0, "bad shape");
+  mgr_planes_forget_range(c, dst, (size_t)rows * 4 * H * sizeof(float));
   hipLaunchKernelGGL(k_pack, dim3(grid_for((size_t)rows * 4 * H)), dim3(kBlock), 0, mgr_stream(c), src, dst, rows, H, to_keras);
   MGR_LAUNCH_CHECK();
   return 0;
@@ -253,6 +408,7 @@
                   float eps, float clipvalue, float gscale) {
   MGR_REQUIRE(c && p && g && m && v, "null argument");
   if (n == 0) return 0;
+  ++c->weights_gen;
   mgr_prof_begin(c, MGR_K_ADAM);
   hipLaunchKernelGGL(k_adam, dim3(grid_for(n)), dim3(kBlock), 0, mgr_stream(c), p, g, m, v, n, lr_t, b1, b2, eps, clipvalue, gscale,
                      c->gate_flag, mgr_status_block(c) + 2);
@@ -264,8 +420,55 @@
 int mgr_maxnorm_cols(mgr_ctx* c, float* W, int rows, int cols, float maxv, float eps) {
   MGR_REQUIRE(c && W, "null argument");
   MGR_REQUIRE(rows > 0 && cols > 0, "bad shape");
+  ++c->weights_gen;
   hipLaunchKernelGGL(k_maxnorm, dim3((cols + 31) / 32), dim3(32 * MN_RG), 0, mgr_stream(c), W, rows, cols, maxv, eps, c->gate_flag);
   MGR_LAUNCH_CHECK();
+  return 0;
+}
+
+int mgr_update_fused(mgr_ctx* c, float* p, const float* g, float* m, float* v, size_t n, float lr_t, float b1, float b2, float eps,
+                     float clipvalue, float gscale, float maxnorm_eps, int nseg, const long long* seg_off, const int* seg_rows,
+                     const int* seg_cols, const float* seg_maxv, float* const* seg_wmax, unsigned gate_mask) {
+  MGR_REQUIRE(c && p && g && m && v && nseg > 0 && seg_off && seg_rows && seg_cols && seg_maxv && seg_wmax, "null argument");
+  for (int i = 0; i < nseg; ++i) {
+    const size_t cnt = seg_rows[i] > 0 ? (size_t)seg_rows[i] * seg_cols[i] : (size_t)seg_cols[i];
+    MGR_REQUIRE(seg_rows[i] >= 0 && seg_cols[i] > 0 && seg_off[i] >= 0 && (size_t)seg_off[i] + cnt <= n,
+                "segment %d (offset %lld, %d x %d) does not lie inside the %zu parameters", i, seg_off[i], seg_rows[i], seg_cols[i], n);
+    MGR_REQUIRE(seg_rows[i] > 0 || (seg_maxv[i] == 0.f && !seg_wmax[i]), "segment %d: a flat segment has no max-norm and no maxima", i);
+  }
+  ++c->weights_gen;
+  mgr_prof_begin(c, MGR_K_ADAM);
+  for (int i0 = 0; i0 < nseg; i0 += UPD_MAXSEG) {
+    UpdTable tab;
+    tab.nseg = nseg - i0 < UPD_MAXSEG ? nseg - i0 : UPD_MAXSEG;
+    int wgs = 0;
+    for (int k = 0; k < tab.nseg; ++k) {
+      const int i = i0 + k;
+      int nwg;
+      if (seg_rows[i] > 0) {
+        nwg = (seg_cols[i] + UPD_TC - 1) / UPD_TC < MGR_WMAX_SLOTS ? (seg_cols[i] + UPD_TC - 1) / UPD_TC : MGR_WMAX_SLOTS;
+      } else {
+        nwg = (seg_cols[i] + 4095) / 4096 < 256 ? (seg_cols[i] + 4095) / 4096 : 256;
+      }
+      tab.s[k] = UpdSeg{seg_off[i], seg_rows[i], seg_cols[i], seg_maxv[i], wgs, nwg, seg_wmax[i]};
+      wgs += nwg;
+      if (seg_wmax[i]) {
+        float* W = p + seg_off[i];
+        int slot = -1;
+        for (int e = 0; e < MGR_MAX_WMAX; ++e)
+          if (c->wmax[e].W == W) slot = e;
+        for (int e = 0; e < MGR_MAX_WMAX && slot < 0; ++e)
+          if (!c->wmax[e].W || c->wmax[e].gen != c->weights_gen) slot = e;
+        if (slot < 0) slot = (int)(c->wmax_evict++ % MGR_MAX_WMAX);
+        c->wmax[slot] = mgr_ctx::WmaxEntry{W, (size_t)seg_rows[i] * seg_cols[i] * sizeof(float), seg_wmax[i], nwg, c->weights_gen};
+      }
+    }
+    hipLaunchKernelGGL(k_adam_maxnorm, dim3(wgs), dim3(UPD_TC * MN_RG), 0, mgr_stream(c), p, g, m, v, tab, lr_t, b1, b2, eps, clipvalue,
+                       gscale, maxnorm_eps, c->gate_flag, gate_mask ? mgr_status_block(c) : (const unsigned*)nullptr, gate_mask,
+                       i0 == 0 ? mgr_status_block(c) + 2 : (unsigned*)nullptr);
+    MGR_LAUNCH_CHECK();
+  }
+  mgr_prof_end(c, MGR_K_ADAM);
   return 0;
 }
 
diff --git a/multimodal-gesture-recognition-with-lstms-and-ctc_amd/csrc/gemm.hip b/multimodal-gesture-recognition-with-lstms-and-ctc_amd/csrc/gemm.hip
--- a/multimodal-gesture-recognition-with-lstms-and-ctc_amd/csrc/gemm.hip
+++ b/multimodal-gesture-recognition-with-lstms-and-ctc_amd/csrc/gemm.hip
@@ -1235,18 +1235,7 @@
 }
 
 __global__ __launch_bounds__(256) void k_reduce_tall(const float* __restrict__ slab, float* __restrict__ out, int n, int nslab) {
-  __shared__ float part[8][32];
-  const int e = blockIdx.x * 32 + (threadIdx.x & 31), kl = threadIdx.x >> 5;
-  float s = 0.f;
-  if (e < n)
-    for (int k = kl; k < nslab; k += 8) s += slab[(size_t)k * n + e];
-  part[kl][threadIdx.x & 31] = s;
-  __syncthreads();
-  if (kl == 0 && e < n) {
-    float t = 0.f;
-    for (int k = 0; k < 8; ++k) t += part[k][threadIdx.x & 31];
-    out[e] = t;
-  }
+  mgr_reduce_tall_part(slab, out, n, nslab, blockIdx.x);
 }
 
 static int tn_groups(int B, int F, int N) {
diff --git a/multimodal-gesture-recognition-with-lstms-and-ctc_amd/csrc/gemm_split.hip b/multimodal-gesture-recognition-with-lstms-and-ctc_amd/csrc/gemm_split.hip
--- a/multimodal-gesture-recognition-with-lstms-and-ctc_amd/csrc/gemm_split.hip
+++ b/multimodal-gesture-recognition-with-lstms-and-ctc_amd/csrc/gemm_split.hip
@@ -21,12 +21,11 @@
 }
 __device__ __forceinline__ int ps_swz(int row) { return ((row & 3) << 2) | ((row >> 2) & 3); }
 
-__global__ __launch_bounds__(64) void k_lists32(const float* __restrict__ mask4, int F, int Fp32, int* __restrict__ lists, int* __restrict__ kcnt,
-                                                int* __restrict__ kpos ,
-                                                unsigned* __restrict__ cword) {
-  const int gb = blockIdx.x, lane = threadIdx.x;
+__device__ __forceinline__ void lists32_wave(const float* __restrict__ mask4, int F, int Fp32, int* __restrict__ lists, int* __restrict__ kcnt,
+                                             int* __restrict__ kpos ,
+                                             unsigned* __restrict__ cword, int gb, int lane) {
   int* out = lists + (size_t)gb * Fp32;
-  int n = 0;
+  int n = 0, first_kept = 0;
   unsigned seen = 0u;
   bool mixed = false;
   if (mask4) {
@@ -43,6 +42,7 @@
         seen = vb;
       }
       if (kpos && f < F) kpos[(size_t)gb * F + f] = take ? n + __popcll(bal & ((1ull << lane) - 1ull)) : -1;
+      if (n == 0 && bal) first_kept = f0 + __ffsll((long long)bal) - 1;
       n += __popcll(bal);
     }
   } else {
@@ -63,9 +63,11 @@
     }
   }
   if (lane == 0) kcnt[gb] = n;
-  __syncthreads();
-  const int first_kept = n > 0 ? (out[0] & 0xFFFF) : 0;
   for (int i = n + lane; i < (n + 31) / 32 * 32; i += 64) out[i] = first_kept | (F << 16);
+}
+__global__ __launch_bounds__(64) void k_lists32(const float* __restrict__ mask4, int F, int Fp32, int* __restrict__ lists, int* __restrict__ kcnt,
+                                                int* __restrict__ kpos, unsigned* __restrict__ cword) {
+  lists32_wave(mask4, F, Fp32, lists, kcnt, kpos, cword, blockIdx.x, threadIdx.x);
 }
 
 __global__ __launch_bounds__(256) void k_wmax(const float* __restrict__ Wp, size_t n4, unsigned* __restrict__ wmax) {
@@ -84,11 +86,10 @@
 __device__ __forceinline__ float ps_wscale(const unsigned* wmax) {
   return split_scale<SPLIT_NONFINITE_ZERO>(__uint_as_float(*wmax), -60);
 }
-__global__ __launch_bounds__(256) void k_wplanes(const float* __restrict__ Wp, _Float16* __restrict__ WS, int F, int H, int Hp,
-                                                 const unsigned* __restrict__ wmax) {
-  const float sw = ps_wscale(wmax);
+__device__ __forceinline__ void wplanes_part(const float* __restrict__ Wp, _Float16* __restrict__ WS, int F, int H, int Hp, float sw, int wg,
+                                             int nwg) {
   const size_t n = (size_t)(F + 1) * Hp;
-  for (size_t i = blockIdx.x * (size_t)256 + threadIdx.x; i < n; i += (size_t)gridDim.x * 256) {
+  for (size_t i = wg * (size_t)256 + threadIdx.x; i < n; i += (size_t)nwg * 256) {
     const int u = (int)(i % Hp), f = (int)(i / Hp);
     float4 w = make_float4(0.f, 0.f, 0.f, 0.f);
     if (f < F && u < H) w = *reinterpret_cast<const float4*>(Wp + ((size_t)f * H + u) * 4);
@@ -102,6 +103,36 @@
       row[Hp + u] = lo;
     }
   }
+}
+__global__ __launch_bounds__(256) void k_wplanes(const float* __restrict__ Wp, _Float16* __restrict__ WS, int F, int H, int Hp,
+                                                 const unsigned* __restrict__ wmax) {
+  wplanes_part(Wp, WS, F, H, Hp, ps_wscale(wmax), blockIdx.x, gridDim.x);
+}
+
+struct PrepJob {
+  const float *mask, *Wp, *slots;
+  int *lists, *kcnt, *kpos;
+  unsigned* words;
+  _Float16* WSp;
+  int nslots;
+};
+struct PrepJobs {
+  int B, F, H, Fp32, Hp, lwg, pwg;
+  PrepJob j[2];
+};
+__global__ __launch_bounds__(256) void k_proj_prep(const PrepJobs a) {
+  const int per = a.lwg + a.pwg;
+  const PrepJob& J = a.j[blockIdx.x / per];
+  const int w = blockIdx.x % per;
+  if (w < a.lwg) {
+    const int gb = w * 4 + (threadIdx.x >> 6);
+    if (gb < 4 * a.B) lists32_wave(J.mask, a.F, a.Fp32, J.lists, J.kcnt, J.kpos, J.words + 1, gb, threadIdx.x & 63);
+    return;
+  }
+  float mx = 0.f;
+  for (int k = 0; k < J.nslots; ++k) mx = fmaxf(mx, J.slots[k]);
+  if (w == a.lwg && threadIdx.x == 0) J.words[0] = __float_as_uint(mx);
+  wplanes_part(J.Wp, J.WSp, a.F, a.H, a.Hp, split_scale<SPLIT_NONFINITE_ZERO>(mx, -60), w - a.lwg, a.pwg);
 }
 
 constexpr int TS_TT = 128, TS_LP = 66;
@@ -517,10 +548,10 @@
 }
 
 constexpr int DG_SB = 8;
-__global__ __launch_bounds__(256) void k_dw_gather32(const float* __restrict__ P, const int* __restrict__ kpos, float* __restrict__ dWp, int B, int F,
-                                                     int Fp32, int H, int vec ) {
+__device__ __forceinline__ void dw_gather32_part(const float* __restrict__ P, const int* __restrict__ kpos, float* __restrict__ dWp, int B, int F,
+                                                 int Fp32, int H, int vec , int wg, int nwg) {
   const size_t n = (size_t)F * H;
-  for (size_t i = blockIdx.x * (size_t)256 + threadIdx.x; i < n; i += (size_t)gridDim.x * 256) {
+  for (size_t i = wg * (size_t)256 + threadIdx.x; i < n; i += (size_t)nwg * 256) {
     const int u = (int)(i % H);
     const int f = (int)(i / H);
     float sacc[4] = {0.f, 0.f, 0.f, 0.f};
@@ -552,6 +583,17 @@
       for (int g = 0; g < 4; ++g) out[g] = sacc[g];
     }
   }
+}
+__global__ __launch_bounds__(256) void k_dw_gather32(const float* __restrict__ P, const int* __restrict__ kpos, float* __restrict__ dWp, int B, int F,
+                                                     int Fp32, int H, int vec) {
+  dw_gather32_part(P, kpos, dWp, B, F, Fp32, H, vec, blockIdx.x, gridDim.x);
+}
+__global__ __launch_bounds__(256) void k_dw_gather32_db(const float* __restrict__ P, float* __restrict__ dUp, int B, int Hp32, int H, int vec,
+                                                        int gwg, const float* __restrict__ dbsum, float* __restrict__ dbp) {
+  if ((int)blockIdx.x < gwg)
+    dw_gather32_part(P, nullptr, dUp, B, H, Hp32, H, vec, blockIdx.x, gwg);
+  else
+    mgr_reduce_tall_part(dbsum, dbp, 4 * H, B, blockIdx.x - gwg);
 }
 
 static bool aligned16(const void* p) { return (reinterpret_cast<uintptr_t>(p) & 15) == 0; }
@@ -592,22 +634,35 @@
     c->attr_done |= MGR_ATTR_PROJ_SPLIT;
   }
   mgr_prof_begin(c, MGR_K_GEMM_NN);
+  bool prepared = false;
+  for (int i = 0; i < MGR_MAX_PREP; ++i) {
+    mgr_ctx::PrepEntry& e = c->prep[i];
+    if (e.Wp == Wp && e.ws == ws && e.mask == mask4 && e.B == B && e.F == F && e.H == H && e.stream == c->cur && e.gen == c->weights_gen) {
+      prepared = true;
+      e = mgr_ctx::PrepEntry{};
+    }
+  }
   const char* region = reinterpret_cast<const char*>(words);
   const size_t region_bytes = (size_t)(reinterpret_cast<const char*>(kpos) - region);
   bool frozen = false;
   int hit = -1;
-  for (int i = 0; i < MGR_MAX_FROZEN; ++i) frozen = frozen || (c->frozen_w[i] == Wp);
+  for (int i = 0; i < MGR_MAX_FROZEN && !prepared; ++i) frozen = frozen || (c->frozen_w[i] == Wp);
   if (frozen) {
     for (int i = 0; i < MGR_MAX_FROZEN; ++i) {
       const mgr_ctx::PlaneEntry& e = c->planes[i];
       if (e.Wp == Wp && e.ws == ws && e.B == B && e.F == F && e.H == H) hit = i;
     }
   }
-  for (int i = 0; i < MGR_MAX_FROZEN; ++i)
-    if (i != hit && mgr_planes_overlap(c->planes[i], ws, need)) c->planes[i] = mgr_ctx::PlaneEntry{};
-  const bool cached = hit >= 0;
-  MGR_HIP(hipMemsetAsync(words + (cached ? 1 : 0), 0, (cached ? 1 : 2) * sizeof(unsigned), s));
-  hipLaunchKernelGGL(k_lists32, dim3(4 * B), dim3(64), 0, s, mask4, F, Fp32, lists, kcnt, kpos, words + 1);
+  if (!prepared) {
+    for (int i = 0; i < MGR_MAX_FROZEN; ++i)
+      if (i != hit && mgr_planes_overlap(c->planes[i], ws, need)) c->planes[i] = mgr_ctx::PlaneEntry{};
+    mgr_prepared_forget_range(c, ws, need);
+  }
+  const bool cached = hit >= 0 || prepared;
+  if (!prepared) {
+    MGR_HIP(hipMemsetAsync(words + (cached ? 1 : 0), 0, (cached ? 1 : 2) * sizeof(unsigned), s));
+    hipLaunchKernelGGL(k_lists32, dim3(4 * B), dim3(64), 0, s, mask4, F, Fp32, lists, kcnt, kpos, words + 1);
+  }
   if (!cached) {
     const size_t n4 = (size_t)F * H;
     hipLaunchKernelGGL(k_wmax, dim3(mgr_grid256(n4, 256)), dim3(256), 0, s, Wp, n4, words);
@@ -636,6 +691,39 @@
   return 0;
 }
 
+int mgr_lstm_input_proj_prepare_ts(mgr_ctx* c, int njobs, const float* const* mask4, const float* const* Wp, void* const* ws,
+                                   const size_t* ws_bytes, int B, int F, int H) {
+  MGR_REQUIRE(c && mask4 && Wp && ws && ws_bytes && njobs >= 1 && njobs <= 2, "null argument / 1 or 2 jobs");
+  MGR_REQUIRE(B > 0 && H > 0 && F >= 16 && F <= 2048, "bad shape (16 <= F <= 2048)");
+  const size_t need = proj_ts_ws_layout(nullptr, B, F, H).bytes;
+  PrepJobs a{B, F, H, fp32_of(F), hp_of(H), B, mgr_grid256((size_t)(F + 1) * hp_of(H), 1024), {}};
+  int n = 0;
+  hipStream_t s = mgr_stream(c);
+  for (int k = 0; k < njobs; ++k) {
+    MGR_REQUIRE(Wp[k] && aligned16(Wp[k]) && ws[k] && ws_bytes[k] >= need, "job %d: Wp (16-byte aligned) / workspace too small", k);
+    for (int o = 0; o < k; ++o) MGR_REQUIRE(!mgr_ranges_overlap(ws[o], need, ws[k], need), "the jobs' workspaces overlap");
+    mgr_planes_forget_range(c, ws[k], need);
+    mgr_ctx::WmaxEntry wm{};
+    for (int e = 0; e < MGR_MAX_WMAX; ++e)
+      if (c->wmax[e].W == Wp[k] && c->wmax[e].bytes == (size_t)F * 4 * H * sizeof(float) && c->wmax[e].gen == c->weights_gen) wm = c->wmax[e];
+    if (!wm.W) continue;
+    const ProjTsWs L = proj_ts_ws_layout(ws[k], B, F, H);
+    a.j[n++] = PrepJob{mask4[k], Wp[k], wm.slots, L.lists, L.kcnt, L.kpos, L.words, L.WSp, wm.nslots};
+    MGR_HIP(hipMemsetAsync(L.words + 1, 0, sizeof(unsigned), s));
+    int slot = -1;
+    for (int e = 0; e < MGR_MAX_PREP && slot < 0; ++e)
+      if (!c->prep[e].Wp) slot = e;
+    if (slot < 0) slot = (int)(c->prep_evict++ % MGR_MAX_PREP);
+    c->prep[slot] = mgr_ctx::PrepEntry{Wp[k], ws[k], mask4[k], B, F, H, c->cur, c->weights_gen, need};
+  }
+  if (n == 0) return 0;
+  mgr_prof_begin(c, MGR_K_GEMM_NN);
+  hipLaunchKernelGGL(k_proj_prep, dim3(n * (a.lwg + a.pwg)), dim3(256), 0, s, a);
+  MGR_LAUNCH_CHECK();
+  mgr_prof_end(c, MGR_K_GEMM_NN);
+  return 0;
+}
+
 struct DwTsGroup { int *lists, *kcnt; unsigned* words ; int* kpos; float* P; };
 static DwTsGroup dw_ts_group(mgr_ws_carver& w, int B, int F, int H) {
   const size_t nl = (size_t)4 * B * fp32_of(F);
@@ -653,6 +741,8 @@
                                     void* ws, size_t ws_bytes, const unsigned* dzmax, const float* dbsum, const void* proj_ws,
                                     const float* HsT) {
   MGR_REQUIRE(c && XS && mask4 && Hs && dZ && dWp && dUp && dbp, "null argument");
+  mgr_ctx::DuListEntry du_kept[MGR_MAX_PREP];
+  memcpy(du_kept, c->du_lists, sizeof(du_kept));
   mgr_planes_forget_range(c, ws, ws_bytes);
   MGR_REQUIRE(B > 0 && T > 0 && H > 0 && F >= 16 && F <= 2048 && ldh >= H, "bad shape (16 <= F <= 2048)");
   MGR_REQUIRE(ldt % 32 == 0 && ldt >= (T + DW_TK - 1) / DW_TK * DW_TK, "the split copy must be padded to whole stages of %d time steps (ldt %d, T %d)", DW_TK, ldt, T);
@@ -663,7 +753,8 @@
   (void)drop_rate;
   mgr_prof_begin(c, MGR_K_GEMM_TN);
   MGR_REQUIRE(!HsT || (H >= 16 && aligned16(HsT) && (size_t)H * ldt * 4 < (1ull << 32)), "HsT: 16 <= H, 16-byte aligned");
-  int r = mgr_param_grads_du_db(c, Hs, ldh, dZ, HsT ? nullptr : dUp, dbp, B, T, F, H, reverse, ws, dbsum);
+  const bool db_with_gather = HsT && dbsum;
+  int r = db_with_gather ? 0 : mgr_param_grads_du_db(c, Hs, ldh, dZ, HsT ? nullptr : dUp, dbp, B, T, F, H, reverse, ws, dbsum);
   if (r) return r;
   const int Fp32 = fp32_of(F), N = 4 * H;
   int *lists = L.dW.lists, *kcnt = L.dW.kcnt, *kpos = L.dW.kpos;
@@ -692,8 +783,19 @@
                      (int)(ldt % 8 == 0));
   if (HsT) {
     const int grid2 = 8 * ((B + 7) / 8) * 4 * ((Hp32 + DW_BM - 1) / DW_BM) * ((H + DW_BN - 1) / DW_BN);
-    MGR_HIP(hipMemsetAsync(words2, 0, 2 * sizeof(unsigned), s));
-    hipLaunchKernelGGL(k_lists32, dim3(4 * B), dim3(64), 0, s, (const float*)nullptr, H, Hp32, lists2, kcnt2, (int*)nullptr, words2 + 1);
+    const size_t du_bytes = (size_t)(reinterpret_cast<const char*>(words2 + 64) - reinterpret_cast<const char*>(lists2));
+    bool du_hit = false;
+    for (int i = 0; i < MGR_MAX_PREP; ++i)
+      du_hit = du_hit || (du_kept[i].lists == lists2 && du_kept[i].bytes == du_bytes && du_kept[i].B == B && du_kept[i].H == H && du_kept[i].stream == c->cur);
+    if (!du_hit) {
+      MGR_HIP(hipMemsetAsync(words2, 0, 2 * sizeof(unsigned), s));
+      hipLaunchKernelGGL(k_lists32, dim3(4 * B), dim3(64), 0, s, (const float*)nullptr, H, Hp32, lists2, kcnt2, (int*)nullptr, words2 + 1);
+    }
+    int slot = -1;
+    for (int i = 0; i < MGR_MAX_PREP && slot < 0; ++i)
+      if (!c->du_lists[i].lists) slot = i;
+    if (slot < 0) slot = (int)(c->du_evict++ % MGR_MAX_PREP);
+    c->du_lists[slot] = mgr_ctx::DuListEntry{lists2, du_bytes, B, H, c->cur};
     if (c->tune[MGR_TUNE_PROJ_TS_TILE] == 1)
       hipLaunchKernelGGL(k_dw_split<4>, dim3(grid2), dim3(256), 3 * DW_STAGE, s, reinterpret_cast<const char*>(HsT), ldt, lists2, kcnt2, words2 + 1,
                          reinterpret_cast<const char*>(dZS), zmax, P2, B, T, Hp32, H, H);
@@ -701,8 +803,12 @@
       hipLaunchKernelGGL(k_dw_split<8>, dim3(grid2), dim3(512), 4 * DW_STAGE, s, reinterpret_cast<const char*>(HsT), ldt, lists2, kcnt2, words2 + 1,
                          reinterpret_cast<const char*>(dZS), zmax, P2, B, T, Hp32, H, H);
     const size_t n2 = (size_t)H * H;
-    hipLaunchKernelGGL(k_dw_gather32, dim3(mgr_grid256(n2, 4096)), dim3(256), 0, s, P2, (const int*)nullptr, dUp, B, H,
-                       Hp32, H, (int)aligned16(dUp));
+    if (db_with_gather)
+      hipLaunchKernelGGL(k_dw_gather32_db, dim3(mgr_grid256(n2, 4096) + (N + 31) / 32), dim3(256), 0, s, P2, dUp, B, Hp32, H,
+                         (int)aligned16(dUp), mgr_grid256(n2, 4096), dbsum, dbp);
+    else
+      hipLaunchKernelGGL(k_dw_gather32, dim3(mgr_grid256(n2, 4096)), dim3(256), 0, s, P2, (const int*)nullptr, dUp, B, H,
+                         Hp32, H, (int)aligned16(dUp));
   }
   const int grid = 8 * ((B + 7) / 8) * 4 * ((Fp32 + DW_BM - 1) / DW_BM) * ((H + DW_BN - 1) / DW_BN);
   if (c->tune[MGR_TUNE_PROJ_TS_TILE] == 1)
@@ -721,6 +827,7 @@
 
 int mgr_weight_planes_cache(mgr_ctx* c, const float* Wp, int frozen) {
   MGR_REQUIRE(c && Wp, "null argument");
+  ++c->weights_gen;
   for (int i = 0; i < MGR_MAX_FROZEN; ++i) {
     if (c->planes[i].Wp == Wp) c->planes[i] = mgr_ctx::PlaneEntry{};
     if (c->frozen_w[i] == Wp) c->frozen_w[i] = nullptr;
diff --git a/multimodal-gesture-recognition-with-lstms-and-ctc_amd/engine.py b/multimodal-gesture-recognition-with-lstms-and-ctc_amd/engine.py
--- a/multimodal-gesture-recognition-with-lstms-and-ctc_amd/engine.py
+++ b/multimodal-gesture-recognition-with-lstms-and-ctc_amd/engine.py
@@ -78,7 +78,8 @@
                  deepest_scan_after_fusion_proj=True, depth1_proj_ahead=True, bptt_yields_beside_scans=True,
                  fused_encoder_scans=True, fused_wide_tiles=True, bptt_direct_when_alone=False, fusion_scan_fused=True,
                  bptt_fused=False, chain_stream_priority=0, param_grads_two_streams=False, first_pass_on_encoder_stream=True,
-                 bptt_single_cu=False, du_split=True):
+                 bptt_single_cu=False, du_split=True, fused_update_tail=True):
+        self.fused_update_tail = bool(fused_update_tail)
         self.bptt_single_cu = bool(bptt_single_cu)
         self.du_split = bool(du_split)
         self.first_pass_on_encoder_stream = bool(first_pass_on_encoder_stream)
@@ -158,6 +159,7 @@
             self.loss_slot = self.grads.view(max(off, 4) + 1, (1,))
             self.m = dev.zeros((max(off, 4),))
             self.v = dev.zeros((max(off, 4),))
+            self._update_table()
         self.frozen = {}
         for name, shape, tr, kind in table:
             if not tr:
@@ -505,6 +507,12 @@
             self._make_xt(X, ldx, XT, B, T, fin)
         split = XT is not None and self._xt_split.get(XT.ptr, False)
         if masked or unmasked_wide:
+            wnames = ["%s/%s/W" % (L.prefix, L.d) for L in Ls]
+            if split and self.schedule.fused_update_tail and not self.inference_only and all(n in self._wmax_slots for n in wnames):
+                vp2 = C.c_void_p * 2
+                self.dev.call("mgr_lstm_input_proj_prepare_ts", 2, vp2(*[pair[4 * d] or None for d in range(2)]),
+                              vp2(*[getattr(pair[4 * d + 1], "ptr", pair[4 * d + 1]) for d in range(2)]), vp2(*[Ls[d].ws_sp.ptr for d in range(2)]),
+                              (C.c_size_t * 2)(*[Ls[d].ws_sp.nbytes for d in range(2)]), B, fin, H)
             for d in range(2):
                 m, Wp, bp, Z = pair[4 * d:4 * d + 4]
                 ws = Ls[d].ws_sp
@@ -1626,11 +1634,34 @@
         if dF is not None:
             self._frontend_bwd(name)
 
+    def _update_table(self):
+        segs, self._wmax_slots, pos = [], {}, 0
+        kernels = [name for name, (_, _, _, kind) in self.seg.items() if kind == "kernel"]
+        slots = self.mem.zeros((64 * max(len(kernels), 1),))
+        for name, (off, n, shape, kind) in self.seg.items():
+            if kind != "kernel":
+                continue
+            if off > pos:
+                segs.append((pos, 0, off - pos, 0.0, 0))
+            mv = self.spec.kernel_maxnorm(name.rsplit("/", 2)[0])
+            self._wmax_slots[name] = slots.ptr + 256 * len(self._wmax_slots)
+            segs.append((off, shape[0], shape[1], float(mv) if mv > 0 else 0.0, self._wmax_slots[name]))
+            pos = off + n
+        if self.n_train > pos:
+            segs.append((pos, 0, self.n_train - pos, 0.0, 0))
+        k = len(segs)
+        self._upd_segs = (k, (C.c_longlong * k)(*[s[0] for s in segs]), (C.c_int * k)(*[s[1] for s in segs]),
+                          (C.c_int * k)(*[s[2] for s in segs]), (C.c_float * k)(*[s[3] for s in segs]),
+                          (C.c_void_p * k)(*[s[4] or None for s in segs]))
+
     def apply_gradients(self):
         dev, o = self.dev, self.spec.optimizer
         dev.stream(0)
         self._bind()
-        dev.call("mgr_update_gate_eval", _capi.SCAN_GAVE_UP | _capi.SCAN_NONFINITE, self.gate_flag)
+        fused = self.schedule.fused_update_tail and self._upd_segs[0] > 0
+        gate_bits = _capi.SCAN_GAVE_UP | _capi.SCAN_NONFINITE
+        if not (fused and self.comm is None):
+            dev.call("mgr_update_gate_eval", gate_bits, self.gate_flag)
         gscale = 1.0
         if self.comm is not None:
             self.comm.allreduce_sum(self.grads, max(self.n_train, 4) + 4)
@@ -1644,6 +1675,16 @@
         t = k + 1
         b1, b2 = float(np.float32(o["beta_1"])), float(np.float32(o["beta_2"]))
         lr_t = lr_k * math.sqrt(1.0 - b2 ** t) / (1.0 - b1 ** t)
+        if fused:
+            if self.comm is not None:
+                dev.call("mgr_update_gate_set", self.gate_flag)
+            try:
+                dev.call("mgr_update_fused", self.params, self.grads, self.m, self.v, self.n_train, lr_t, b1, b2, o["epsilon"],
+                         o["clipvalue"] or 0.0, gscale, 1e-7, *self._upd_segs, 0 if self.comm is not None else gate_bits)
+            finally:
+                dev.call("mgr_update_gate_set", 0)
+            self._adam_calls += 1
+            return
         dev.call("mgr_update_gate_set", self.gate_flag)
         try:
             dev.call("mgr_adam_step", self.params, self.grads, self.m, self.v, self.n_train, lr_t, b1, b2, o["epsilon"],
```
